# LittleDang/2DLIW-SLAM

Hardware: AMD Instinct MI355X
Metric: sliding-window solves/sec (30 KF, 2k scan pts) (higher is better)
Workload: dtype f64; 1 GPU; C2 synthetic: 49152 windows/GPU x (n=30 frames, L=2000 laser_factor blocks, 29 IMU + 29 wheel, 1800 ground); step = init-topology LM solve (cap 50 iters) + marginalization per window; windows_per_gpu=49152, frames=30, laser_blocks=2000, parallelism=windows replicated over 1 GPU(s), no data-path collective, distinct_windows_per_gpu=64

## Files before the change

2dliw-slam_amd/__init__.py:

```python
import ctypes as C
import os

import numpy as np

_HERE = os.path.dirname(os.path.abspath(__file__))
LIB_PATH = os.path.join(_HERE, "libliw_window.so")

LIW_MODE_INIT, LIW_MODE_TRACK, LIW_MODE_MARG = 0, 1, 2
LIW_ENODEV = -19
LASER_PARTIAL = 128
LASER_PARTIAL_COMPACT = 48

dp = C.POINTER(C.c_double)
ip = C.POINTER(C.c_int)
up = C.POINTER(C.c_ubyte)


class LiwError(RuntimeError):
    def __init__(self, code, msg):
        super().__init__("liw error %d: %s" % (code, msg))
        self.code = code


class ParamsC(C.Structure):
    _fields_ = [("T_imu_to_wheel", C.c_double * 16), ("T_imu_to_laser", C.c_double * 16), ("g", C.c_double),
                ("line_to_line_sigma", C.c_double), ("manifold_p_sigma", C.c_double), ("manifold_q_sigma", C.c_double),
                ("imu_noise_acc_sigma", C.c_double * 3), ("imu_bias_acc_sigma", C.c_double * 3),
                ("imu_noise_gyro_sigma", C.c_double * 3), ("imu_bias_gyro_sigma", C.c_double * 3),
                ("wheel_sigma", C.c_double * 3), ("fast_mode", C.c_int), ("normalize_extrinsics", C.c_int),
                ("device", C.c_int)]


class WindowC(C.Structure):
    _fields_ = [("n", C.c_int), ("L", C.c_int), ("states", dp), ("laser_frame", ip), ("laser_pts", dp),
                ("match_pose", dp), ("has_match", up), ("imu_X", dp), ("imu_J", dp), ("imu_sqrtP", dp), ("imu_Dt", dp),
                ("wheel_T", dp), ("wheel_sqrtP", dp), ("wheel_Dt", dp)]


class SummaryC(C.Structure):
    _fields_ = [("iterations", C.c_int), ("successful_steps", C.c_int), ("termination", C.c_int),
                ("initial_cost", C.c_double), ("final_cost", C.c_double)]


class BatchC(C.Structure):
    _fields_ = [("B", C.c_int), ("n", C.c_int), ("Ltot", C.c_int), ("x", C.c_void_p), ("laser_off", C.c_void_p),
                ("laser_frame", C.c_void_p), ("laser_pts", C.c_void_p), ("match_pose", C.c_void_p),
                ("has_match", C.c_void_p), ("imu_X", C.c_void_p), ("imu_J", C.c_void_p), ("imu_sqrtP", C.c_void_p),
                ("imu_Dt", C.c_void_p), ("wheel_T", C.c_void_p), ("wheel_sqrtP", C.c_void_p), ("prior_X", C.c_void_p),
                ("prior_J", C.c_void_p), ("prior_R", C.c_void_p), ("has_prior", C.c_void_p), ("eval_small", C.c_int),
                ("history_records", C.c_int)]


class WsLayoutC(C.Structure):
    _fields_ = [("bytes", C.c_size_t), ("laser_partial_off", C.c_size_t * 2), ("laser_partial_bytes", C.c_size_t),
                ("info_off", C.c_size_t), ("history_off", C.c_size_t), ("laser_partial_stride", C.c_int)]


EXPORTS = [
    "liw_create", "liw_destroy", "liw_last_error", "liw_get_extrinsics", "liw_set_window", "liw_clear_window", "liw_solve", "liw_get_history",
    "liw_linearize", "liw_eval_factors", "liw_marginalize", "liw_get_prior", "liw_set_prior", "liw_batch_ws_layout",
    "liw_batch_set_max_iters", "liw_batch_launch_paths", "liw_batch_packed_rows", "liw_batch_linearize", "liw_batch_time_kernels", "liw_batch_lm_begin", "liw_batch_lm_linearize", "liw_batch_laser_records", "liw_batch_lm_step",
    "liw_batch_lm_finish", "liw_batch_lm_linearize_async", "liw_batch_lm_join", "liw_batch_exchange_doubles", "liw_batch_exchange_pack",
    "liw_batch_exchange_unpack", "liw_batch_solve_sharded", "liw_batch_exchange_timing", "liw_batch_p2p_area_doubles", "liw_batch_p2p_setup", "liw_batch_p2p_status", "liw_batch_solve", "liw_batch_marg_linearize", "liw_batch_marg_schur", "liw_batch_export_dense",
    "liw_set_timing", "liw_get_timing", "liw_batch_imu_preint", "liw_batch_wheel_preint", "liw_imu_preint_create", "liw_imu_preint_destroy", "liw_imu_preint_reset",
    "liw_imu_preint_add", "liw_imu_preint_update_only_t", "liw_imu_preint_Dt", "liw_imu_preint_result",
    "liw_wheel_preint_create", "liw_wheel_preint_destroy", "liw_wheel_preint_reset", "liw_wheel_preint_add",
    "liw_wheel_preint_update_only_t", "liw_wheel_preint_result",
]

_LIB = None


def lib():
    global _LIB
    if _LIB is None:
        if not os.path.exists(LIB_PATH):
            raise LiwError(-2, "libliw_window.so is not built (run python 2dliw-slam_amd/build.py); there is no CPU fallback")
        try:
            import torch
        except ImportError:
            pass
        L = C.CDLL(LIB_PATH)
        L.liw_create.restype = C.c_void_p
        L.liw_create.argtypes = [C.POINTER(ParamsC)]
        L.liw_last_error.restype = C.c_char_p
        L.liw_last_error.argtypes = [C.c_void_p]
        L.liw_destroy.argtypes = [C.c_void_p]
        L.liw_imu_preint_create.restype = C.c_void_p
        L.liw_imu_preint_create.argtypes = [C.POINTER(ParamsC)]
        L.liw_wheel_preint_create.restype = C.c_void_p
        L.liw_wheel_preint_create.argtypes = [C.POINTER(ParamsC)]
        L.liw_imu_preint_Dt.restype = C.c_double
        for name in ("liw_imu_preint_destroy", "liw_wheel_preint_destroy"):
            getattr(L, name).argtypes = [C.c_void_p]
        _LIB = L
    return _LIB


def params_struct(prm, device=0):
    s = ParamsC()
    s.T_imu_to_wheel[:] = [float(v) for v in np.asarray(prm["T_imu_to_wheel"], dtype=np.float64).reshape(16)]
    s.T_imu_to_laser[:] = [float(v) for v in np.asarray(prm["T_imu_to_laser"], dtype=np.float64).reshape(16)]
    for k in ("g", "line_to_line_sigma", "manifold_p_sigma", "manifold_q_sigma"):
        setattr(s, k, float(prm[k]))
    for k in ("imu_noise_acc_sigma", "imu_bias_acc_sigma", "imu_noise_gyro_sigma", "imu_bias_gyro_sigma", "wheel_sigma"):
        getattr(s, k)[:] = [float(v) for v in prm[k]]
    s.fast_mode = int(bool(prm.get("fast_mode", False)))
    s.normalize_extrinsics = int(bool(prm.get("normalize_extrinsics", True)))
    s.device = int(device)
    return s


def _p(a):
    return a.ctypes.data_as(dp)
# ... 216 lines not shown
```

2dliw-slam_amd/batch.py:

```python
import ctypes as C

import numpy as np


XFN = C.CFUNCTYPE(C.c_int, C.c_void_p, C.c_void_p, C.c_void_p, C.c_size_t, C.c_void_p)


def shard_laser(win, rank, world):
    L = int(np.asarray(win["laser_frame"]).shape[0])
    lo, hi = (L * rank) // world, (L * (rank + 1)) // world
    out = dict(win)
    out["laser_frame"] = np.asarray(win["laser_frame"])[lo:hi].copy()
    out["laser_pts"] = np.asarray(win["laser_pts"])[lo:hi].copy()
    return out


def allreduce_sum_(t, group=None):
    import torch.distributed as dist
    if dist.is_available() and dist.is_initialized() and dist.get_world_size(group) > 1:
        dist.all_reduce(t, op=dist.ReduceOp.SUM, group=group)
    return t


def allgather_(out, t, group=None):
# ... 164 lines not shown
        self.comm = comm if comm is not None else TorchComm(group)
        self.exchange_ms, self.exchange_calls, self._xev, self._xbuf = 0.0, 0, [], {}
        self.time_exchange = False
        if world > 1:
            windows = [shard_laser(w, rank, world) for w in windows]
        self.n = int(windows[0]["n"])
        n = self.n
        for w in windows:
            assert int(w["n"]) == n, "uniform n per batch"
        if tile is None:
            self.B = len(windows)
            host = host_arrays(windows)
            self.Ltot = int(host.pop("_Ltot"))
            self.t = {}
            for k, a in host.items():
                if a.size == 0:
                    a = np.zeros(1, dtype=a.dtype)
                self.t[k] = torch.from_numpy(a).to(self.dev)
        else:
            self.t, self.B, self.Ltot = tiled_tensors(windows, tile, self.dev)
        B = self.B
        self.history_records = int(history_records)
        lay = WsLayoutC()
        r = self.L.liw_batch_ws_layout(C.c_int(B), C.c_int(n), C.c_int(self.history_records), C.byref(lay))
        if r < 0:
            raise LiwError(r, "liw_batch_ws_layout")
        self.lay = lay
        self.ws = torch.zeros(int(lay.bytes), dtype=torch.uint8, device=self.dev)
        b = BatchC()
        b.B, b.n, b.Ltot = B, n, self.Ltot
        for k in ("x", "laser_off", "laser_frame", "laser_pts", "match_pose", "has_match", "imu_X", "imu_J", "imu_sqrtP", "imu_Dt",
                  "wheel_T", "wheel_sqrtP", "prior_X", "prior_J", "prior_R", "has_prior"):
            setattr(b, k, self.t[k].data_ptr())
        b.eval_small = 1
        b.history_records = self.history_records
        self.b = b
        nd = int(lay.laser_partial_bytes) // 8
        self.PL_raw = [self.ws[int(lay.laser_partial_off[k]):int(lay.laser_partial_off[k]) + nd * 8].view(torch.float64) for k in range(2)]
        self._pl_mode = 0

    @property
    def PL(self):
        from . import LASER_PARTIAL
        if int(self.lay.laser_partial_stride) == LASER_PARTIAL:
            return self.PL_raw
        out = []
        for k in range(2):
            o = self.torch.empty(self.B * self.n * LASER_PARTIAL, dtype=self.torch.float64, device=self.dev)
            self._chk(self.L.liw_batch_laser_records(self.h, C.byref(self.b), C.c_int(self._pl_mode), C.c_int(k), self._wsp(),
                                                     C.c_void_p(o.data_ptr()), self._stream()))
            out.append(o)
        return out

    INPUT_KEYS = ("x", "laser_off", "laser_frame", "laser_pts", "match_pose", "has_match", "imu_X", "imu_J", "imu_sqrtP", "imu_Dt", "wheel_T", "wheel_sqrtP")

    def rebind(self, t, Ltot):
        for k in self.INPUT_KEYS:
            self.t[k] = t[k]
            setattr(self.b, k, t[k].data_ptr())
        self.Ltot = int(Ltot)
        self.b.Ltot = int(Ltot)

    def close(self):
        if self.h:
            self.L.liw_destroy(self.h)
            self.h = None

    def __del__(self):
        try:
            self.close()
        except Exception:
            pass

    def _chk(self, r):
        if r < 0:
            raise self.LiwError(r, self.L.liw_last_error(self.h).decode())
        return r

    def _stream(self):
        return C.c_void_p(self.torch.cuda.current_stream(self.dev).cuda_stream)

    def _wsp(self):
        return C.c_void_p(self.ws.data_ptr())

    def launch_paths(self):
        flags, rows, blocks = C.c_int(0), C.c_longlong(0), C.c_longlong(0)
        self._chk(self.L.liw_batch_launch_paths(self.h, C.byref(self.b), self._wsp(), C.byref(flags)))
        self._chk(self.L.liw_batch_packed_rows(self.h, C.byref(self.b), self._wsp(), C.byref(rows), C.byref(blocks)))
        return dict(flags=flags.value, large_batch_format=bool(flags.value & 1), lane_per_group_laser=bool(flags.value & 2), packed_rows=rows.value,
                    blocks=blocks.value, padding_ratio=(64.0 * rows.value / blocks.value) if (rows.value and blocks.value) else None)

    def solve(self, mode, max_iters=0, use_graph=False):
        self._pl_mode = int(mode)
        if not self.sharded:
            if use_graph:
                torch = self.torch
                if getattr(self, "_side", None) is None:
                    self._side = torch.cuda.Stream(device=self.dev)
                cur = torch.cuda.current_stream(self.dev)
                self._side.wait_stream(cur)
                with torch.cuda.stream(self._side):
                    self._chk(self.L.liw_batch_solve(self.h, C.byref(self.b), C.c_int(mode), C.c_int(max_iters), self._wsp(), self._stream(), C.c_int(1)))
                cur.wait_stream(self._side)
                return
            self._chk(self.L.liw_batch_solve(self.h, C.byref(self.b), C.c_int(mode), C.c_int(max_iters), self._wsp(), self._stream(), C.c_int(0)))
            return
# ... 323 lines not shown
```

2dliw-slam_amd/csrc/k_linearize.hip:

```cpp
#include <type_traits>
#include <cstring>
#include "liw_kernels.hpp"

#ifndef LIW_IMU_PROBE_NOSTORE
#define LIW_IMU_PROBE_NOSTORE 0
#endif
#ifndef LIW_IMU_PROBE_PHASE
#define LIW_IMU_PROBE_PHASE 0
#endif
namespace liw {

__device__ __forceinline__ void frame_tf_record(const DevParams& P, const double* pose6, int dir, double* o) {
    V3<LJ> p = cast_v3<LJ>(pose6);
    V3<LJ> th(LJ(pose6[3], dir == 0 ? 1.0 : 0.0), LJ(pose6[4], dir == 1 ? 1.0 : 0.0), LJ(pose6[5], dir == 2 ? 1.0 : 0.0));
    Iso<LJ> Twl = mul(make_tf(p, th), cast_iso<LJ>(P.Ril, P.til));
    const LJ tt[2] = {Twl.t.x, Twl.t.y};
    if (dir == 3) {
        for (int r = 0; r < 2; ++r) { for (int c = 0; c < 3; ++c) o[r * 3 + c] = Twl.R(r, c).v; o[6 + r] = tt[r].v; }
    } else {
        for (int r = 0; r < 2; ++r) { for (int c = 0; c < 3; ++c) o[8 + 6 * dir + r * 3 + c] = Twl.R(r, c).d; o[26 + 2 * dir + r] = tt[r].d; }
    }
}
template <int V, int BIT>
__device__ __forceinline__ void bfly_step(double* v, int lane) {
// ... 410 lines not shown
#pragma unroll
                    for (int r = 0; r < 4; ++r) img[so_d[r]] = (ml == 15 && !with_gi) ? 0.0 : gd[r];
                    lds_sync();
                    if (lane < 60 && !LIW_IMU_PROBE_NOSTORE) nt_store<4>(reinterpret_cast<dbl2*>(rec + PIF_D + 2 * lane), *reinterpret_cast<const dbl2*>(img + 2 * lane));
                    if (lane < 15) rec[PIF_GI + lane] = img[120 + lane];
                    lds_sync();
                };
                diag_out(g00, rf, true);
                if (lastb) diag_out(g11, rf + PIFS, false);
                if (mk == 3 && ml == 15) { rf[PIFS + PIF_C] = g00[3]; if (A.CS[0]) (sel ? A.CS[1] : A.CS[0])[cs_index(n, bq, CS_IMU, kq)] = g00[3]; }
                continue;
            }
            double* out = (sel ? A.PI[1] : A.PI[0]) + fg * PIS;
#pragma unroll
            for (int r = 0; r < 4; ++r) {
                const int row = mk + 4 * r;
                if (row < 15 && ml < 15) {
                    out[PI_IJ + row * 15 + ml] = g01[r];
                    if (ml >= row) {
                        const int tq = row * 15 - (row * (row - 1)) / 2 + (ml - row);
                        out[PI_II + tq] = g00[r];
                        out[PI_JJ + tq] = g11[r];
                    }
                }
                if (row < 15 && ml == 15) out[PI_G + row] = g00[r];
                if (r == 3) {
                    if (row == 15 && ml < 15) out[PI_G + 15 + ml] = g01[r];
                    if (row == 15 && ml == 15) out[PI_C] = g00[r];
                }
                if (A.dbg_imu_res && ml == 15 && row < 15) A.dbg_imu_res[fg * 15 + row] = y0[r];
                if (A.dbg_imu_jac && row < 15 && ml < 15) {
                    A.dbg_imu_jac[(fg * 15 + row) * 30 + ml] = y0[r];
                    A.dbg_imu_jac[(fg * 15 + row) * 30 + 15 + ml] = y1[r];
                }
            }
        }
        if constexpr (COAL) {
#pragma unroll
            for (int q = 0; q < GRP; ++q) sraw[q] = srawn[q];
        } else {
#pragma unroll
            for (int q = 0; q < GRP; ++q)
#pragma unroll
                for (int c = 0; c < 4; ++c) sop[q][c] = sopn[q][c];
        }
    }
    LSTAMP(311);
}

constexpr int WHEEL_PER_WAVE = 21;
struct WheelRcTab { int e[PWS]; };
constexpr WheelRcTab make_wheel_rc() {
    WheelRcTab t{};
    for (int e = 0; e < PWS; ++e) {
        int r = 12, c = 12;
        if (e < PW_IJ(0, 0) || (e >= PW_JJ(0, 0) && e < PW_G(0))) {
            const int jj = e >= PW_JJ(0, 0);
            int q = e - (jj ? PW_JJ(0, 0) : 0);
            r = 0;
            while (q >= 6 - r) { q -= 6 - r; ++r; }
            c = r + q + (jj ? 6 : 0); r += jj ? 6 : 0;
        } else if (e < PW_JJ(0, 0)) { r = (e - PW_IJ(0, 0)) / 6; c = 6 + (e - PW_IJ(0, 0)) % 6; }
        else if (e < PW_C) { r = e - PW_G(0); c = 12; }
        t.e[e] = e <= PW_C ? (r << 8) | c : -1;
    }
    return t;
}
__constant__ WheelRcTab c_wheel_rc = make_wheel_rc();
template <int ND, bool COSTCOPY>
__device__ __forceinline__ void wheel_blocks(const LinArgs& A, const DevParams& P, int wave, double* lds, const int* const act) {
    constexpr int LPB = 9 / ND;
    constexpr int MAXB = 63 / LPB;
    typedef LJN<ND> JN;
    const int lane = threadIdx.x & 63, blk = lane / LPB, g = lane % LPB;
    const int f = g / (LPB / 3), e0 = ND == 3 ? 0 : g % 3;
    const int n = A.n, nb = n - 1;
    const long total = (long)(act ? act[0] : A.B) * nb, gb = (long)wave * A.small_per_wave + blk;
    bool on = blk < A.small_per_wave && gb < total;
    const int wi = on ? (int)(gb / nb) : 0, k = on ? (int)(gb % nb) : 0;
    const int b = act ? act[1 + wi] : wi;
    if (on && !act) on = window_live(A, b);
    double* Y = lds + (blk < MAXB ? blk : 0) * 64;
    const size_t fk = on ? (size_t)b * nb + k : 0;
    if (on) {
        const double* si_ = A.x + ((size_t)b * n + k) * 15;
        const double* sj_ = si_ + 15;
        const double* T12 = A.wheel_T + fk * 12;
        const double* sq9 = A.wheel_sqrtP + fk * 9;
        const V3<double> thi = cast_v3<double>(si_ + 3), thj = cast_v3<double>(sj_ + 3);
        V3<JN> arg;
        {
            JN* ac[3] = {&arg.x, &arg.y, &arg.z};
            const double av[3] = {f == 1 ? thj.x : thi.x, f == 1 ? thj.y : thi.y, f == 1 ? thj.z : thi.z};
#pragma unroll
            for (int c = 0; c < 3; ++c) {
                *ac[c] = JN(av[c]);
#pragma unroll
                for (int e = 0; e < ND; ++e) if (f < 2 && c == e0 + e) ac[c]->d[e] = 1.0;
            }
        }
        const M3<JN> Md = exp_so3(arg);
        M3<double> Ri, Rj;
        {
            const int l0 = lane - g;
#pragma unroll
            for (int q = 0; q < 9; ++q) {
                const double mv = Md.m[q].v;
                Ri.m[q] = __shfl(mv, l0, 64);
                Rj.m[q] = __shfl(mv, l0 + LPB / 3, 64);
            }
        }
        const M3<double> Riw = cast_m3<double>(P.Riw);
        const V3<double> tiw(P.tiw[0], P.tiw[1], P.tiw[2]);
        const M3<double> Rwi = mul(Ri, Riw);
        const M3<double> Am = transpose(Rwi);
        const M3<double> RjRiw = mul(Rj, Riw);
        const V3<double> Rjt = mul(Rj, tiw);
        const V3<double> w(Rjt.x + sj_[0] - si_[0], Rjt.y + sj_[1] - si_[1], Rjt.z + sj_[2] - si_[2]);
// ... 83 lines not shown
    if (on && A.dbg_wheel_jac)
        for (int e = g; e < 36; e += LPB) A.dbg_wheel_jac[fk * 36 + e] = Y[(e / 12) * 13 + e % 12];
    int* meta = reinterpret_cast<int*>(lds + WHEEL_PER_WAVE * 64);
    if (g == 0 && blk < MAXB) {
        meta[blk] = on ? (A.lm ? (A.candidate ? 1 - A.lm[b].cur : A.lm[b].cur) : 0) : -1;
        meta[32 + blk] = (int)fk;
        meta[64 + blk] = (int)cs_index(n, b, CS_WHEEL, k);
    }
    lds_sync();
    {
        const long gb0 = (long)wave * A.small_per_wave;
        const int nblk = (int)min((long)A.small_per_wave, total - gb0);
        const int ml = lane < MAXB ? lane : 0;
        const int selv = meta[ml], fkv = meta[32 + ml], csv = meta[64 + ml];
        const bool all_on = __builtin_amdgcn_ballot_w64(lane < nblk && selv < 0) == 0;
        if (lane < PWS / 2) {
            const int rc0 = c_wheel_rc.e[2 * lane], rc1 = c_wheel_rc.e[2 * lane + 1];
            const int r0 = rc0 >> 8, c0 = rc0 & 255;
            const int r1 = rc1 >= 0 ? rc1 >> 8 : 0, c1 = rc1 >= 0 ? rc1 & 255 : 0;
            auto block = [&](int q) {
                const double* Yq = lds + q * 64;
                double2 v;
                v.x = __builtin_fma(Yq[26 + r0], Yq[26 + c0], __builtin_fma(Yq[r0], Yq[c0], Yq[13 + r0] * Yq[13 + c0]));
                const double w1 = __builtin_fma(Yq[26 + r1], Yq[26 + c1], __builtin_fma(Yq[r1], Yq[c1], Yq[13 + r1] * Yq[13 + c1]));
                v.y = rc1 >= 0 ? w1 : 0.0;
                return v;
            };
            auto put = [&](int q, const double2& v) {
                const int sel = __builtin_amdgcn_readlane(selv, q);
                nt_store<8>(reinterpret_cast<double2*>(&(sel ? A.PW[1] : A.PW[0])[(size_t)__builtin_amdgcn_readlane(fkv, q) * PWS + 2 * lane]), v);
            };
            int q = 0;
            if (all_on)
                for (; q + 3 <= nblk; q += 3) {
                    const double2 va = block(q), vb = block(q + 1), vc = block(q + 2);
                    put(q, va); put(q + 1, vb); put(q + 2, vc);
                }
            for (; q < nblk; ++q) {
                const double2 v = block(q);
                if (__builtin_amdgcn_readlane(selv, q) >= 0) put(q, v);
            }
        }
        if (COSTCOPY && A.CS[0] && lane < nblk && selv >= 0) {
            const double* Yq = lds + lane * 64;
            (selv ? A.CS[1] : A.CS[0])[csv] = __builtin_fma(Yq[38], Yq[38], __builtin_fma(Yq[12], Yq[12], Yq[25] * Yq[25]));
        }
    }
}

constexpr int GROUND_PER_WAVE = 32;
struct GroundRcTab { int e[PGS]; };
constexpr GroundRcTab make_ground_rc() {
    GroundRcTab t{};
    for (int e = 0; e < PGS; ++e) {
        int r = 0, c = e;
        while (c >= 7 - r) { c -= 7 - r; ++r; }
        t.e[e] = (r << 8) | (c + r);
    }
    return t;
}
__constant__ GroundRcTab c_ground_rc = make_ground_rc();
template <bool COSTCOPY>
__device__ __forceinline__ void ground_frames(const LinArgs& A, const DevParams& P, int wave, double* lds, const int* const act) {
    const int lane = threadIdx.x & 63, sub = lane >> 1, g = lane & 1;
    const int n = A.n;
    const long total = (long)(act ? act[0] : A.B) * n, gf = (long)wave * GROUND_PER_WAVE + sub;
    bool on = gf < total;
    const int wi = on ? (int)(gf / n) : 0;
    const int b = act ? act[1 + wi] : wi;
    if (on && !act) on = window_live(A, b);
    double* Y = lds + sub * 16;
    const size_t fi = on ? (size_t)b * n + (size_t)(gf % n) : 0;
    if (on) {
        const double* s_ = A.x + fi * 15;
        J3 res[2];
        {
            V3<J3> q;
            q.x = seed<3>(s_[3], 0, g == 1); q.y = seed<3>(s_[4], 1, g == 1); q.z = seed<3>(s_[5], 2, g == 1);
            const M3<J3> R = exp_so3(q);
            const J3 pz = seed<3>(s_[2], 2, g == 0);
            res[0] = (R(2, 0) * P.tiw[0] + R(2, 1) * P.tiw[1] + R(2, 2) * P.tiw[2] + pz) * P.ground_p_info;
            const J3 zx = R(0, 0) * P.Riw[2] + R(0, 1) * P.Riw[5] + R(0, 2) * P.Riw[8];
            const J3 zy = R(1, 0) * P.Riw[2] + R(1, 1) * P.Riw[5] + R(1, 2) * P.Riw[8];
            res[1] = dasin(dsqrt(zy * zy + zx * zx)) * P.ground_q_info;
        }
#pragma unroll
        for (int e = 0; e < 3; ++e) { Y[3 * g + e] = res[0].d[e]; Y[7 + 3 * g + e] = res[1].d[e]; }
        if (g == 0) { Y[6] = res[0].v; Y[13] = res[1].v; }
        if (g == 0 && A.dbg_ground_res) { A.dbg_ground_res[fi * 2] = res[0].v; A.dbg_ground_res[fi * 2 + 1] = res[1].v; }
        if (A.dbg_ground_jac)
            for (int e = 0; e < 3; ++e) { A.dbg_ground_jac[(fi * 2) * 6 + 3 * g + e] = res[0].d[e]; A.dbg_ground_jac[(fi * 2 + 1) * 6 + 3 * g + e] = res[1].d[e]; }
    }
    int* meta = reinterpret_cast<int*>(lds + GROUND_PER_WAVE * 16);
    if (g == 0) { meta[sub] = on ? (A.lm ? (A.candidate ? 1 - A.lm[b].cur : A.lm[b].cur) : 0) : -1; meta[32 + sub] = (int)fi; meta[64 + sub] = (int)cs_index(n, b, CS_GROUND, (int)(gf % n)); }
    lds_sync();
    {
        const long gf0 = (long)wave * GROUND_PER_WAVE;
        const int nfr = (int)min((long)GROUND_PER_WAVE, total - gf0);
        const double mult = (double)n;
        constexpr int LPF = PGS / 2;
        const int j = lane / LPF, pr = lane - j * LPF;
        const bool all_on = __builtin_amdgcn_ballot_w64(lane < nfr && meta[lane & 31] < 0) == 0;
        if (j < 4) {
            const int rc0 = c_ground_rc.e[2 * pr], rc1 = c_ground_rc.e[2 * pr + 1];
            const int r0 = rc0 >> 8, c0 = rc0 & 255, r1 = rc1 >> 8, c1 = rc1 & 255;
            auto frame = [&](int q) {
                const double* Yq = lds + q * 16;
                double2 v;
                v.x = mult * __builtin_fma(Yq[7 + r0], Yq[7 + c0], Yq[r0] * Yq[c0]);
                v.y = mult * __builtin_fma(Yq[7 + r1], Yq[7 + c1], Yq[r1] * Yq[c1]);
                return v;
            };
            auto put = [&](int sel, int fq, const double2& v) { nt_store<8>(reinterpret_cast<double2*>(&(sel ? A.PG[1] : A.PG[0])[(size_t)fq * PGS + 2 * pr]), v); };
            int q = j;
            if (all_on)
                for (; q + 4 < nfr; q += 8) {
                    const int sa = meta[q], fa = meta[32 + q], sb = meta[q + 4], fb = meta[36 + q];
                    const double2 va = frame(q), vb = frame(q + 4);
                    put(sa, fa, va); put(sb, fb, vb);
                }
            for (; q < nfr; q += 4) {
                const int sel = meta[q], fq = meta[32 + q];
                const double2 v = frame(q);
                if (sel >= 0) put(sel, fq, v);
            }
        }
        if (COSTCOPY && A.CS[0] && lane < nfr && meta[lane & 31] >= 0) {
            const double* Yq = lds + lane * 16;
            (meta[lane] ? A.CS[1] : A.CS[0])[meta[64 + lane]] = mult * __builtin_fma(Yq[13], Yq[13], Yq[6] * Yq[6]);
        }
    }
}

constexpr int WG_PER_WAVE = 31, WG_REC = 68;
constexpr int WG_LDS = WG_PER_WAVE * WG_REC + 96;
__device__ __forceinline__ LJN<4> ext4(const J3& a) { LJN<4> r; r.v = a.v; r.d[0] = a.d[0]; r.d[1] = a.d[1]; r.d[2] = a.d[2]; r.d[3] = 0.0; return r; }
template <bool COSTCOPY>
__device__ __forceinline__ void wheel_ground2_blocks(const LinArgs& A, const DevParams& P, int wave, double* lds, const int* const act) {
    typedef LJN<4> J4;
    typedef LJN<6> J6;
    const int lane = threadIdx.x & 63, blk = lane >> 1, f = lane & 1;
    const int n = A.n, nb = n - 1;
    const long total = (long)(act ? act[0] : A.B) * nb, gb = (long)wave * A.small_per_wave + blk;
    bool on = blk < A.small_per_wave && blk < WG_PER_WAVE && gb < total;
    const int wi = on ? (int)(gb / nb) : 0, k = on ? (int)(gb % nb) : 0;
    const int b = act ? act[1 + wi] : wi;
    if (on && !act) on = window_live(A, b);
    double* Y = lds + (blk < WG_PER_WAVE ? blk : 0) * WG_REC;
    const size_t fk = on ? (size_t)b * nb + k : 0, fi0 = on ? (size_t)b * n + k : 0;
    if (on) {
#if defined(LIW_SMALL_PROBE_INCACHE)
        const double* si_ = A.x;
        const double* sj_ = si_ + 15;
        const double* T12 = A.wheel_T;
        const double* sq9 = A.wheel_sqrtP;
#else
// ... 81 lines not shown
            const J6 dx = p.x / len, dy = p.y / len;
            const J6 cz = dy * odx - dx * ody;
            angle = dasin(dsqrt(cz * cz));
        } else {
            angle = len;
        }
        if (len.v < 0.0001 || o_len < 0.0001) res0 = len * sq9[0];
        else res0 = (J6(o_len) - len) * sq9[0];
        res1 = angle * sq9[4];
        const J4 nq = norm(q);
        const double noq = sqrt(oq.x * oq.x + oq.y * oq.y + oq.z * oq.z);
        J4 res2;
        if (nq.v < 0.001 || noq < 0.001) res2 = nq * sq9[8];
        else res2 = (J4(noq) - nq) * sq9[8];
#pragma unroll
        for (int e = 0; e < 3; ++e) {
            const int col = f ? 9 + e : 3 + e;
            Y[col] = res0.d[e]; Y[13 + col] = res1.d[e]; Y[26 + col] = res2.d[e];
        }
        if (f == 0) {
            const double Dp[3][3] = {{res0.d[3], res0.d[4], res0.d[5]}, {res1.d[3], res1.d[4], res1.d[5]}, {res2.d[3], res2.d[3], res2.d[3]}};
#pragma unroll
            for (int r = 0; r < 3; ++r) {
#pragma unroll
                for (int c = 0; c < 3; ++c) {
                    const double v = Dp[r][0] * Rwi.m[c * 3] + Dp[r][1] * Rwi.m[c * 3 + 1] + Dp[r][2] * Rwi.m[c * 3 + 2];
                    Y[r * 13 + 6 + c] = v;
                    Y[r * 13 + c] = -v;
                }
            }
            Y[12] = res0.v; Y[25] = res1.v; Y[38] = res2.v;
        }
    }
    lds_sync();
    if (on && f == 0 && A.dbg_wheel_res)
        for (int r = 0; r < 3; ++r) A.dbg_wheel_res[fk * 3 + r] = Y[r * 13 + 12];
    if (on && A.dbg_wheel_jac)
        for (int e = f; e < 36; e += 2) A.dbg_wheel_jac[fk * 36 + e] = Y[(e / 12) * 13 + e % 12];
    int* meta = reinterpret_cast<int*>(lds + WG_PER_WAVE * WG_REC);
    if (f == 0 && blk < WG_PER_WAVE) {
        meta[blk] = on ? (A.lm ? (A.candidate ? 1 - A.lm[b].cur : A.lm[b].cur) : 0) : -1;
        meta[32 + blk] = (int)fk;
        meta[64 + blk] = (int)cs_index(n, b, CS_WHEEL, k);
        meta[96 + blk] = (int)fi0;
        meta[128 + blk] = (int)cs_index(n, b, CS_GROUND, k);
        meta[160 + blk] = k;
    }
    lds_sync();
    const long gb0 = (long)wave * A.small_per_wave;
    const int nblk = (int)min((long)min(A.small_per_wave, WG_PER_WAVE), total - gb0);
    const int ml = lane < WG_PER_WAVE ? lane : 0;
    const int selv = meta[ml], fkv = meta[32 + ml], csv = meta[64 + ml], fiv = meta[96 + ml], cgv = meta[128 + ml], kv = meta[160 + ml];
    const bool all_on = __builtin_amdgcn_ballot_w64(lane < nblk && selv < 0) == 0;
    if (lane < PWS / 2) {
        const int rc0 = c_wheel_rc.e[2 * lane], rc1 = c_wheel_rc.e[2 * lane + 1];
        const int r0 = rc0 >> 8, c0 = rc0 & 255;
        const int r1 = rc1 >= 0 ? rc1 >> 8 : 0, c1 = rc1 >= 0 ? rc1 & 255 : 0;
        auto block = [&](int q) {
            const double* Yq = lds + q * WG_REC;
            double2 v;
            v.x = __builtin_fma(Yq[26 + r0], Yq[26 + c0], __builtin_fma(Yq[r0], Yq[c0], Yq[13 + r0] * Yq[13 + c0]));
            const double w1 = __builtin_fma(Yq[26 + r1], Yq[26 + c1], __builtin_fma(Yq[r1], Yq[c1], Yq[13 + r1] * Yq[13 + c1]));
            v.y = rc1 >= 0 ? w1 : 0.0;
            return v;
        };
        auto put = [&](int q, const double2& v) {
            const int sel = __builtin_amdgcn_readlane(selv, q);
            nt_store<8>(reinterpret_cast<double2*>(&(sel ? A.PW[1] : A.PW[0])[(size_t)__builtin_amdgcn_readlane(fkv, q) * PWS + 2 * lane]), v);
        };
        int q = 0;
        if (all_on)
            for (; q + 3 <= nblk; q += 3) {
                const double2 va = block(q), vb = block(q + 1), vc = block(q + 2);
                put(q, va); put(q + 1, vb); put(q + 2, vc);
            }
        for (; q < nblk; ++q) {
            const double2 v = block(q);
            if (__builtin_amdgcn_readlane(selv, q) >= 0) put(q, v);
        }
    }
    {
        const double mult = (double)n;
        constexpr int LPF = PGS / 2;
        const int j = lane / LPF, pr = lane - j * LPF;
        const bool any_k0 = __builtin_amdgcn_ballot_w64(lane < nblk && kv == 0) != 0;
        if (j < 4) {
            const int rc0 = c_ground_rc.e[2 * pr], rc1 = c_ground_rc.e[2 * pr + 1];
            const int r0 = rc0 >> 8, c0 = rc0 & 255, r1 = rc1 >> 8, c1 = rc1 & 255;
            for (int pass = 0; pass < (any_k0 ? 2 : 1); ++pass) {
                const int yo = pass ? 53 : 39;
                for (int q = j; q < nblk; q += 4) {
                    const int sel = meta[q], fq = meta[96 + q] + (pass ? 0 : 1), kq = meta[160 + q];
                    const double* Yq = lds + q * WG_REC + yo;
                    double2 v;
                    v.x = mult * __builtin_fma(Yq[7 + r0], Yq[7 + c0], Yq[r0] * Yq[c0]);
                    v.y = mult * __builtin_fma(Yq[7 + r1], Yq[7 + c1], Yq[r1] * Yq[c1]);
                    if (sel >= 0 && (pass == 0 || kq == 0))
                        nt_store<8>(reinterpret_cast<double2*>(&(sel ? A.PG[1] : A.PG[0])[(size_t)fq * PGS + 2 * pr]), v);
                }
            }
        }
        if (COSTCOPY && A.CS[0] && lane < nblk && selv >= 0) {
            const double* Yq = lds + lane * WG_REC;
            double* CSb = selv ? A.CS[1] : A.CS[0];
            CSb[csv] = __builtin_fma(Yq[38], Yq[38], __builtin_fma(Yq[12], Yq[12], Yq[25] * Yq[25]));
            CSb[cgv + 1] = mult * __builtin_fma(Yq[39 + 13], Yq[39 + 13], Yq[39 + 6] * Yq[39 + 6]);
            if (kv == 0) CSb[cgv] = mult * __builtin_fma(Yq[53 + 13], Yq[53 + 13], Yq[53 + 6] * Yq[53 + 6]);
        }
        (void)fiv;
    }
}

__host__ __device__ inline int imu_wave_count(int B, int n, int per_wave) { return n > 1 ? (int)(((long)B * (n - 1) + per_wave - 1) / per_wave) : 0; }
__host__ __device__ inline int wheel_wave_count(int B, int n, int per_wave) { return imu_wave_count(B, n, per_wave); }
__host__ __device__ inline int ground_wave_count(int B, int n) { return (int)(((long)B * n + GROUND_PER_WAVE - 1) / GROUND_PER_WAVE); }
template <int ND, bool COSTCOPY>
__device__ __forceinline__ void small_role(const LinArgs& A, const DevParams& P, int vblock, double* lds, const int* const act) {
    const int nw = wheel_wave_count(A.B, A.n, A.small_per_wave);
    if (vblock < nw) wheel_blocks<ND, COSTCOPY>(A, P, vblock, lds, act);
    else ground_frames<COSTCOPY>(A, P, vblock - nw, lds, act);
}
constexpr int SMALL_LDS = WHEEL_PER_WAVE * 64 + 32 + 16 + 64;
__global__ __launch_bounds__(64, 2) void k_lin_imu(LinArgs A, DevParams P) {
    __shared__ double lds[IMU_PER_WAVE * IMU_REC];
    const int* const act = usable_active_list(A.active, A.B);
    if (A.imu_pk && *A.imu_pk_bad == 0) imu_blocks<3, true>(A, P, (int)blockIdx.x, lds, act);
    else imu_blocks<3>(A, P, (int)blockIdx.x, lds, act);
}
__global__ __launch_bounds__(64, 2) void k_lin_imu_chain(LinArgs A, DevParams P) {
    __shared__ __attribute__((aligned(16))) double lds[IMU_PER_WAVE * IMU_REC + IMU_STAGE + IMU_SBUF];
    const int* const act = usable_active_list(A.active, A.B);
    if (A.imu_pk && *A.imu_pk_bad == 0) imu_blocks<3, true, true>(A, P, (int)blockIdx.x, lds, act);
    else imu_blocks<3, false, true>(A, P, (int)blockIdx.x, lds, act);
}
__global__ __launch_bounds__(64, 2) void k_lin_imu_chain_multi(LinArgs A, DevParams P) {
    __shared__ __attribute__((aligned(16))) double lds[IMU_PER_WAVE * IMU_REC + IMU_STAGE + IMU_SBUF];
    const int* const act = usable_active_list(A.active, A.B);
    if (A.imu_pk && *A.imu_pk_bad == 0) imu_blocks<3, true, true, true>(A, P, (int)blockIdx.x, lds, act);
    else imu_blocks<3, false, true, true>(A, P, (int)blockIdx.x, lds, act);
// ... 207 lines not shown
            hipStreamWaitEvent(s, fk->ev_join[1], 0);
        }
    }
}
void launch_linearize_join(hipStream_t s, const LinFork* fk) {
    if (!fk || !fk->side[0]) return;
    hipStreamWaitEvent(s, fk->ev_join[0], 0);
    hipStreamWaitEvent(s, fk->ev_join[1], 0);
}

__global__ void k_exchange_pack(int groups, int n, int np, int compact, LaserPackTable tb, const double* PL0, const double* PL1, int candidate, const LmState* lm, double* buf) {
    const int t = blockIdx.x * blockDim.x + threadIdx.x;
    if (t >= groups * np) return;
    const int grp = t / np, p = t % np;
    const bool dead = lm && lm[grp / n].done;
    const int sel = lm ? (candidate ? 1 - lm[grp / n].cur : lm[grp / n].cur) : 0;
    const double* PL = sel ? PL1 : PL0;
    double v;
    if (compact) v = PL[(size_t)grp * LPC + p];
    else { v = PL[(size_t)grp * LP + tb.slot[p]]; v = tb.neg[p] ? -v : v; }
    buf[t] = dead ? 0.0 : v;
}
template <bool BOTH>
__global__ void k_exchange_unpack(int groups, int n, int np, int compact, int world, size_t stride, const double* buf, double* PL0, double* PL1, double* CS0, double* CS1, int candidate, const LmState* lm, int sysload) {
    const int t = blockIdx.x * blockDim.x + threadIdx.x;
    const int lps = laser_stride(compact);
    if (t >= groups * lps) return;
    const int grp = t / lps, s = t % lps;
    const int sel = lm ? (candidate ? 1 - lm[grp / n].cur : lm[grp / n].cur) : 0;
    double* PL = sel ? PL1 : PL0;
    const int code = compact ? (s < np ? s : -1) : laser_slot_code<BOTH>(s);
    double v = 0.0;
    if (code >= 0) {
        const double* src = buf + (size_t)grp * np + (code & 63);
        for (int r = 0; r < world; ++r)
            v += sysload ? __hip_atomic_load(src + (size_t)r * stride, __ATOMIC_RELAXED, __HIP_MEMORY_SCOPE_SYSTEM) : src[(size_t)r * stride];
        if (code & 64) v = -v;
    }
    PL[t] = v;
    if (s == (compact ? np - 1 : 120) && CS0) (sel ? CS1 : CS0)[cs_index(n, grp / n, CS_LASER, grp % n)] = v;
}
template <bool BOTH>
__global__ void k_laser_expand(int groups, int compact, const double* PL, double* out) {
    const size_t t = (size_t)blockIdx.x * blockDim.x + threadIdx.x;
    if (t >= (size_t)groups * LP) return;
    out[t] = laser_slot<BOTH>(PL + (t / LP) * laser_stride(compact), (int)(t % LP), compact);
}
void launch_laser_expand(int B, int n, bool both, int compact, const double* PL, double* out, hipStream_t s) {
    const int groups = B * n;
    const unsigned blocks = (unsigned)(((size_t)groups * LP + 255) / 256);
    if (both) hipLaunchKernelGGL(k_laser_expand<true>, dim3(blocks), dim3(256), 0, s, groups, compact, PL, out);
    else hipLaunchKernelGGL(k_laser_expand<false>, dim3(blocks), dim3(256), 0, s, groups, compact, PL, out);
}
__global__ void k_count_active(int B, const LmState* lm, double* out) {
    __shared__ int cnt;
    if (threadIdx.x == 0) cnt = 0;
    __syncthreads();
    int c = 0;
    for (int b = threadIdx.x; b < B; b += blockDim.x) c += lm[b].done ? 0 : 1;
    atomicAdd(&cnt, c);
    __syncthreads();
    if (threadIdx.x == 0) out[0] = (double)cnt;
}
void launch_exchange_pack(int B, int n, bool both, int compact, const double* PL0, const double* PL1, int candidate, const LmState* lm, double* buf, hipStream_t s) {
    const int np = both ? 45 : 21, groups = B * n;
    LaserPackTable tb{};
    for (int p = 0; p < np; ++p) tb.slot[p] = -1;
    for (int sl = 0; sl < LP; ++sl) {
        const int code = both ? laser_slot_code<true>(sl) : laser_slot_code<false>(sl);
        if (code >= 0 && tb.slot[code & 63] < 0) { tb.slot[code & 63] = sl; tb.neg[code & 63] = (code & 64) ? 1 : 0; }
    }
    hipLaunchKernelGGL(k_exchange_pack, dim3((groups * np + 255) / 256), dim3(256), 0, s, groups, n, np, compact, tb, PL0, PL1, candidate, lm, buf);
    if (lm) hipLaunchKernelGGL(k_count_active, dim3(1), dim3(256), 0, s, B, lm, buf + (size_t)groups * np);
}
void launch_exchange_unpack(int B, int n, bool both, int compact, int world, size_t stride, const double* buf, double* PL0, double* PL1, double* CS0, double* CS1, int candidate, const LmState* lm, hipStream_t s, bool sysload) {
    const int np = both ? 45 : 21, groups = B * n, lps = laser_stride(compact);
    if (both) hipLaunchKernelGGL(k_exchange_unpack<true>, dim3((groups * lps + 255) / 256), dim3(256), 0, s, groups, n, np, compact, world, stride, buf, PL0, PL1, CS0, CS1, candidate, lm, sysload ? 1 : 0);
    else hipLaunchKernelGGL(k_exchange_unpack<false>, dim3((groups * lps + 255) / 256), dim3(256), 0, s, groups, n, np, compact, world, stride, buf, PL0, PL1, CS0, CS1, candidate, lm, sysload ? 1 : 0);
}

__global__ void k_p2p_push(size_t nd, const double* buf, P2pPeers peers, int rank, int world, int parity) {
    const size_t t = (size_t)blockIdx.x * blockDim.x + threadIdx.x;
    if (t >= nd) return;
    const double v = buf[t];
    for (int p = 0; p < world; ++p)
        __hip_atomic_store(peers.area[p] + ((size_t)(parity * world + rank)) * nd + t, v, __ATOMIC_RELAXED, __HIP_MEMORY_SCOPE_SYSTEM);
}
__global__ void k_p2p_signal(P2pPeers peers, int rank, int world, unsigned long long epoch) {
    const int p = threadIdx.x;
    if (p >= world) return;
    __atomic_thread_fence(__ATOMIC_RELEASE);
    __hip_atomic_store(peers.flags[p] + rank, epoch, __ATOMIC_RELEASE, __HIP_MEMORY_SCOPE_SYSTEM);
}
__global__ void k_p2p_wait(const unsigned long long* flags, int world, unsigned long long epoch, long long max_polls, int* err) {
    const int r = threadIdx.x;
    if (r < world && *(volatile int*)err == 0) {
        long long polls = 0;
        while (__hip_atomic_load(flags + r, __ATOMIC_RELAXED, __HIP_MEMORY_SCOPE_SYSTEM) < epoch) {
            __builtin_amdgcn_s_sleep(32);
            if (++polls > max_polls) { atomicExch(err, 1 + r); break; }
        }
    }
    __syncthreads();
    __atomic_thread_fence(__ATOMIC_ACQUIRE);
}
void launch_p2p_exchange(size_t nd, const double* buf, const P2pPeers& peers, int rank, int world, unsigned long long epoch, int* err, hipStream_t s) {
// ... 15 lines not shown
```

2dliw-slam_amd/csrc/k_lm.hip:

```cpp
#include "liw_kernels.hpp"
#include "k_lm_common.hpp"

namespace liw {

typedef double d4 __attribute__((ext_vector_type(4)));
#ifdef LIW_CLK
__device__ long long g_clk[8192];
__device__ long long g_span[3 * 16384];
#ifndef LIW_CLK_IT
#define LIW_CLK_IT 3
#endif
#define STAMP(id) do { if (b == 0 && lane == 0 && iteration_dbg == LIW_CLK_IT) g_clk[(id)] = clock64(); } while (0)
#define STAMPE(id) do { if (b == 0 && lane == 0 && iteration == LIW_CLK_IT) g_clk[(id)] = clock64(); } while (0)
#define STAMPM(id) do { if (b == 0 && lane == 0) g_clk[(id)] = clock64(); } while (0)
#define JSTAMP(id) do { if (t == 0 && blockIdx.x == 0 && sweep == 1 && rnd == 3) g_clk[(id)] = clock64(); } while (0)
#define JSTAMPV(id, v) do { double w_ = (v); asm volatile("" : "+v"(w_)); if (t == 0 && blockIdx.x == 0 && sweep == 1 && rnd == 3) g_clk[(id)] = clock64(); } while (0)
#define SPAN(k) do { if (lane == 0 && iteration_dbg == LIW_CLK_IT && b < 16384) { g_span[3 * b + (k)] = clock64(); \
                     if ((k) == 0) g_span[3 * b + 2] = __builtin_amdgcn_s_getreg((4 << 0) | (0 << 6) | (31 << 11)); } } while (0)
#else
#define STAMP(id) do { } while (0)
#define STAMPE(id) do { } while (0)
#define STAMPM(id) do { } while (0)
#define JSTAMP(id) do { } while (0)
#define JSTAMPV(id, v) do { } while (0)
#define SPAN(k) do { } while (0)
#endif


struct AsmCtx {
    int n, mode, fast, b, buf;
    int pif;
    int plc;
    const double* PL; const double* PI; const double* PW; const double* PG;
    const double* x;
    const double* pJ; const double* pX; bool prior_on;
};

__device__ __forceinline__ double prior_r(const AsmCtx& c, int k) {
    const double* xs = c.x + (size_t)(c.n - 2) * 15;
    double s = 0.0;
    for (int j = 0; j < 15; ++j) s += c.pJ[k * 15 + j] * (xs[j] - c.pX[j]);
    return s;
}

__device__ __forceinline__ double pl_slot(const AsmCtx& c, const double* rec, int s) { return laser_slot(rec, s, c.plc, c.mode == LIW_MODE_INIT); }

struct FrameExtra { double sc_i, sc_m, dg_i, x_i; };

constexpr int MS = 41;
template <int LAYOUT> struct Tiles {
    double* D; double* O; double* R; double* g;
    __device__ __forceinline__ double& d(int r, int c) const { return LAYOUT ? D[r * MS + c] : D[r * 16 + c]; }
    __device__ __forceinline__ double& o(int r, int c) const { return LAYOUT ? D[c * MS + 16 + r] : O[r * 16 + c]; }
    __device__ __forceinline__ double& rr(int r, int c) const { return LAYOUT ? D[c * MS + 32 + r] : R[r * 16 + c]; }
    __device__ __forceinline__ double& gg(int r) const { return LAYOUT ? D[r * MS + 40] : g[r]; }
};

struct AsmRegs {
    double v5[4], v6[4], v7[4];
    double t1, t2, t3, t4, t8, t9, t10;
    double g1, g2, g3, g4, g5, g6;
    double xq, sc_i, sc_m, dg_i;
    double e1[2], e2;
};
struct PriorRegs { double pj[4], pdx; };
__device__ __forceinline__ PriorRegs prior_issue(const AsmCtx& c, int lane) {
    PriorRegs P;
#pragma unroll
    for (int q = 0; q < 4; ++q) {
        const int e = lane + 64 * q, r = e >> 4, cc = e & 15;
        P.pj[q] = (r < 15 && cc < 15) ? c.pJ[r * 15 + cc] : 0.0;
    }
    const int v = lane < 15 ? lane : 0;
    P.pdx = c.x[(size_t)(c.n - 2) * 15 + v] - c.pX[v];
    return P;
}
constexpr int ASM_TMP = 16;

__device__ __forceinline__ AsmRegs asm_issue(const AsmCtx& c, int i, const double* scl, const double* dgl, int lane = threadIdx.x & 63, int dir = -1) {
    const int n = c.n;
    const bool up = dir > 0;
    const int LPS = laser_stride(c.plc);
    const double* PLb = c.PL + (size_t)c.b * n * LPS;
    const bool pif = c.pif != 0;
    const bool hasm = i >= 1, hasp = i <= n - 2;
    const double* PIb = c.PI + (size_t)c.b * (pif ? (size_t)n * PIFS : (size_t)(n - 1) * PIS);
    const double* PWb = c.PW + (size_t)c.b * (n - 1) * PWS;
    const double* PGb = c.PG + (size_t)c.b * n * PGS;
    const double* PIm = pif ? PIb + (size_t)i * PIFS : PIb + (size_t)(hasm ? i - 1 : 0) * PIS;
    const double* PIp = pif ? PIb + (size_t)(hasp ? i + 1 : i) * PIFS : PIb + (size_t)(hasp ? i : 0) * PIS;
    const int oJJ = pif ? PIF_D : PI_JJ, oIJ = pif ? PIF_IJ : PI_IJ;
    const double* PWm = PWb + (size_t)(hasm ? i - 1 : 0) * PWS;
    const double* PWp = PWb + (size_t)(hasp ? i : 0) * PWS;
    const double* PLi = PLb + (size_t)i * LPS;
    const double* PL1 = PLb + (size_t)(n > 1 ? 1 : 0) * LPS;
    const double* PGi = PGb + (size_t)i * PGS;
    AsmRegs R;
#pragma unroll
    for (int q = 0; q < 4; ++q) {
        const int e = lane + 64 * q, r = e >> 4, cc = e & 15;
        const bool valid = r < 15 && cc < 15;
        const int rs = valid ? r : 0, cs = valid ? cc : 0;
        const int tq = pi_tri(rs, cs);
        R.v5[q] = PIm[(unsigned)(oJJ + tq)];
        R.v6[q] = pif ? 0.0 : PIp[(unsigned)(PI_II + tq)];
        R.v7[q] = up ? PIp[(unsigned)(oIJ + cs * 15 + rs)] : PIm[(unsigned)(oIJ + rs * 15 + cs)];
    }
    {
        const bool pl = lane < 36;
        const int r = pl ? lane / 6 : 0, cc = pl ? lane % 6 : 0;
        R.t1 = pl_slot(c, PLi, 36 + r * 6 + cc);
        R.t2 = PWm[(unsigned)PW_JJ(r, cc)];
        R.t3 = PWp[(unsigned)PW_II(r, cc)];
        R.t4 = PGi[(unsigned)PG_H(r, cc)];
        R.t8 = up ? PWp[(unsigned)PW_IJ(cc, r)] : PWm[(unsigned)PW_IJ(r, cc)];
        R.e2 = up ? PWm[(unsigned)PW_IJ(r, cc)] : 0.0;
        R.t9 = pl_slot(c, PL1, 72 + r * 6 + cc);
        R.t10 = pl_slot(c, PLi, 72 + r * 6 + cc);
    }
    {
        const int r = lane < 15 ? lane : 0, r6 = r < 6 ? r : 0;
        R.g1 = pl_slot(c, PLi, 114 + r6);
        R.g2 = PWm[(unsigned)PW_G(6 + r6)];
        R.g3 = PWp[(unsigned)PW_G(r6)];
        R.g4 = PGi[(unsigned)PG_G(r6)];
        R.g5 = PIm[(unsigned)((pif ? PIF_GJ : PI_G + 15) + r)];
        R.g6 = pif ? PIm[(unsigned)(PIF_GI + r)] : PIp[(unsigned)(PI_G + r)];
    }
    const int nbf = up ? (hasp ? i + 1 : i) : (hasm ? i - 1 : i);
    {
        int idx = i * 15 + (lane < 15 ? lane : 0);
        if (lane >= 16 && lane < 19) idx = nbf * 15 + 3 + (lane - 16);
        if (lane >= 20 && lane < 23) idx = 3 + (lane - 20);
        R.xq = c.x[(unsigned)idx];
        const int v = lane < 15 ? lane : 0;
        R.sc_i = scl ? scl[(unsigned)(i * 15 + v)] : 1.0;
        R.sc_m = scl ? scl[(unsigned)(nbf * 15 + v)] : 1.0;
        R.dg_i = dgl ? dgl[(unsigned)(i * 15 + v)] : 0.0;
    }
#pragma unroll
    for (int q = 0; q < 2; ++q) {
        const int e = lane + 64 * q;
        R.e1[q] = up ? PIm[(unsigned)(oIJ + (e < 90 ? e : 0))] : 0.0;
    }
    return R;
}

__device__ __forceinline__ d4 xty16(const double* X, const double* Y);
template <int LAYOUT>
__device__ void asm_commit(const AsmCtx& c, int i, const AsmRegs& R, const Tiles<LAYOUT>& T_, double* tmp, FrameExtra* ex = nullptr,
                           int lane = threadIdx.x & 63, int dir = -1, const PriorRegs* pr = nullptr) {
    const int n = c.n;
    const int LPS = laser_stride(c.plc);
    const double* PLb = c.PL + (size_t)c.b * n * LPS;
    const bool hasm = i >= 1, hasp = i <= n - 2;
    const bool up = dir > 0, hasnb = up ? hasp : hasm;
    const int nbf = up ? (hasp ? i + 1 : i) : (hasm ? i - 1 : i);
    const bool arrow1 = up && i == 1;
    const bool prior_here = c.prior_on && i == n - 2;
    d4 jtj = {0.0, 0.0, 0.0, 0.0};
    double gprior = 0.0;
    if (prior_here) {
        double* Jt = T_.D;
        double* dxp = LAYOUT ? T_.D + 256 : T_.O;
        const PriorRegs P_ = pr ? *pr : prior_issue(c, lane);
#pragma unroll
        for (int q = 0; q < 4; ++q) Jt[lane + 64 * q] = P_.pj[q];
        if (lane < 16) dxp[lane] = lane < 15 ? P_.pdx : 0.0;
        lds_sync();
        if (lane < 15) {
            double sp = 0.0;
#pragma unroll
            for (int j = 0; j < 15; ++j) sp += Jt[lane * 16 + j] * dxp[j];
            tmp[lane] = sp;
        }
        jtj = xty16(Jt, Jt);
        lds_sync();
        if (lane < 15) {
// ... 98 lines not shown
                    double t[3];
                    for (int k = 0; k < 3; ++k) t[k] = at(kind, r, 3) * P[k] + at(kind, r, 4) * P[3 + k] + at(kind, r, 5) * P[6 + k];
                    for (int k = 0; k < 3; ++k) at(kind, r, 3 + k) = t[k];
                }
            };
            auto left = [&](int kind, const double* P) {
                for (int cc = 0; cc < 15; ++cc) {
                    double t[3];
                    for (int k = 0; k < 3; ++k) t[k] = P[k] * at(kind, 3, cc) + P[3 + k] * at(kind, 4, cc) + P[6 + k] * at(kind, 5, cc);
                    for (int k = 0; k < 3; ++k) at(kind, 3 + k, cc) = t[k];
                }
            };
            if (li) {
                right(0, 15, Pi); left(0, Pi); right(1, 15, Pi); right(2, 6, Pi);
                double t[3];
                for (int k = 0; k < 3; ++k) t[k] = Pi[k] * T_.gg(3) + Pi[3 + k] * T_.gg(4) + Pi[6 + k] * T_.gg(5);
                for (int k = 0; k < 3; ++k) T_.gg(3 + k) = t[k];
            }
            if (lm) left(1, Pm);
            if (l0) left(2, P0);
        }
        lds_sync();
    }
    if (c.mode == LIW_MODE_TRACK) {
        for (int e = lane; e < 256; e += 64) {
            const int r = e >> 4, cc = e & 15;
            if (r < 15 && cc < 15) {
                const bool cr = var_is_const(c.mode, c.fast, n, i, r), ccn = var_is_const(c.mode, c.fast, n, i, cc);
                if (cr || ccn) T_.d(r, cc) = 0.0;
                if ((hasnb && var_is_const(c.mode, c.fast, n, nbf, r)) || ccn) T_.o(r, cc) = 0.0;
                if (arrow1 && r < 6 && (var_is_const(c.mode, c.fast, n, 0, r) || ccn)) T_.rr(r, cc) = 0.0;
            }
        }
        if (lane < 15 && var_is_const(c.mode, c.fast, n, i, lane)) T_.gg(lane) = 0.0;
        lds_sync();
    }
}

template <int LAYOUT>
__device__ void assemble_frame(const AsmCtx& c, int i, const Tiles<LAYOUT>& T_, double* tmp,
                               const double* scl = nullptr, const double* dgl = nullptr, FrameExtra* ex = nullptr) {
    const AsmRegs R = asm_issue(c, i, scl, dgl);
    __builtin_amdgcn_sched_barrier(0);
    asm_commit<LAYOUT>(c, i, R, T_, tmp, ex);
}

__device__ double window_cost(const AsmCtx& c, double* gchk = nullptr) {
    const int lane = threadIdx.x & 63;
    const int n = c.n;
    const int LPS = laser_stride(c.plc);
    const double* PLb = c.PL + (size_t)c.b * n * LPS;
    const bool pif = c.pif != 0;
    const double* PIb = c.PI + (size_t)c.b * (pif ? (size_t)n * PIFS : (size_t)(n - 1) * PIS);
    const double* PWb = c.PW + (size_t)c.b * (n - 1) * PWS;
    const double* PGb = c.PG + (size_t)c.b * n * PGS;
    const bool track = c.mode == LIW_MODE_TRACK;
    double s = 0.0, gs = 0.0;
    for (int i = lane; i < n; i += 64) {
        const bool gon = !(track && i < n - 1);
        if (gon) s += pl_slot(c, PLb + (size_t)i * LPS, 120);
        if (gon) s += PGb[(size_t)i * PGS + PG_C];
        if (gchk) {
            if (gon) {
#pragma unroll
                for (int k = 0; k < 12; ++k) gs += pl_slot(c, PLb + (size_t)i * LPS, 108 + k);
            }
            if (gon) {
#pragma unroll
                for (int k = 0; k < 6; ++k) gs += PGb[(size_t)i * PGS + PG_G(k)];
            }
        }
    }
    for (int k = lane; k < n - 1; k += 64) {
        s += pif ? PIb[(size_t)(k + 1) * PIFS + PIF_C] : PIb[(size_t)k * PIS + PI_C];
        const bool won = !(track && k < n - 2);
        if (won) s += PWb[(size_t)k * PWS + PW_C];
        if (gchk) {
#pragma unroll
            for (int e = 0; e < 30; ++e)
                gs += pif ? (e < 15 ? PIb[(size_t)k * PIFS + PIF_GI + e] : PIb[(size_t)(k + 1) * PIFS + PIF_GJ + e - 15]) : PIb[(size_t)k * PIS + PI_G + e];
            if (won) {
#pragma unroll
                for (int e = 0; e < 12; ++e) gs += PWb[(size_t)k * PWS + PW_G(e)];
            }
        }
    }
    if (c.prior_on && lane < 15) { const double r = prior_r(c, lane); s += r * r; }
    if (gchk) *gchk = wave_sum(gs);
    return 0.5 * wave_sum(s);
}

__device__ __forceinline__ d4 xty16(const double* X, const double* Y) {
    const int lane = threadIdx.x & 63;
    d4 acc = {0.0, 0.0, 0.0, 0.0};
#pragma unroll
    for (int c = 0; c < 4; ++c) {
        const int k = (lane >> 4) + 4 * c;
        acc = __builtin_amdgcn_mfma_f64_16x16x4f64(X[k * 16 + (lane & 15)], Y[k * 16 + (lane & 15)], acc, 0, 0, 0);
    }
    return acc;
}

template <int XS, int YS>
__device__ __forceinline__ d4 xty15(const double* X, const double* Y, const double* Z) {
    const int lane = threadIdx.x & 63, m = lane & 15;
    d4 acc = {0.0, 0.0, 0.0, 0.0};
#pragma unroll
    for (int c = 0; c < 4; ++c) {
        const int k = (lane >> 4) + 4 * c;
        const double* xr = X + k * XS;
        const double* yr = Y + k * YS;
        if (c == 3) { const bool z = (lane >> 4) == 3; xr = z ? Z : xr; yr = z ? Z : yr; }
        acc = __builtin_amdgcn_mfma_f64_16x16x4f64(xr[m], yr[m], acc, 0, 0, 0);
    }
    return acc;
}

struct LdsTiles {
    double D[256], O[256], R[256], W[256], Wa[256], CD[256], CR[256];
    double g[16], Cg[16], y0[16], yprev[16], tmp[ASM_TMP], D0acc[36], g0acc[8], sci[16], scm[16], sc0[16], dgi[16];
};
struct LdsStep {
    double M[720], C[15 * MS], Z[16];
    double tmp[ASM_TMP], D0acc[36], g0acc[8];
};
constexpr int LW = 0, LLI = 240, LWA = 480;
struct LdsDense2 {
    LdsStep S;
    double D1[256], O1[256], R1[256], D0[256], O0[256], R0[256], g1[16], g0[16];
};
__device__ __forceinline__ LdsStep& step_lds(LdsStep& T) { return T; }
__device__ __forceinline__ LdsStep& step_lds(LdsDense2& T) { return T.S; }

template <int NP = 15>
__device__ __forceinline__ bool fused_chol_solve(double (&a)[15]) {
    bool ok = true;
#pragma unroll
    for (int k = 0; k < NP; ++k) {
        const double piv = rdlane(a[k], k);
        if (k == NP - 1 && (!(piv > 0.0) || !isfinite(piv))) ok = false;
        const double inv = fast_rsqrt(piv);
        const double wk = a[k] * inv;
        a[k] = wk;
#pragma unroll
        for (int r = k + 1; r < 15; ++r) a[r] -= rdlane(wk, r) * wk;
    }
    return ok;
}

__device__ __forceinline__ bool fused_chol_solve30(double (&a)[30], unsigned inert) {
    bool ok = true;
#pragma unroll
    for (int k = 0; k < 30; ++k) {
        if (k < 15 && ((inert >> k) & 1u)) continue;
        const double piv = rdlane(a[k], k);
        if (k == 29 && (!(piv > 0.0) || !isfinite(piv))) ok = false;
        const double inv = fast_rsqrt(piv);
        const double wk = a[k] * inv;
        a[k] = wk;
#pragma unroll
        for (int r = k + 1; r < 30; ++r) a[r] -= rdlane(wk, r) * wk;
    }
    return ok;
}

template <bool WAVE_ONLY = false>
__device__ double frame_diag(const AsmCtx& c, int i, LdsStep& T) {
    const int lane = threadIdx.x & 63, n = c.n;
    double Pq[9];
    if (so3_plus_jac(c.x + (size_t)i * 15 + 3, Pq)) {
        assemble_frame<1>(c, i, Tiles<1>{T.M, nullptr, nullptr, nullptr}, T.tmp);
        const double d = lane < 15 ? T.M[lane * MS + lane] : 0.0;
        lds_sync();
        return d;
    }
    if (lane >= 15) return 0.0;
    const int r = lane;
    const int LPS = laser_stride(c.plc);
    const double* PLb = c.PL + (size_t)c.b * n * LPS;
    const double* PIb = c.PI + (size_t)c.b * (c.pif ? (size_t)n * PIFS : (size_t)(n - 1) * PIS);
    const double* PWb = c.PW + (size_t)c.b * (n - 1) * PWS;
    const double* PGb = c.PG + (size_t)c.b * n * PGS;
    double d = 0.0;
    if (r < 6) {
        d += pl_slot(c, PLb + (size_t)i * LPS, 36 + r * 7);
        if (i == 0) for (int j = 0; j < n; ++j) d += pl_slot(c, PLb + (size_t)j * LPS, r * 7);
        if (i >= 1) d += PWb[(size_t)(i - 1) * PWS + PW_JJ(r, r)];
        if (i <= n - 2) d += PWb[(size_t)i * PWS + PW_II(r, r)];
        d += PGb[(size_t)i * PGS + PG_H(r, r)];
    }
    if (c.pif) { if (n > 1) d += PIb[(size_t)i * PIFS + PIF_D + pi_tri(r, r)]; }
    else {
        if (i >= 1) d += PIb[(size_t)(i - 1) * PIS + PI_JJ + pi_tri(r, r)];
        if (i <= n - 2) d += PIb[(size_t)i * PIS + PI_II + pi_tri(r, r)];
    }
    if (c.prior_on && i == n - 2) { double s = 0.0; for (int k = 0; k < 15; ++k) s += c.pJ[k * 15 + r] * c.pJ[k * 15 + r]; d += s; }
    return d;
}

template <bool THROUGHPUT, bool DENSE2 = false, class LDS = LdsStep>
__device__ __forceinline__ void lm_step_body(const StepArgs& a, const int b, LDS& TL) {
    constexpr bool LIW_PF1 = !THROUGHPUT, LIW_PF2 = true;
    LdsStep& T = step_lds(TL);
    const int lane = threadIdx.x & 63;
    LmState& st = a.w.lm[b];
    if constexpr (DENSE2) {
        double pf_sink = 0.0;
        int done0 = st.done;
        const int n2 = a.n;
        const bool pr = a.mode == LIW_MODE_TRACK && !a.fast_mode;
        double v[14];
#pragma unroll
        for (int k = 0; k < 2; ++k) {
            v[4 * k + 0] = touch_lines(a.w.PL[k] + (size_t)b * n2 * laser_stride(a.w.pl_compact), sizeof(double) * n2 * laser_stride(a.w.pl_compact));
            v[4 * k + 1] = touch_lines(a.w.PI[k] + (size_t)b * (n2 - 1) * PIS, sizeof(double) * (n2 - 1) * PIS);
            v[4 * k + 2] = touch_lines(a.w.PW[k] + (size_t)b * (n2 - 1) * PWS, sizeof(double) * (n2 - 1) * PWS);
            v[4 * k + 3] = touch_lines(a.w.PG[k] + (size_t)b * n2 * PGS, sizeof(double) * n2 * PGS);
        }
        v[8] = touch_lines(a.x + (size_t)b * n2 * 15, sizeof(double) * n2 * 15);
        v[9] = touch_lines(a.w.x_cand + (size_t)b * n2 * 15, sizeof(double) * n2 * 15);
        v[10] = touch_lines(st.scale, sizeof(double) * n2 * 15);
        v[11] = touch_lines(st.diagonal, sizeof(double) * n2 * 15);
        {
            const double* const xb = a.x + (size_t)b * n2 * 15;
            const double* const PJ = a.prior_J; const double* const PX = a.prior_X;
            const bool pj = pr && PJ != nullptr, px = pr && PX != nullptr;
            const size_t qj = (size_t)(PJ + (size_t)b * 225), qx = (size_t)(PX + (size_t)b * 15), q0 = (size_t)xb;
            v[12] = touch_lines(reinterpret_cast<const void*>(pj ? qj : q0), pj ? sizeof(double) * 225 : sizeof(double) * 8);
            v[13] = touch_lines(reinterpret_cast<const void*>(px ? qx : q0), px ? sizeof(double) * 15 : sizeof(double) * 8);
        }
#pragma unroll
        for (int k = 0; k < 14; ++k) pf_sink += v[k];
        asm volatile("" : "+v"(pf_sink), "+v"(done0));
        if (done0) return;
    }
    if (st.done) return;
    if (a.only_slow) {
        const int taken = st.pad_;
        wave_mem_sync();
        if (taken) { if (lane == 0) st.pad_ = 0; return; }
    }
    const int n = a.n;
    double* xw = a.x + (size_t)b * n * 15;
    double* xc = a.w.x_cand + (size_t)b * n * 15;

    AsmCtx c;
    c.pif = a.w.pi_frame;
    c.plc = a.w.pl_compact;
    c.n = n; c.mode = a.mode; c.fast = a.fast_mode; c.b = b;
    c.pJ = a.prior_J + (size_t)b * 225; c.pX = a.prior_X + (size_t)b * 15;
    c.prior_on = a.mode == LIW_MODE_TRACK && a.has_prior[b] && !a.fast_mode;

    double radius = st.radius, dec = st.decrease_factor, x_cost = st.x_cost, x_norm = st.x_norm;
    int reuse = __builtin_amdgcn_readfirstlane(st.reuse_diagonal), iteration = __builtin_amdgcn_readfirstlane(st.iteration),
        cur = __builtin_amdgcn_readfirstlane(st.cur);
    bool last_successful = true;
    bool fresh = false;
    STAMPE(4000);

    if (iteration == 0 && !st.have_candidate) {
        c.buf = cur; c.PL = a.w.PL[cur]; c.PI = a.w.PI[cur]; c.PW = a.w.PW[cur]; c.PG = a.w.PG[cur]; c.x = xw;
        x_cost = window_cost(c);
        if (lane == 0) { st.initial_cost = x_cost; st.minimum_cost = x_cost; }
        if (!isfinite(x_cost)) {
            if (lane == 0) { st.done = 1; st.termination = 6; st.x_cost = x_cost; }
            return;
        }
        double s = 0.0;
        for (int e = lane; e < n * 15; e += 64) {
            const double xv = xw[e];
            st.x0[e] = xv;
            if (!var_is_const(a.mode, a.fast_mode, n, e / 15, e % 15)) s += xv * xv;
        }
        x_norm = sqrt(wave_sum(s));
        fresh = true;
        if (a.w.history && a.w.history_records > 0)
            for (int e = lane; e < n * 15; e += 64) a.w.history[((size_t)b) * n * 15 + e] = xw[e];
    } else if (st.have_candidate) {
        const int cb = 1 - cur;
        c.buf = cb; c.PL = a.w.PL[cb]; c.PI = a.w.PI[cb]; c.PW = a.w.PW[cb]; c.PG = a.w.PG[cb]; c.x = xc;
        double cand_cost = window_cost(c);
        STAMPE(4001);
        if (!isfinite(cand_cost)) cand_cost = 1.7976931348623157e308;
        int term = 0;
        if (st.cand_step_norm <= kParamTol * (x_norm + kParamTol)) term = 3;
        else if (fabs(x_cost - cand_cost) <= kFuncTol * x_cost) term = 2;
        if (term) {
            if (a.w.history && iteration < a.w.history_records)
                for (int e = lane; e < n * 15; e += 64) a.w.history[((size_t)iteration * a.B + b) * n * 15 + e] = xw[e];
            if (lane == 0) { st.done = 1; st.termination = term; }
            return;
        }
        const double rho = (x_cost - cand_cost) / st.model_cost_change;
        if (rho > kMinRelDec) {
            for (int e = lane; e < n * 15; e += 64) xw[e] = xc[e];
            cur = cb;
            x_cost = cand_cost;
            double s = 0.0;
            for (int e = lane; e < n * 15; e += 64) if (!var_is_const(a.mode, a.fast_mode, n, e / 15, e % 15)) s += xc[e] * xc[e];
            x_norm = sqrt(wave_sum(s));
            { const double t3 = 2.0 * rho - 1.0; radius = radius / fmax(1.0 / 3.0, 1.0 - t3 * t3 * t3); }
// ... 397 lines not shown
    if (b < a.B) {
        LmState& st = a.w.lm[b];
        if (!st.done) { if (st.pad_) st.pad_ = 0; else mine = true; }
    }
    unsigned long long m = __ballot(mine);
    if (!m) return;
    wave_mem_sync();
    while (m) {
        const int l = __builtin_amdgcn_readfirstlane(__builtin_ctzll(m));
        m &= m - 1;
        lm_step_body<true>(a, (int)blockIdx.x * 64 + l, T);
        lds_sync();
    }
}

__global__ __launch_bounds__(64, 1) void k_lm_step_dense2(StepArgs a) {
    __shared__ LdsDense2 T;
    if ((int)blockIdx.x >= a.B) return;
    lm_step_body<false, true, LdsDense2>(a, (int)blockIdx.x, T);
}

struct LdsTwSide {
    double PM[720], Ptmp[ASM_TMP];
    double PT[2][15 * MS];
    LdsStep T;
};
struct LdsTw {
    LdsTwSide side[2];
    double Haa[36], ga[8];
    double sc0[16], dg0[16];
    double ya[8];
    double red[4][4];
    double ctld[4];
    int ctl[8];
};

__global__ __launch_bounds__(256, 1) void k_lm_step_tw(StepArgs a) {
    __shared__ LdsTw S;
    const int b = blockIdx.x, lane = threadIdx.x & 63, w = threadIdx.x >> 6;
    if (b >= a.B) return;
    LmState& st = a.w.lm[b];
    if (st.done) return;
    const int n = a.n;
    double* xw = a.x + (size_t)b * n * 15;
    double* xc = a.w.x_cand + (size_t)b * n * 15;
    const int sd = w & 1;
    const bool producer = w >= 2;
    LdsTwSide& SS = S.side[sd];
    LdsStep& T = SS.T;

    AsmCtx c;
    c.pif = a.w.pi_frame;
    c.plc = a.w.pl_compact;
    c.n = n; c.mode = a.mode; c.fast = a.fast_mode; c.b = b;
    c.pJ = a.prior_J + (size_t)b * 225; c.pX = a.prior_X + (size_t)b * 15;
    c.prior_on = a.mode == LIW_MODE_TRACK && a.has_prior[b] && !a.fast_mode;

    double radius = 0.0, dec = 0.0, x_cost = 0.0, x_norm = 0.0;
    int reuse = 0, iteration = 0, cur = 0;
    bool last_successful = true, fresh = false;

    if (w == 0) {
        radius = st.radius; dec = st.decrease_factor; x_cost = st.x_cost; x_norm = st.x_norm;
        reuse = st.reuse_diagonal; iteration = st.iteration; cur = st.cur;
        int proceed = 1;
        if (iteration == 0 && !st.have_candidate) {
            c.buf = cur; c.PL = a.w.PL[cur]; c.PI = a.w.PI[cur]; c.PW = a.w.PW[cur]; c.PG = a.w.PG[cur]; c.x = xw;
            double gchk;
            x_cost = window_cost(c, &gchk);
            if (lane == 0) { st.initial_cost = x_cost; st.minimum_cost = x_cost; }
            double sq = 0.0;
            for (int e = lane; e < n * 15; e += 64) {
                const double xv = xw[e];
                st.x0[e] = xv;
                if (!var_is_const(a.mode, a.fast_mode, n, e / 15, e % 15)) sq += xv * xv;
            }
            x_norm = sqrt(wave_sum(sq));
            fresh = true;
            if (a.w.history && a.w.history_records > 0)
                for (int e = lane; e < n * 15; e += 64) a.w.history[((size_t)b) * n * 15 + e] = xw[e];
            if (!isfinite(x_cost) || !isfinite(gchk)) {
                if (lane == 0) { st.done = 1; st.termination = 6; st.x_cost = x_cost; }
                proceed = 0;
            }
        } else if (st.have_candidate) {
            const int cb = 1 - cur;
            c.buf = cb; c.PL = a.w.PL[cb]; c.PI = a.w.PI[cb]; c.PW = a.w.PW[cb]; c.PG = a.w.PG[cb]; c.x = xc;
            double cand_gchk;
            double cand_cost = window_cost(c, &cand_gchk);
            if (!isfinite(cand_cost)) cand_cost = 1.7976931348623157e308;
            int term = 0;
            if (st.cand_step_norm <= kParamTol * (x_norm + kParamTol)) term = 3;
            else if (fabs(x_cost - cand_cost) <= kFuncTol * x_cost) term = 2;
            const double rho = term ? 0.0 : (x_cost - cand_cost) / st.model_cost_change;
            if (term) {
                if (a.w.history && iteration < a.w.history_records)
                    for (int e = lane; e < n * 15; e += 64) a.w.history[((size_t)iteration * a.B + b) * n * 15 + e] = xw[e];
                if (lane == 0) { st.done = 1; st.termination = term; }
                proceed = 0;
            } else if (rho > kMinRelDec && !isfinite(cand_gchk)) {
                if (st.successful > 0)
                    for (int e = lane; e < n * 15; e += 64) xw[e] = st.x0[e];
                wave_mem_sync();
                if (lane == 0) { st.done = 1; st.termination = 6; st.iteration = iteration - 1; st.x_cost = st.initial_cost; st.have_candidate = 0; }
                proceed = 0;
            } else {
// ... 368 lines not shown
        } else if (a.mode == LIW_MODE_TRACK) {
            if (i == n - 1 && a.has_match[i]) a.match_pose[i * 12 + 6 + k] = a.x[(size_t)i * 15 + k];
        }
    }
    __syncthreads();
    int* hdr = reinterpret_cast<int*>(a.out);
    if (t == 0) { hdr[0] = a.lm[0].done; hdr[1] = a.marg_status ? a.marg_status[0] : 3; hdr[2] = 0; }
    if (t == 1) {
        const LmState& st = a.lm[0];
        liw_summary o;
        o.iterations = st.iteration; o.successful_steps = st.successful; o.termination = st.termination;
        o.initial_cost = st.initial_cost; o.final_cost = st.x_cost;
        *reinterpret_cast<liw_summary*>(a.out + 2) = o;
        a.info[0] = o;
    }
    double* o = a.out + LIW_RESULT_HDR;
    for (int e = t; e < n * 15; e += blockDim.x) o[e] = a.x[e];
    o += n * 15;
    for (int e = t; e < n * 12; e += blockDim.x) o[e] = a.match_pose[e];
    o += n * 12;
    if (a.marg) for (int e = t; e < 276; e += blockDim.x) o[e] = a.marg[e];
    __threadfence_system();
    __syncthreads();
    if (t == 0) { __threadfence_system(); __hip_atomic_store(hdr + 3, a.seq, __ATOMIC_RELEASE, __HIP_MEMORY_SCOPE_SYSTEM); }
}
__global__ void k_pack_result(PackArgs a) { pack_result_body(a); }

__global__ void k_lm_finish(StepArgs a) {
    const int t = blockIdx.x * blockDim.x + threadIdx.x;
    const int n = a.n;
    if (t >= a.B * n * 6) return;
    const int k = t % 6, i = (t / 6) % n, b = t / (6 * n);
    const double* xw = a.x + (size_t)b * n * 15;
    double* mp = a.match_pose + (size_t)b * n * 12;
    if (a.mode == LIW_MODE_INIT) {
        if (a.has_match[b * n + i]) { mp[i * 12 + k] = xw[k]; mp[i * 12 + 6 + k] = xw[(size_t)i * 15 + k]; }
    } else if (a.mode == LIW_MODE_TRACK) {
        if (i == n - 1 && a.has_match[b * n + i]) mp[i * 12 + 6 + k] = xw[(size_t)i * 15 + k];
    }
    if (i == 0 && k == 0) {
        const LmState& st = a.w.lm[b];
        liw_summary& o = a.w.info[b];
        o.iterations = st.iteration; o.successful_steps = st.successful; o.termination = st.termination;
        o.initial_cost = st.initial_cost; o.final_cost = st.x_cost;
    }
}

__global__ __launch_bounds__(64) void k_export_dense(ExportArgs a) {
    __shared__ LdsTiles T;
    const int b = blockIdx.x, lane = threadIdx.x & 63, n = a.n, N = 15 * n;
    AsmCtx c;
    c.pif = a.w.pi_frame;
    c.plc = a.w.pl_compact;
    c.n = n; c.mode = a.mode; c.fast = a.fast_mode; c.b = b; c.buf = a.buf;
    c.PL = a.w.PL[0]; c.PI = a.w.PI[0]; c.PW = a.w.PW[0]; c.PG = a.w.PG[0];
    c.x = a.x + (size_t)b * n * 15;
    c.pJ = a.prior_J + (size_t)b * 225; c.pX = a.prior_X + (size_t)b * 15;
    c.prior_on = a.has_prior[b] && ((a.mode == LIW_MODE_TRACK && !a.fast_mode) || a.mode == LIW_MODE_MARG);
    double* H = a.H + (size_t)b * N * N;
    double* g = a.g + (size_t)b * N;
    for (size_t e = lane; e < (size_t)N * N; e += 64) H[e] = 0.0;
    __syncthreads();
    const double sgn = a.mode == LIW_MODE_MARG ? -1.0 : 1.0;
    for (int i = 0; i < n; ++i) {
        assemble_frame<0>(c, i, Tiles<0>{T.D, T.O, T.R, T.g}, T.tmp);
        for (int e = lane; e < 256; e += 64) {
            const int r = e >> 4, cc = e & 15;
            if (r < 15 && cc < 15) {
                H[(size_t)(i * 15 + r) * N + i * 15 + cc] = T.D[e];
                if (i >= 1) { H[(size_t)((i - 1) * 15 + r) * N + i * 15 + cc] = T.O[e]; H[(size_t)(i * 15 + cc) * N + (i - 1) * 15 + r] = T.O[e]; }
                if (i >= 2 && r < 6) { H[(size_t)r * N + i * 15 + cc] = T.R[e]; H[(size_t)(i * 15 + cc) * N + r] = T.R[e]; }
            }
        }
        if (lane < 15) g[i * 15 + lane] = sgn * T.g[lane];
        __syncthreads();
    }
    const double cst = window_cost(c);
    if (lane == 0) a.cost[b] = cst;
}

template <class TILES>
__device__ __forceinline__ bool marg_chain(const MargArgs& a, const int b, TILES& T) {
    const int lane = threadIdx.x & 63, n = a.n;
    AsmCtx c;
    c.pif = a.w.pi_frame;
    c.plc = a.w.pl_compact;
    const int sel = a.use_cur ? __builtin_amdgcn_readfirstlane(a.w.lm[b].cur) : 0;
    c.n = n; c.mode = LIW_MODE_MARG; c.fast = 0; c.b = b; c.buf = sel;
    c.PL = sel ? a.w.PL[1] : a.w.PL[0]; c.PI = sel ? a.w.PI[1] : a.w.PI[0]; c.PW = sel ? a.w.PW[1] : a.w.PW[0]; c.PG = sel ? a.w.PG[1] : a.w.PG[0];
    c.x = a.x + (size_t)b * n * 15;
    c.pJ = a.prior_J + (size_t)b * 225; c.pX = a.prior_X + (size_t)b * 15;
    c.prior_on = a.has_prior[b] != 0;
    STAMPM(5000);
    for (int e = lane; e < 256; e += 64) { T.CD[e] = 0.0; T.W[e] = 0.0; }
    if (lane < 16) T.Cg[lane] = 0.0;
    lds_sync();
    bool ok = true;
    double* Dc = T.D; double* gc = T.g;
    double* Dn = T.Wa; double* gn = T.y0;
    assemble_frame<0>(c, 0, Tiles<0>{Dc, T.O, T.R, gc}, T.tmp);
    AsmRegs areg = asm_issue(c, n > 1 ? 1 : 0, nullptr, nullptr);
    for (int i = 0; i + 1 < n; ++i) {
        asm_commit<0>(c, i + 1, areg, Tiles<0>{Dn, T.O, T.R, gn}, T.tmp);
        __builtin_amdgcn_sched_barrier(0);
        if (i + 2 < n) areg = asm_issue(c, i + 2, nullptr, nullptr);
        __builtin_amdgcn_sched_barrier(0);
        double col[15];
        {
            const bool ml_ = lane < 15, ol_ = lane >= 16 && lane < 31, gl_ = lane == 40;
            const double* pA = ml_ ? Dc + lane : (ol_ ? T.O + (lane - 16) : (gl_ ? gc : T.R));
            const double* pB = ml_ ? T.CD + lane : (gl_ ? T.Cg : (ol_ ? T.Cg + 15 : T.R));
            const int st = gl_ ? 1 : 16, stB = ol_ ? 0 : st;
#pragma unroll
            for (int r = 0; r < 15; ++r) col[r] = pA[r * st] + pB[r * stB];
        }
        if (!fused_chol_solve(col)) { ok = false; break; }
        if ((lane >= 16 && lane < 31) || lane == 40) {
            double* const wc = T.W + (lane == 40 ? 15 : lane - 16);
#pragma unroll
            for (int r = 0; r < 15; ++r) wc[r * 16] = col[r];
        }
        lds_sync();
        const d4 p1 = xty16(T.W, T.W);
        lds_sync();
#pragma unroll
        for (int r = 0; r < 4; ++r) {
            const int row = (lane >> 4) + 4 * r, colx = lane & 15;
            if (row < 15 && colx < 15) T.CD[row * 16 + colx] = -p1[r];
            if (row < 15 && colx == 15) T.Cg[row] = -p1[r];
        }
        lds_sync();
        double* t1 = Dc; Dc = Dn; Dn = t1;
        double* t2 = gc; gc = gn; gn = t2;
    }
    {
        double dv[4], gv = 0.0;
#pragma unroll
        for (int q = 0; q < 4; ++q) {
            const int e = lane + 64 * q, r = e >> 4, cc = e & 15;
// ... 452 lines not shown
```

2dliw-slam_amd/csrc/k_lm_quad.hip:

```cpp
#include <cstddef>
#include <cstdlib>
#include <type_traits>

#include "liw_kernels.hpp"
#include "k_lm_common.hpp"

namespace liw {

template <int B_, int E_, class F> __device__ __forceinline__ void sfor(F&& f) {
    if constexpr (B_ < E_) { f(std::integral_constant<int, B_>{}); sfor<B_ + 1, E_>(f); }
}
#define KI(K) (std::remove_reference_t<decltype(K)>::value)
template <int V> using KC = std::integral_constant<int, V>;
__device__ __forceinline__ double bits_and(double x, unsigned long long m) { return __longlong_as_double((long long)((unsigned long long)__double_as_longlong(x) & m)); }

template <int L> __device__ __forceinline__ double bc(double v) {
    double r;
    asm volatile("v_mov_b64_dpp %0, %1 row_newbcast:%2 row_mask:0xf bank_mask:0xf" : "=v"(r) : "v"(v), "n"(L));
    return r;
}
template <int L> __device__ __forceinline__ void fnma_bc(double& acc, double src, double mul) {
    asm volatile("v_fmac_f64_dpp %0, -%1, %2 row_newbcast:%3 row_mask:0xf bank_mask:0xf" : "+v"(acc) : "v"(src), "v"(mul), "n"(L));
}
template <int L> __device__ __forceinline__ double mul_bc(double src, double mul) {
    double r;
    asm volatile("v_mul_f64_dpp %0, %1, %2 row_newbcast:%3 row_mask:0xf bank_mask:0xf" : "=v"(r) : "v"(src), "v"(mul), "n"(L));
    return r;
}
__device__ __forceinline__ double mul_nop(double x, double y) {
    double r;
    asm volatile("v_mul_f64 %0, %1, %2\n s_nop 1" : "=v"(r) : "v"(x), "v"(y));
    return r;
}
__device__ __forceinline__ void dpp_fence() { asm volatile("s_nop 1"); }

__device__ __forceinline__ double row_max(double v) {
    v = fmax(v, dpp64<0xB1>(v, v)); v = fmax(v, dpp64<0x4E>(v, v)); v = fmax(v, dpp64<0x141>(v, v)); v = fmax(v, dpp64<0x140>(v, v));
    return v;
}

__device__ long long g_qclk[64];
__device__ int g_qclk_on[4];
__device__ int g_qprobe;
#define QSTAMP(id) do { if (clk_on && i == clk_frame) { if (lane == 0) g_qclk[(id)] = clock64(); } } while (0)

#ifdef LIW_QUAD_TILE_ALIAS
constexpr int QTR = 0;
#else
constexpr int QNT1 = (LIW_NT_MASK & 16) ? 2 : 0, QNT2 = (LIW_NT_MASK & 64) ? 2 : 0;
constexpr int QTR = 4 * 15 * 6;
#endif
constexpr int K_A = 0, K_B = 6, K_C = 12, K_HA = 18, K_D = 24, K_CW = 39, K_GSH = 45, K_RL = 46, NRD = 52;
constexpr int QTAB = NRD * 16;
constexpr int QZB = 86;
constexpr int QPAD = 96;
constexpr int QTOT_1 = 4 * (PIFS + LPC + PWS + PGS) + QPAD + QTR + QZB + QTAB;
constexpr int quad_laser_slot(int kind, int r, int j) {
    return kind == 0 ? (j == 15 ? 114 + r : 36 + r * 6 + j) : kind == 1 ? (j == 15 ? 108 + r : r * 6 + j) : 72 + j * 6 + r;
}
template <bool BOTH> constexpr bool quad_sign_rows_ok() {
    for (int jj = 0; jj < 7; ++jj) {
        const int j = jj < 6 ? jj : 15;
        auto sg = [&](int kind, int r) { const int c = laser_slot_code<BOTH>(quad_laser_slot(kind, r, j)); return c >= 0 && (c & 64) != 0; };
        for (int r = 0; r < 6; ++r) {
            if (sg(1, r)) return false;
            if (sg(0, r) != (r < 2 ? sg(0, 0) : (r > 2 && sg(0, 3)))) return false;
            if (j < 6 && sg(2, r) != (r < 2 && sg(2, 0))) return false;
        }
        if (sg(0, 0) != sg(0, 1) || (j < 6 && sg(2, 0) != sg(2, 1))) return false;
    }
    return true;
}
static_assert(quad_sign_rows_ok<true>() && quad_sign_rows_ok<false>(), "sign rows of the laser reads");
template <bool BOTH> constexpr unsigned long long quad_code_pack(int kind, int r) {
    unsigned long long v = 0;
    for (int jj = 0; jj < 7; ++jj) {
        const int c = (kind == 2 && jj == 6) ? -1 : laser_slot_code<BOTH>(quad_laser_slot(kind, r, jj < 6 ? jj : 15));
        v |= (unsigned long long)(c < 0 ? 0xff : c) << (8 * jj);
    }
    return v;
}
template <int KIND, int R> __device__ __forceinline__ int quad_code(bool track, int role) {
    constexpr unsigned long long both = quad_code_pack<true>(KIND, R), one = quad_code_pack<false>(KIND, R);
    const int c = (int)(((track ? one : both) >> (8 * role)) & 0xffull);
    return c == 0xff ? -1 : c;
}
__device__ __forceinline__ double flip_sign(double x, unsigned m) { return __hiloint2double(__double2hiint(x) ^ (int)m, __double2loint(x)); }
#ifndef LIW_QUAD_BSD
#define LIW_QUAD_BSD 3
#endif
constexpr int BSD2 = LIW_QUAD_BSD;
constexpr int QTOT_2 = BSD2 * (((4 * REC_GS + 127) / 128) * 128 + 6 * 32);
constexpr int QTOT = QTOT_1 > QTOT_2 ? QTOT_1 : QTOT_2;

template <int R> __device__ __forceinline__ int tri_rc(int j, int cj) {
    constexpr int cR = 14 * R - (R * (R - 1)) / 2;
    return R <= j ? cR + j : cj + R;
}

#ifndef LIW_QUAD_OCC
#define LIW_QUAD_OCC 1
#endif
__global__ __launch_bounds__(64, LIW_QUAD_OCC) void k_lm_step_quad(StepArgs a) {
    __shared__ double S[QTOT];
    const int lane = threadIdx.x & 63, j = lane & 15, w = lane >> 4;
    const int n = a.n;
    const bool track = a.mode == LIW_MODE_TRACK;
    const int fast = a.fast_mode;
    auto is_const = [&](int i, int v) { return track && i < n - 1 && (v < 6 || (fast && v >= 9)); };
// ... 89 lines not shown
        {
            double s2 = 0.0;
            const bool restore = act && fail_eval && !fresh && successful0 > 0;
            const bool hist = act && a.w.history && iteration < a.w.history_records && !fail_eval;
            for (int e0 = j; e0 < n * 15; e0 += 16 * 8) {
                double xv[8];
#pragma unroll
                for (int q = 0; q < 8; ++q) {
                    const int e = e0 + 16 * q;
                    const unsigned ee = (unsigned)(e < n * 15 ? e : j);
                    xv[q] = restore ? LMD[oLM + LM_X0 + ee] : (accept ? XC[oX + ee] : X[oX + ee]);
                }
#pragma unroll
                for (int q = 0; q < 8; ++q) {
                    const int e = e0 + 16 * q;
                    if (e < n * 15) {
                        if (act && (accept || restore)) X[oX + (unsigned)e] = xv[q];
                        if (act && fresh) LMD[oLM + LM_X0 + (unsigned)e] = xv[q];
                        if (!is_const(e / 15, e % 15)) s2 += xv[q] * xv[q];
                        if (hist) a.w.history[((size_t)iteration * a.B + b) * (size_t)(n * 15) + e] = xv[q];
                    }
                }
            }
            s2 = row_sum(s2);
            if (fresh || accept) x_norm = sqrt(s2);
        }
        if (act && (fail_eval || term)) {
            if (j == 0) {
                st.done = 1; st.termination = fail_eval ? 6 : term;
                if (fail_eval) { st.x_cost = fresh ? cost : initial_cost0; st.have_candidate = 0; if (!fresh) st.iteration = iteration - 1; }
                if (fresh) { st.initial_cost = initial_cost; st.minimum_cost = minimum_cost; }
            }
            proceed = false;
        }
        const bool cap = proceed && iteration >= max_iters && !fresh;
        if (proceed && j == 0) {
            st.radius = radius; st.decrease_factor = dec; st.x_cost = x_cost; st.x_norm = x_norm; st.cur = cur;
            st.successful = successful; st.minimum_cost = minimum_cost;
            if (fresh) st.initial_cost = initial_cost;
            if (cap) { st.done = 1; st.termination = 4; st.reuse_diagonal = reuse; st.have_candidate = 0; }
        }
        if (cap) proceed = false;
        inv_radius = 1.0 / radius;
    }
    if (!__any(proceed)) return;

    const double* const PL0 = a.w.PL[0];
    const double* const PI0 = a.w.PI[0];
    const double* const PW0 = a.w.PW[0];
    const double* const PG0 = a.w.PG[0];
    const unsigned bp = (g_qprobe & 1) ? 0u : (unsigned)b;
    const unsigned oPL = bp * (unsigned)(n * LPC) + (cur ? (unsigned)(a.w.PL[1] - a.w.PL[0]) : 0u);
    const unsigned oPI = bp * (unsigned)(n * PIFS) + (cur ? (unsigned)(a.w.PI[1] - a.w.PI[0]) : 0u);
    const unsigned oPW = bp * (unsigned)((n - 1) * PWS) + (cur ? (unsigned)(a.w.PW[1] - a.w.PW[0]) : 0u);
    const unsigned oPG = bp * (unsigned)(n * PGS) + (cur ? (unsigned)(a.w.PG[1] - a.w.PG[0]) : 0u);
    const int qprobe = g_qprobe;
    const unsigned oWS = (qprobe & 2) ? 0u : (unsigned)b * (unsigned)(n * SOLVE_WS);
    double* const WS = a.w.solve_ws;
    const unsigned oSC = oLM + LM_SCALE, oDG = oLM + LM_DIAG;
    const int jc = j < 15 ? j : 0;
    const bool l6 = j < 6, lm = j < 15;

    const bool prior_row = track && !fast && a.has_prior[b] != 0;
    if (__any(proceed && fresh)) {
        double sp = 0.0;
        if (prior_row) for (int k = 0; k < 15; ++k) { const double v = a.prior_J[(size_t)b * 225 + k * 15 + jc]; sp += v * v; }
        const int cbb = track ? laser_slot_code<false>(36 + (l6 ? jc : 0) * 7) : laser_slot_code<true>(36 + (l6 ? jc : 0) * 7);
        const int caa = track ? laser_slot_code<false>((l6 ? jc : 0) * 7) : laser_slot_code<true>((l6 ? jc : 0) * 7);
        for (int i0 = 0; i0 < n; i0 += 4) {
            double vbb[4], vjj[4], vii[4], vg[4], vi[4];
#pragma unroll
            for (int u = 0; u < 4; ++u) {
                const int i = min(i0 + u, n - 1);
                const int j6 = l6 ? jc : 0;
                vbb[u] = PL0[oPL + (unsigned)(i * LPC + (cbb >= 0 ? cbb & 63 : 0))];
                vbb[u] = cbb >= 0 ? vbb[u] : 0.0;
                vjj[u] = n > 1 ? PW0[oPW + (unsigned)(max(i - 1, 0) * PWS + PW_JJ(j6, j6))] : 0.0;
                vii[u] = n > 1 ? PW0[oPW + (unsigned)(min(i, n - 2) * PWS + PW_II(j6, j6))] : 0.0;
                vg[u] = PG0[oPG + (unsigned)(i * PGS + PG_H(j6, j6))];
                vi[u] = PI0[oPI + (unsigned)(i * PIFS + PIF_D + pi_tri(jc, jc))];
            }
#pragma unroll
            for (int u = 0; u < 4; ++u) {
                const int i = i0 + u;
                if (i >= n) break;
                double dd = 0.0;
                if (l6) {
                    dd += vbb[u];
                    if (i == 0) for (int f = 0; f < n; ++f) { const double va = PL0[oPL + (unsigned)(f * LPC + (caa >= 0 ? caa & 63 : 0))]; dd += caa >= 0 ? va : 0.0; }
                    if (i >= 1) dd += vjj[u];
                    if (i <= n - 2) dd += vii[u];
                    dd += vg[u];
                }
                if (n > 1) dd += vi[u];
                if (prior_row && i == n - 2) dd += sp;
                if (proceed && fresh && lm) LMD[oSC + (unsigned)(i * 15 + j)] = is_const(i, j) ? 1.0 : 1.0 / (1.0 + sqrt(dd));
            }
        }
    }
    const double sc0 = l6 ? LMD[oSC + (unsigned)jc] : 0.0;

    constexpr int S_IMU = 0, S_PL = 4 * PIFS, S_PW = S_PL + 4 * LPC, S_PG = S_PW + 4 * PWS, S_TR = S_PG + 4 * PGS + QPAD;
    constexpr int S_ZERO = S_TR + QTR, S_TAB = S_ZERO + QZB;
    static_assert(S_TAB + QTAB <= QTOT && 8 * QTOT < 65536, "LDS layout");
    const unsigned rPI[4] = {(unsigned)__builtin_amdgcn_readlane(oPI, 0), (unsigned)__builtin_amdgcn_readlane(oPI, 16), (unsigned)__builtin_amdgcn_readlane(oPI, 32), (unsigned)__builtin_amdgcn_readlane(oPI, 48)};
    const unsigned rPW[4] = {(unsigned)__builtin_amdgcn_readlane(oPW, 0), (unsigned)__builtin_amdgcn_readlane(oPW, 16), (unsigned)__builtin_amdgcn_readlane(oPW, 32), (unsigned)__builtin_amdgcn_readlane(oPW, 48)};
    const unsigned oPGw = oPG + (unsigned)(PG0 - PW0);
    const unsigned oPLw = oPL + (unsigned)(PL0 - PW0);
    const unsigned rPLw[4] = {(unsigned)__builtin_amdgcn_readlane(oPLw, 0), (unsigned)__builtin_amdgcn_readlane(oPLw, 16), (unsigned)__builtin_amdgcn_readlane(oPLw, 32), (unsigned)__builtin_amdgcn_readlane(oPLw, 48)};
    const unsigned rPGw[4] = {(unsigned)__builtin_amdgcn_readlane(oPGw, 0), (unsigned)__builtin_amdgcn_readlane(oPGw, 16), (unsigned)__builtin_amdgcn_readlane(oPGw, 32), (unsigned)__builtin_amdgcn_readlane(oPGw, 48)};
    typedef __attribute__((address_space(3))) void* lds_t;
    const int j_ = j;
    double scm_n = 1.0, dg_n = 0.0, xq_n = 0.0;
    auto prefetch_regs = [&](int f) {
        const int jq = j_ < 15 ? j_ : 0;
        scm_n = (j_ < 15 && f >= 1) ? LMD[oSC + (unsigned)((f - 1) * 15 + jq)] : 1.0;
        dg_n = LMD[oDG + (unsigned)(f * 15 + jq)];
        xq_n = X[oX + (unsigned)(f * 15 + jq)];
    };
    auto prefetch = [&](int f) {
        asm volatile("s_waitcnt lgkmcnt(0)" ::: "memory");
        const int k = f - 1;
        int lane2 = lane * 2;
        asm volatile("" : "+v"(lane2));
        if (n > 1) {
            sfor<0, 4>([&](auto W) {
                constexpr int ws = KI(W);
                const double* g = PI0 + rPI[ws] + (unsigned)(f * PIFS) + lane2;
                sfor<0, 3>([&](auto Q) { __builtin_amdgcn_global_load_lds(g, (lds_t)(S + S_IMU + ws * PIFS), 16, KI(Q) * 1024, QNT1); });
            });
        }
        {
            const unsigned fl = (unsigned)(f * LPC), fw = (unsigned)((k >= 0 ? k : 0) * PWS), fg = (unsigned)(f * PGS);
            constexpr int NPC = (4 * (LPC + PWS + PGS) + 127) / 128;
            static_assert(NPC * 128 - 4 * (LPC + PWS + PGS) <= QPAD && LPC % 2 == 0 && PWS % 2 == 0 && PGS % 2 == 0, "stream pieces: pad, 16-byte slots");
            sfor<0, NPC>([&](auto P) {
                constexpr int q0 = KI(P) * 128;
                unsigned off = 0;
                sfor<0, 12>([&](auto G) {
                    constexpr int g = KI(G);
                    constexpr int st = g < 4 ? g * LPC : g < 8 ? 4 * LPC + (g - 4) * PWS : 4 * (LPC + PWS) + (g - 8) * PGS;
                    constexpr int en = g == 11 ? (1 << 20) : st + (g < 4 ? LPC : g < 8 ? PWS : PGS);
                    if constexpr (st < q0 + 128 && en > q0) {
                        const unsigned v = (g < 4 ? rPLw[g & 3] + fl : g < 8 ? rPW[g & 3] + fw : rPGw[g & 3] + fg) + (unsigned)(lane2 - (st - q0));
                        if constexpr (st <= q0) off = v; else off = lane2 >= st - q0 ? v : off;
                    }
                });
                __builtin_amdgcn_global_load_lds(PW0 + off, (lds_t)(S + S_PL + q0), 16, 0, QNT1);
            });
        }
        asm volatile("" ::: "memory");
        prefetch_regs(f);
    };
    const double* SI = S + S_IMU + w * PIFS;
    unsigned short* const TAB = reinterpret_cast<unsigned short*>(S + S_TAB);
    {
        const int jt = j < 15 ? j : 0, cjt = 14 * jt - (jt * (jt - 1)) / 2, j6t = j < 6 ? j : 0;
        const bool t6 = j < 6, t15 = j == 15, tm = j < 15;
        const int oL = S_PL + w * LPC, oW_ = S_PW + w * PWS, oG = S_PG + w * PGS, oI = S_IMU + w * PIFS;
        auto put = [&](int k, bool on, int idx) { TAB[k * 64 + lane] = (unsigned short)(8 * (on ? idx : S_ZERO)); };
        const int role = t15 ? 6 : j6t;
        auto put_laser = [&](int k, bool on, int code) { put(k, on && code >= 0, oL + (code & 63)); };
        for (int e = lane; e < QZB; e += 64) S[S_ZERO + e] = 0.0;
        sfor<0, 6>([&](auto R) {
            constexpr int r = KI(R);
            put_laser(K_A + r, t6 || t15, quad_code<0, r>(track, role));
            put(K_B + r, t6 || t15, oW_ + (t15 ? PW_G(6 + r) : PW_JJ(r, j6t)));
            put(K_C + r, t6 || t15, oG + (t15 ? PG_G(r) : PG_H(r, j6t)));
            put_laser(K_HA + r, t6 || t15, quad_code<1, r>(track, role));
            put(K_CW + r, t6 || t15, oW_ + (t15 ? PW_G(r) : PW_II(r, j6t)));
            put_laser(K_RL + r, t6, quad_code<2, r>(track, role));
        });
        put(K_GSH, t6, oW_ + PW_G(j6t));
        sfor<0, 15>([&](auto R) {
            constexpr int r = KI(R);
            put(K_D + r, tm, oI + PIF_D + tri_rc<r>(jt, cjt));
        });
    }
    unsigned sgA0, sgA3, sgR0;
    {
        const bool t6 = j < 6, t15 = j == 15;
        const int role = t15 ? 6 : (t6 ? j : 0);
        const int cA0 = quad_code<0, 0>(track, role), cA3 = quad_code<0, 3>(track, role), cR0 = quad_code<2, 0>(track, role);
        sgA0 = ((t6 || t15) && cA0 >= 0 && (cA0 & 64)) ? 0x80000000u : 0u;
        sgA3 = ((t6 || t15) && cA3 >= 0 && (cA3 & 64)) ? 0x80000000u : 0u;
        sgR0 = (t6 && cR0 >= 0 && (cR0 & 64)) ? 0x80000000u : 0u;
    }
    const int lane_tab = lane * 2;
    auto RD = [&](auto K) -> double {
        constexpr int k = KI(K);
        const unsigned off = *reinterpret_cast<const unsigned short*>(reinterpret_cast<const char*>(TAB) + k * 128 + lane_tab);
        return *reinterpret_cast<const double*>(reinterpret_cast<const char*>(S) + off);
    };
#ifdef LIW_QUAD_TILE_ALIAS
    double* ST = S + S_IMU + w * PIFS + PIF_IJ + 100;
#else
    double* ST = S + S_TR + w * 90;
#endif

    double d[15], o[15], rr[15], cd[15], crt[6], D0[6], hA[6];
    double g0 = 0.0, gm = 0.0, ytg = 0.0, pdiag = 0.0, gsum = 0.0, gsh = 0.0;
    bool solved = true;
    sfor<0, 15>([&](auto R) { constexpr int r = KI(R); cd[r] = 0.0; });
    sfor<0, 6>([&](auto R) { D0[KI(R)] = 0.0; crt[KI(R)] = 0.0; hA[KI(R)] = 0.0; });
    const bool clk_on = g_qclk_on[0] && (int)blockIdx.x == g_qclk_on[1] && iteration == g_qclk_on[3];
    const int clk_frame = g_qclk_on[2];
    if (clk_k) g_qclk[13] = clock64();
    prefetch(n - 1);
    double sci_carry = (j_ < 15) ? LMD[oSC + (unsigned)((n - 1) * 15 + (j_ < 15 ? j_ : 0))] : 1.0;
    for (int i = n - 1; i >= 0; --i) {
        QSTAMP(0);
        int j = j_;
        asm volatile("" : "+v"(j));
        const int jc = j < 15 ? j : 0, j6 = j < 6 ? j : 0;
        const bool l6 = j < 6, l15 = j == 15, lm = j < 15;
        const bool hasm = i >= 1;
        asm volatile("s_waitcnt vmcnt(0)" ::: "memory");
        QSTAMP(1);
        const double sci = sci_carry, scm = scm_n, dg_old = dg_n, xq = xq_n;
        sci_carry = scm;
        const unsigned long long m15 = l15 ? ~0ull : 0ull, mh = hasm ? ~0ull : 0ull;
        double tS[6], oW[6], rL[6];
        {
            constexpr int NT = K_D - K_A;
            unsigned of[NT + 15], ofR[6];
            auto tab_at = [&](int k) { return (unsigned)*reinterpret_cast<const unsigned short*>(reinterpret_cast<const char*>(TAB) + k * 128 + lane_tab); };
            sfor<0, NT>([&](auto Q) { constexpr int q = KI(Q); of[q] = tab_at(K_A + q); });
            sfor<0, 6>([&](auto Q) { constexpr int q = KI(Q); ofR[q] = tab_at(K_RL + q); });
            if (n > 1) sfor<0, 15>([&](auto Q) { constexpr int q = KI(Q); of[NT + q] = tab_at(K_D + q); });
            const char* const Sb = reinterpret_cast<const char*>(S);
            const int w8 = (lane >> 4) * 8;
            const char* const bOV = Sb + (l15 ? 8 * (S_IMU + PIF_GJ) : 8 * (S_IMU + PIF_IJ) + jc * 120) + w8 * PIFS;
            const char* const bGI = Sb + (l15 ? 8 * (S_IMU + PIF_GI) + w8 * PIFS : 8 * S_ZERO);
            const char* const bOW = Sb + (l6 ? 8 * (S_PW + PW_IJ(0, 0)) + w8 * PWS + j6 * 48 : 8 * S_ZERO);
            double gi[15];
            if (n > 1) {
                sfor<0, 15>([&](auto R) { constexpr int r = KI(R); o[r] = *reinterpret_cast<const double*>(bOV + 8 * r); gi[r] = *reinterpret_cast<const double*>(bGI + 8 * r); });
            } else {
                sfor<0, 15>([&](auto R) { constexpr int r = KI(R); d[r] = 0.0; o[r] = 0.0; gi[r] = 0.0; });
            }
            sfor<0, 6>([&](auto R) { constexpr int r = KI(R); oW[r] = *reinterpret_cast<const double*>(bOW + 8 * r); });
            asm volatile("" ::: "memory");
            double pb[NT];
            sfor<0, NT>([&](auto Q) { constexpr int q = KI(Q); pb[q] = *reinterpret_cast<const double*>(Sb + of[q]); });
            sfor<0, 6>([&](auto R) { constexpr int r = KI(R); rL[r] = *reinterpret_cast<const double*>(Sb + ofR[r]); });
            if (n > 1) sfor<0, 15>([&](auto Q) { constexpr int q = KI(Q); d[q] = *reinterpret_cast<const double*>(Sb + of[NT + q]); });
            asm volatile("" ::: "memory");
            pb[K_A + 0] = flip_sign(pb[K_A + 0], sgA0); pb[K_A + 1] = flip_sign(pb[K_A + 1], sgA0);
            pb[K_A + 3] = flip_sign(pb[K_A + 3], sgA3); pb[K_A + 4] = flip_sign(pb[K_A + 4], sgA3); pb[K_A + 5] = flip_sign(pb[K_A + 5], sgA3);
            rL[0] = flip_sign(rL[0], sgR0); rL[1] = flip_sign(rL[1], sgR0);
            sfor<0, 6>([&](auto R) { constexpr int r = KI(R); tS[r] = pb[K_A + r] + bits_and(pb[K_B + r], mh) + pb[K_C + r]; });
            if (!track) {
                sfor<0, 6>([&](auto R) { constexpr int r = KI(R); hA[r] += pb[K_HA + r]; });
                if (i == 0) sfor<0, 6>([&](auto R) { tS[KI(R)] += hA[KI(R)]; });
            }
            sfor<0, 15>([&](auto R) { constexpr int r = KI(R); o[r] = bits_and(o[r], mh) + gi[r]; });
        }
        sfor<0, 15>([&](auto R) { rr[KI(R)] = 0.0; });
        sfor<0, 6>([&](auto R) {
            constexpr int r = KI(R);
            d[r] += bits_and(tS[r], ~m15);
            o[r] += bits_and(tS[r], m15) + bits_and(oW[r], mh);
            rr[r] = bits_and(rL[r], mh);
        });
        if (track && i == n - 2 && __any(prior_row)) {
            double Jc[15];
            const double dxl = (lm && prior_row) ? X[oX + (unsigned)((n - 2) * 15 + jc)] - a.prior_X[(size_t)b * 15 + jc] : 0.0;
            sfor<0, 15>([&](auto K) { constexpr int k = KI(K); Jc[k] = (lm && prior_row) ? a.prior_J[(size_t)b * 225 + k * 15 + jc] : 0.0; });
            double gp = 0.0;
            sfor<0, 15>([&](auto K) { constexpr int k = KI(K); const double rp = row_sum(Jc[k] * dxl); gp = __builtin_fma(Jc[k], rp, gp); });
            dpp_fence();
            sfor<0, 15>([&](auto R) {
                constexpr int r = KI(R);
                sfor<0, 15>([&](auto K) { constexpr int k = KI(K); fnma_bc<r>(d[r], Jc[k], -Jc[k]); });
                const double gr = bc<r>(gp);
                o[r] += l15 ? gr : 0.0;
            });
        }
        QSTAMP(2);
        QSTAMP(3);
        {
            double* GT = const_cast<double*>(SI) + PIF_IJ;
            if (l15) sfor<0, 15>([&](auto R) { constexpr int r = KI(R); GT[r] = o[r]; });
            const double gt = gsh + (lm ? GT[jc] : 0.0);
            double m = fabs(gt);
            {
                const double av = xq - gt;
                const double a2 = mul_nop(av, av);
                const double s2 = bc<3>(a2) + bc<4>(a2) + bc<5>(a2);
                if (__any(proceed && !(s2 < 9.8))) {
                    dpp_fence();
                    const V3<double> nq = normalize_so3(V3<double>(bc<3>(av), bc<4>(av), bc<5>(av)));
                    if (j == 3) m = fabs(xq - nq.x);
                    if (j == 4) m = fabs(xq - nq.y);
                    if (j == 5) m = fabs(xq - nq.z);
                }
            }
            if (!lm || is_const(i, j)) m = 0.0;
            gm = fmax(gm, m);
            gsum += lm ? gt : 0.0;
        }
        double dmp;
        {
            double mjj = d[0];
            sfor<1, 15>([&](auto R) { constexpr int r = KI(R); mjj = (j == r) ? d[r] : mjj; });
            double dgv = dg_old;
            if (!reuse) {
                dgv = fmin(fmax(__builtin_fma(mjj, sci * sci, pdiag), kMinDiag), kMaxDiag);
                if (proceed && lm) LMD[oDG + (unsigned)(i * 15 + j)] = dgv;
            }
            dmp = dgv * inv_radius;
        }
        QSTAMP(4);
        dpp_fence();
        const double* const stp = (l6 && i < n - 1) ? ST + j6 : S + S_ZERO;
        sfor<0, 15>([&](auto R) {
            constexpr int r = KI(R);
            const double rs = bc<r>(sci);
            d[r] = __builtin_fma(d[r], rs * sci, cd[r]) + ((j == r) ? dmp : 0.0);
            o[r] = __builtin_fma(o[r], rs * scm, bits_and(cd[r], m15));
            rr[r] = __builtin_fma(rr[r], rs * sc0, stp[r * 6]);
        });
        if (i == 1) {
            sfor<0, 15>([&](auto R) { constexpr int r = KI(R); o[r] += rr[r]; rr[r] = 0.0; });
        }
        if (i == 0) {
            dpp_fence();
            sfor<0, 6>([&](auto R) {
                constexpr int r = KI(R);
                const double gr = bc<r>(g0);
                d[r] += D0[r];
                o[r] += l15 ? gr : 0.0;
            });
        }
        if (track) {
            const bool colc = lm && is_const(i, j);
            const bool nbc = lm && hasm && is_const(i - 1, j);
            sfor<0, 15>([&](auto R) {
                constexpr int r = KI(R);
                const bool rowc = is_const(i, r);
                if (rowc || colc) d[r] = (j == r) ? 1.0 : 0.0;
                if (rowc || nbc) o[r] = 0.0;
                if (rowc) rr[r] = 0.0;
            });
        }
        QSTAMP(5);
        if (hasm) {
            dpp_fence();
            double cw[6];
            sfor<0, 6>([&](auto R) { constexpr int r = KI(R); cw[r] = RD(KC<K_CW + r>{}); });
            gsh = RD(KC<K_GSH>{});
            __builtin_amdgcn_sched_barrier(0);
            sfor<0, 15>([&](auto R) {
                constexpr int r = KI(R);
                double fi = 0.0;
                if constexpr (r < 6) {
                    const double rs = bc<r>(scm);
                    fi = cw[r] * (rs * scm);
                }
                cd[r] = fi;
                pdiag = (j == r) ? cd[r] : pdiag;
            });
        } else {
            gsh = 0.0;
        }
        sfor<0, 6>([&](auto Q) { crt[KI(Q)] = 0.0; });
        if (i >= 1) prefetch(i - 1);
        QSTAMP(6);
        sfor<0, 15>([&](auto K) {
            constexpr int k = KI(K);
            const double piv = bc<k>(d[k]);
            if (k == 14) solved = solved && (piv > 0.0) && isfinite(piv);
            const double inv = fast_rsqrt(piv);
            const double wkd = mul_nop(d[k], inv);
            const double wko = o[k] * inv, wkr = rr[k] * inv;
            d[k] = l15 ? inv : wkd;
            o[k] = wko; rr[k] = wkr;
            sfor<k + 1, 15>([&](auto R) {
                constexpr int r = KI(R);
                fnma_bc<r>(d[r], wkd, wkd);
                fnma_bc<r>(o[r], wkd, wko);
                fnma_bc<r>(rr[r], wkd, wkr);
            });
        });
        QSTAMP(7);
        sfor<0, 15>([&](auto K) { constexpr int k = KI(K); ytg = __builtin_fma(o[k], o[k], ytg); });
        if (hasm) {
            dpp_fence();
            sfor<0, 15>([&](auto K) {
                constexpr int k = KI(K);
                sfor<0, 15>([&](auto C) { constexpr int c = KI(C); fnma_bc<c>(cd[c], o[k], o[k]); });
            });
            if (i >= 2) {
                sfor<0, 15>([&](auto K) {
                    constexpr int k = KI(K);
                    sfor<0, 6>([&](auto Q) { constexpr int q = KI(Q); fnma_bc<q>(crt[q], rr[k], o[k]); });
                    sfor<0, 6>([&](auto C) { constexpr int c = KI(C); fnma_bc<c>(D0[c], rr[k], rr[k]); });
                    fnma_bc<15>(g0, o[k], rr[k]);
                });
            }
            if (lm) sfor<0, 6>([&](auto Q) { constexpr int q = KI(Q); ST[jc * 6 + q] = crt[q]; });
        }
        QSTAMP(8);
        dpp_fence();
// ... 135 lines not shown
        }
    };
    sfor<0, BSD2>([&](auto Q) { constexpr int q = KI(Q); if (q < n) stage2(q, q); });
    for (int i0 = 0; i0 < n; i0 += BSD2) {
        sfor<0, BSD2>([&](auto Q) {
            constexpr int q = KI(Q);
            __builtin_amdgcn_sched_barrier(0);
            const int i = i0 + q;
            if (i < n) {
                const int later = min(n - 1 - i, BSD2 - 1);
                if (later >= 2) asm volatile("s_waitcnt vmcnt(%0)" ::"n"(2 * NLD) : "memory");
                else if (later == 1) asm volatile("s_waitcnt vmcnt(%0)" ::"n"(NLD) : "memory");
                else asm volatile("s_waitcnt vmcnt(0)" ::: "memory");
                solve_frame(q, i);
                if (i + BSD2 < n) stage2(i + BSD2, q);
            }
        });
    }
    if (clk_k) g_qclk[15] = clock64();
    const double step_norm = sqrt(row_sum(sn2));
    const double model_cost_change = 0.5 * (ytg + row_sum(dsum));
    const bool valid = solved && model_cost_change > 0.0 && isfinite(model_cost_change);
    const int invalid0 = st.invalid_steps, successful = st.successful;
    const bool fail5 = !valid && invalid0 + 1 >= 5;
    if (proceed && fail5 && successful > 0) {
        for (int e = j; e < n * 15; e += 16) X[oX + (unsigned)e] = LMD[oLM + LM_X0 + (unsigned)e];
    }
    if (proceed && j == 0) {
        const double radius = st.radius, dec = st.decrease_factor;
        st.iteration = iteration + 1;
        if (fail5 && successful > 0) st.x_cost = st.initial_cost;
        if (valid) {
            st.reuse_diagonal = 1;
            st.model_cost_change = model_cost_change; st.cand_step_norm = step_norm; st.have_candidate = 1; st.invalid_steps = 0;
        } else {
            st.invalid_steps = invalid0 + 1;
            st.have_candidate = 0;
            if (fail5) { st.done = 1; st.termination = 6; st.iteration = iteration; }
            st.radius = radius / dec; st.decrease_factor = dec * 2.0; st.reuse_diagonal = 1;
        }
    }
}

bool lm_step_quad_fits(const StepArgs& a) {
    const unsigned long long lim = 0xFFFFFFFFull - 4096;
    auto span = [&](const double* p0, const double* p1, unsigned long long per) {
        const unsigned long long d = p1 >= p0 ? (unsigned long long)(p1 - p0) : ~0ull;
        return d <= lim && d + (unsigned long long)a.B * per <= lim;
    };
    const int nm = a.n > 1 ? a.n - 1 : 1;
    return a.n >= 1 && (a.mode == LIW_MODE_INIT || (a.mode == LIW_MODE_TRACK && a.n >= 2)) && span(a.w.PL[0], a.w.PL[1], (unsigned long long)a.n * LPC) && a.w.pi_frame && a.w.pl_compact &&
           a.w.PL[0] >= a.w.PW[0] && span(a.w.PW[0], a.w.PL[1], (unsigned long long)a.n * LPC) &&
           a.w.CS[0] && a.w.CS[1] && span(a.w.PI[0], a.w.PI[1], (unsigned long long)a.n * PIFS) &&
           span(a.w.PW[0], a.w.PW[1], (unsigned long long)nm * PWS) && span(a.w.PG[0], a.w.PG[1], (unsigned long long)a.n * PGS) &&
           a.w.PG[0] >= a.w.PW[0] && span(a.w.PW[0], a.w.PG[1], (unsigned long long)a.n * PGS) &&
           (unsigned long long)a.B * (sizeof(LmState) / 8) <= lim && (unsigned long long)a.B * a.n * SOLVE_WS <= lim;
}
extern "C" void liw_debug_quad_clk(int on, int block, int frame, int iteration, long long* out) {
    const int v[4] = {on, block, frame, iteration};
    (void)hipMemcpyToSymbol(HIP_SYMBOL(g_qclk_on), v, sizeof(v));
    if (out) (void)hipMemcpyFromSymbol(out, HIP_SYMBOL(g_qclk), sizeof(long long) * 64);
}
void launch_lm_step_quad(const StepArgs& a, hipStream_t s) {
    static const int probe = [] { const char* e = getenv("LIW_QUAD_PROBE"); const int v = e ? atoi(e) : 0; if (v) (void)hipMemcpyToSymbol(HIP_SYMBOL(g_qprobe), &v, sizeof(v)); return v; }();
    (void)probe;
    hipLaunchKernelGGL(k_lm_step_quad, dim3((a.B + 3) / 4), dim3(64), 0, s, a);
}

}
```

2dliw-slam_amd/csrc/liw_capi.hip:

```cpp
#include <hip/hip_runtime.h>

#include <algorithm>
#include <cmath>
#include <cstdio>
#include <cstdlib>
#include <atomic>
#include <chrono>
#include <cstring>
#include <string>
#include <vector>

#include "liw_kernels.hpp"

using namespace liw;

struct DevBuf {
    void* p = nullptr;
    size_t cap = 0;
    int ensure(size_t bytes) {
        if (bytes <= cap && p) return 0;
        if (p) (void)hipFree(p);
        p = nullptr; cap = 0;
        if (hipMalloc(&p, bytes ? bytes : 8) != hipSuccess) return -1;
        cap = bytes ? bytes : 8;
// ... 145 lines not shown
            }
        }
    }
    if (!c->have_device && c->err.empty()) c->err = "no HIP device";
    return c;
}

void liw_destroy(liw_ctx* c) {
    if (!c) return;
    if (c->have_device) {
        (void)hipSetDevice(c->prm.device);
        DevBuf* bufs[] = {&c->lpk, &c->lpk_off, &c->lpk_mx, &c->lpk_perm, &c->p2p_err, &c->arena, &c->prior_X, &c->prior_J, &c->prior_R, &c->has_prior, &c->ws, &c->scratch,
                          &c->priorn_X, &c->priorn_J, &c->priorn_R, &c->has_priorn, &c->result, &c->marg_status};
        if (c->pinned) (void)hipHostFree(c->pinned);
        if (c->rb_pin) (void)hipHostFree(c->rb_pin);
        if (c->ev_upload) (void)hipEventDestroy(c->ev_upload);
        for (DevBuf* b : bufs) b->release();
        for (auto e : c->ev_lin) (void)hipEventDestroy(e);
        for (auto e : c->ev_step) (void)hipEventDestroy(e);
        for (auto e : c->ev_x) (void)hipEventDestroy(e);
        if (c->gexec) (void)hipGraphExecDestroy(c->gexec);
        if (c->have_fork) {
            (void)hipStreamDestroy(c->fork.side[0]); (void)hipStreamDestroy(c->fork.side[1]);
            (void)hipEventDestroy(c->fork.ev_fork); (void)hipEventDestroy(c->fork.ev_join[0]); (void)hipEventDestroy(c->fork.ev_join[1]); (void)hipEventDestroy(c->fork.ev_compact);
        }
        if (c->stream) (void)hipStreamDestroy(c->stream);
    }
    delete c;
}

const char* liw_last_error(const liw_ctx* c) { return c ? c->err.c_str() : "null ctx"; }

int liw_get_extrinsics(const liw_ctx* c, double* A, double* Bm) {
    if (!c) return LIW_EINVAL;
    auto put = [](const double* R, const double* t, double* m) {
        for (int i = 0; i < 3; ++i) { for (int j = 0; j < 3; ++j) m[i * 4 + j] = R[i * 3 + j]; m[i * 4 + 3] = t[i]; }
        m[12] = m[13] = m[14] = 0.0; m[15] = 1.0;
    };
    if (A) put(c->dp.Riw, c->dp.tiw, A);
    if (Bm) put(c->dp.Ril, c->dp.til, Bm);
    return LIW_OK;
}

static size_t al256(size_t v) { return (v + 255) & ~(size_t)255; }
struct FullLayout {
    size_t PL[2], PI[2], PW[2], PG[2], CS[2], x_cand, group_off, lm, solve_ws, info, history, active, imu_pk, imu_pk_bad, bytes;
};
static FullLayout full_layout(int B, int n, int hist) {
    FullLayout f{};
    size_t o = 0;
    const int nm = n > 1 ? n - 1 : 1;
    const int lps = laser_stride(pi_frame_format(B) ? 1 : 0);
    for (int k = 0; k < 2; ++k) { f.PI[k] = o; o = al256(o + sizeof(double) * (size_t)B * pi_doubles_per_window(n)); }
    for (int k = 0; k < 2; ++k) { f.PW[k] = o; o = al256(o + sizeof(double) * (size_t)B * nm * PWS); }
    for (int k = 0; k < 2; ++k) { f.PL[k] = o; o = al256(o + sizeof(double) * (size_t)B * n * lps); }
    for (int k = 0; k < 2; ++k) { f.PG[k] = o; o = al256(o + sizeof(double) * (size_t)B * n * PGS); }
    f.x_cand = o; o = al256(o + sizeof(double) * (size_t)B * n * 15);
    f.group_off = o; o = al256(o + sizeof(int) * (size_t)B * (n + 1));
    f.active = o; o = al256(o + compact_list_bytes_host(B));
    f.lm = o; o = al256(o + sizeof(LmState) * (size_t)B);
    f.solve_ws = o; o = al256(o + sizeof(double) * (size_t)B * n * SOLVE_WS);
    f.info = o; o = al256(o + sizeof(liw_summary) * (size_t)B);
    f.history = hist > 0 ? o : 0;
    if (hist > 0) o = al256(o + sizeof(double) * (size_t)hist * B * n * 15);
    f.imu_pk_bad = o; o = al256(o + 2 * sizeof(int));
    f.imu_pk = o; o = al256(o + sizeof(double) * (size_t)B * nm * IMU_PK);
    for (int k = 0; k < 2; ++k) { f.CS[k] = o; o = al256(o + sizeof(double) * (size_t)B * 4 * n); }
    f.bytes = o;
    return f;
}
static WsView make_view(void* ws, int B, int n, int hist) {
    FullLayout f = full_layout(B, n, hist);
    char* base = (char*)ws;
    WsView v{};
    for (int k = 0; k < 2; ++k) {
        v.PL[k] = (double*)(base + f.PL[k]); v.PI[k] = (double*)(base + f.PI[k]);
        v.PW[k] = (double*)(base + f.PW[k]); v.PG[k] = (double*)(base + f.PG[k]);
    }
    v.x_cand = (double*)(base + f.x_cand);
    v.group_off = (int*)(base + f.group_off);
    v.lm = (LmState*)(base + f.lm);
    v.solve_ws = (double*)(base + f.solve_ws);
    v.info = (liw_summary*)(base + f.info);
    v.history = hist > 0 ? (double*)(base + f.history) : nullptr;
    v.history_records = hist;
    v.active = (int*)(base + f.active);
    v.pi_frame = pi_frame_format(B) ? 1 : 0;
    v.pl_compact = v.pi_frame;
    for (int k = 0; k < 2; ++k) v.CS[k] = (double*)(base + f.CS[k]);
    v.imu_pk = (double*)(base + f.imu_pk);
    v.imu_pk_bad = (int*)(base + f.imu_pk_bad);
    return v;
}

int liw_batch_ws_layout(int B, int n, int history_records, liw_ws_layout* out) {
    if (!out || B <= 0 || n <= 0 || n > 64) return LIW_EINVAL;
    FullLayout f = full_layout(B, n, history_records);
    out->bytes = f.bytes;
    out->laser_partial_off[0] = f.PL[0];
    out->laser_partial_off[1] = f.PL[1];
    out->laser_partial_stride = laser_stride(pi_frame_format(B) ? 1 : 0);
    out->laser_partial_bytes = sizeof(double) * (size_t)B * n * out->laser_partial_stride;
    out->info_off = f.info;
    out->history_off = f.history;
    return LIW_OK;
}

static int check_batch(liw_ctx* c, const liw_batch* b, int min_n = 1) {
    if (!b || b->B <= 0 || b->n <= 0 || b->n > 64) return fail(c, LIW_EINVAL, "bad batch (need 1 <= n <= 64, B >= 1)");
    if (b->n < min_n) return fail(c, LIW_EINVAL, "TRACK / MARG topology needs n >= 2 (the prior block is tied to frame n-2)");
    return LIW_OK;
}
static int min_frames(int mode) { return mode == LIW_MODE_INIT ? 1 : 2; }
static bool lpk_matches(const liw_ctx* c, const liw_batch* b, const void* ws) {
    return c && c->lpk_on && c->lpk_key.ws == ws && c->lpk_key.pts == b->laser_pts && c->lpk_key.frame == b->laser_frame && c->lpk_key.B == b->B &&
           c->lpk_key.n == b->n && c->lpk_key.Ltot == (long)b->Ltot;
}
static int laser_slab_begin(liw_ctx* c, const liw_batch* b, int mode, const WsView& v, void* ws, hipStream_t s, bool may_sync) {
    c->lpk_on = false;
    if (!may_sync || std::getenv("LIW_NO_LASER_SLAB")) return LIW_OK;
    const int S = laser_slab_count(b->B), N = S * b->n;
    if ((mode == LIW_MODE_INIT ? N < 2048 : S < 256) || b->Ltot <= 0) return LIW_OK;
    if (c->lpk_mx.ensure(sizeof(int) * (size_t)N) || c->lpk_off.ensure(sizeof(long long) * ((size_t)N + 2)) || c->lpk_perm.ensure(sizeof(int) * (size_t)N * 64))
        return fail(c, LIW_ENOMEM, "hipMalloc");
    launch_laser_slab_prepare(b->B, b->n, v.group_off, c->lpk_perm.as<int>(), c->lpk_mx.as<int>(), c->lpk_off.as<long long>(), v.imu_pk_bad + 1, s);
    if (!c->rb_pin) HIPCHK(c, hipHostMalloc((void**)&c->rb_pin, 64, hipHostMallocDefault));
    long long* const tail = reinterpret_cast<long long*>(c->rb_pin) + 2;
    tail[0] = 0; tail[1] = 1;
    HIPCHK(c, hipMemcpyAsync(tail, c->lpk_off.as<long long>() + N, 2 * sizeof(long long), hipMemcpyDeviceToHost, s));
    HIPCHK(c, hipStreamSynchronize(s));
    const long long rows = tail[0];
    if (tail[1] != 0 || rows <= 0) return LIW_OK;
    if (rows * 64 > 4 * (long long)b->Ltot + 64ll * N) return LIW_OK;
    if (c->lpk.ensure(sizeof(double) * LASER_SLAB_ROWD * (size_t)rows)) { c->lpk.release(); return LIW_OK; }
    launch_laser_slab_pack(b->B, b->n, (long)b->Ltot, v.group_off, c->lpk_perm.as<int>(), b->laser_pts, c->lpk_off.as<long long>(), c->lpk_mx.as<int>(), c->lpk.as<double>(), s);
    c->lpk_key = {ws, b->laser_pts, b->laser_frame, b->B, b->n, (long)b->Ltot};
    c->lpk_on = true;
    c->lpk_rows = rows;
    return LIW_OK;
}
static LinArgs lin_args(const liw_batch* b, int mode, const double* x, const WsView& v, int candidate, bool use_lm, bool packed = false, const liw_ctx* c = nullptr, const void* ws = nullptr) {
    LinArgs A{};
    A.B = b->B; A.n = b->n; A.mode = mode; A.eval_small = b->eval_small;
    A.x = x; A.group_off = v.group_off; A.laser_off = b->laser_off; A.laser_pts = b->laser_pts; A.Ltot = b->Ltot;
    A.match_pose = b->match_pose; A.has_match = b->has_match;
    A.imu_X = b->imu_X; A.imu_J = b->imu_J; A.imu_sqrtP = b->imu_sqrtP; A.imu_Dt = b->imu_Dt;
    A.wheel_T = b->wheel_T; A.wheel_sqrtP = b->wheel_sqrtP;
    for (int k = 0; k < 2; ++k) { A.PL[k] = v.PL[k]; A.PI[k] = v.PI[k]; A.PW[k] = v.PW[k]; A.PG[k] = v.PG[k]; }
    A.lm = use_lm ? v.lm : nullptr;
    A.active = use_lm ? v.active : nullptr;
    A.candidate = candidate;
    A.pi_frame = v.pi_frame;
    A.pl_compact = v.pl_compact;
    for (int k = 0; k < 2; ++k) A.CS[k] = v.pi_frame ? v.CS[k] : nullptr;
    if (packed && b->n > 1 && b->eval_small) { A.imu_pk = v.imu_pk; A.imu_pk_bad = v.imu_pk_bad; }
    if (packed) A.laser_hz = v.imu_pk_bad + 1;
    if (packed && lpk_matches(c, b, ws)) { A.laser_pk = c->lpk.as<double>(); A.laser_slab_off = c->lpk_off.as<long long>(); A.laser_perm = c->lpk_perm.as<int>(); }
    return A;
}
static StepArgs step_args(liw_ctx* c, const liw_batch* b, int mode, int max_iters, const WsView& v) {
    StepArgs a{};
    a.B = b->B; a.n = b->n; a.mode = mode; a.max_iters = max_iters; a.fast_mode = c->prm.fast_mode;
    a.x = b->x; a.match_pose = b->match_pose; a.has_match = b->has_match;
    a.prior_X = b->prior_X; a.prior_J = b->prior_J; a.has_prior = b->has_prior;
    a.w = v;
    a.use_active = lin_builds_active_list(b->B, b->eval_small) ? 1 : 0;
    return a;
}
static int resolve_iters(liw_ctx* c, int mode, int max_iters) {
    if (max_iters > 0) return max_iters;
    return (mode == LIW_MODE_TRACK && c->prm.fast_mode) ? 10 : 50;
}


int liw_batch_lm_begin(liw_ctx* c, const liw_batch* b, int mode, int max_iters, void* ws, void* stream) {
    NEEDDEV(c);
    if (int r = check_batch(c, b, min_frames(mode))) return r;
    c->last_iters = resolve_iters(c, mode, max_iters);
    WsView v = make_view(ws, b->B, b->n, b->history_records);
    hipStream_t s = (hipStream_t)stream;
    launch_group_offsets(b->B, b->n, b->laser_off, b->laser_frame, v.group_off, s);
    launch_lm_begin(b->B, b->n, v.lm, c->last_iters, s);
    (void)hipMemsetAsync(v.active + b->B + 1, 0, compact_list_bytes_host(b->B) - sizeof(int) * ((size_t)b->B + 1), s);
    if (b->n > 1 && b->eval_small) {
        if ((long)b->B * (b->n - 1) >= 4096 && !std::getenv("LIW_NO_IMU_PACK"))
            launch_imu_pack(b->B, b->n, b->imu_X, b->imu_J, b->imu_sqrtP, b->imu_Dt, v.imu_pk, v.imu_pk_bad, s);
        else (void)hipMemsetAsync(v.imu_pk_bad, 0xff, sizeof(int), s);
    }
    if ((long)b->B * (b->n - 1) >= 4096) {
        launch_laser_z_scan(b->Ltot, b->laser_pts, v.imu_pk_bad + 1, s);
        hipStreamCaptureStatus cap = hipStreamCaptureStatusNone;
        (void)hipStreamIsCapturing(s, &cap);
        if (int r = laser_slab_begin(c, b, mode, v, ws, s, cap == hipStreamCaptureStatusNone)) return r;
    } else {
        (void)hipMemsetAsync(v.imu_pk_bad + 1, 0xff, sizeof(int), s);
        c->lpk_on = false;
    }
    HIPCHK(c, hipGetLastError());
    return LIW_OK;
}
int liw_batch_launch_paths(liw_ctx* c, const liw_batch* b, const void* ws, int* flags) {
    if (!c) return LIW_EINVAL;
    if (int r = check_batch(c, b)) return r;
    if (!flags) return fail(c, LIW_EINVAL, "liw_batch_launch_paths: null flags");
    *flags = (pi_frame_format(b->B) ? 1 : 0) | (lpk_matches(c, b, ws) ? 2 : 0);
    return LIW_OK;
}
int liw_batch_packed_rows(liw_ctx* c, const liw_batch* b, const void* ws, long long* rows, long long* blocks) {
    if (!c) return LIW_EINVAL;
    if (int r = check_batch(c, b)) return r;
    if (rows) *rows = lpk_matches(c, b, ws) ? c->lpk_rows : 0;
    if (blocks) *blocks = (long long)b->Ltot;
    return LIW_OK;
}
int liw_batch_lm_linearize(liw_ctx* c, const liw_batch* b, int mode, int candidate, void* ws, void* stream) {
    NEEDDEV(c);
    if (int r = check_batch(c, b, min_frames(mode))) return r;
    WsView v = make_view(ws, b->B, b->n, b->history_records);
    LinArgs A = lin_args(b, mode, candidate ? v.x_cand : b->x, v, candidate != 0, true, true, c, ws);
    launch_linearize(A, c->dp, (hipStream_t)stream, c->have_fork ? &c->fork : nullptr);
    HIPCHK(c, hipGetLastError());
    return LIW_OK;
}
int liw_batch_lm_linearize_async(liw_ctx* c, const liw_batch* b, int mode, int candidate, void* ws, void* stream) {
    NEEDDEV(c);
    if (int r = check_batch(c, b, min_frames(mode))) return r;
    WsView v = make_view(ws, b->B, b->n, b->history_records);
    LinArgs A = lin_args(b, mode, candidate ? v.x_cand : b->x, v, candidate != 0, true, true, c, ws);
    launch_linearize(A, c->dp, (hipStream_t)stream, c->have_fork ? &c->fork : nullptr, true);
    HIPCHK(c, hipGetLastError());
    return LIW_OK;
}
int liw_batch_lm_join(liw_ctx* c, void* stream) {
    NEEDDEV(c);
    launch_linearize_join((hipStream_t)stream, c->have_fork ? &c->fork : nullptr);
    HIPCHK(c, hipGetLastError());
    return LIW_OK;
}
int liw_batch_exchange_doubles(int B, int n, int mode) {
    if (B <= 0 || n <= 0 || n > 64) return LIW_EINVAL;
    return B * n * (mode == LIW_MODE_INIT ? 45 : 21) + 1;
}
int liw_batch_exchange_pack(liw_ctx* c, const liw_batch* b, int mode, int candidate, void* ws, double* buf, void* stream) {
    NEEDDEV(c);
    if (int r = check_batch(c, b, min_frames(mode))) return r;
    if (!buf) return fail(c, LIW_EINVAL, "liw_batch_exchange_pack: null buffer");
    WsView v = make_view(ws, b->B, b->n, b->history_records);
    launch_exchange_pack(b->B, b->n, mode == LIW_MODE_INIT, v.pl_compact, v.PL[0], v.PL[1], candidate, mode == LIW_MODE_MARG ? nullptr : v.lm, buf, (hipStream_t)stream);
    HIPCHK(c, hipGetLastError());
    return LIW_OK;
}
int liw_batch_exchange_unpack(liw_ctx* c, const liw_batch* b, int mode, int candidate, void* ws, const double* buf, int copies, void* stream) {
    NEEDDEV(c);
    if (int r = check_batch(c, b, min_frames(mode))) return r;
    if (!buf || copies < 1) return fail(c, LIW_EINVAL, "liw_batch_exchange_unpack: null buffer / copies < 1");
    WsView v = make_view(ws, b->B, b->n, b->history_records);
    const size_t stride = (size_t)liw_batch_exchange_doubles(b->B, b->n, mode);
    launch_exchange_unpack(b->B, b->n, mode == LIW_MODE_INIT, v.pl_compact, copies, stride, buf, v.PL[0], v.PL[1], v.pi_frame ? v.CS[0] : nullptr, v.pi_frame ? v.CS[1] : nullptr, candidate, mode == LIW_MODE_MARG ? nullptr : v.lm, (hipStream_t)stream);
    HIPCHK(c, hipGetLastError());
    return LIW_OK;
}
int liw_batch_laser_records(liw_ctx* c, const liw_batch* b, int mode, int buffer, void* ws, double* out, void* stream) {
    NEEDDEV(c);
    if (int r = check_batch(c, b, min_frames(mode))) return r;
    if (!out || buffer < 0 || buffer > 1) return fail(c, LIW_EINVAL, "liw_batch_laser_records: null output / buffer not 0 or 1");
    WsView v = make_view(ws, b->B, b->n, b->history_records);
    launch_laser_expand(b->B, b->n, mode == LIW_MODE_INIT, v.pl_compact, v.PL[buffer], out, (hipStream_t)stream);
    HIPCHK(c, hipGetLastError());
    return LIW_OK;
}
static hipEvent_t next_event(std::vector<hipEvent_t>& pool, size_t& used);
int liw_batch_solve_sharded(liw_ctx* c, const liw_batch* b, int mode, int max_iters, void* ws, void* stream,
                            double* xbuf, double* xall, int world, liw_exchange_fn exchange, void* user) {
    NEEDDEV(c);
    if (int r = check_batch(c, b, min_frames(mode))) return r;
    if (mode != LIW_MODE_INIT && mode != LIW_MODE_TRACK) return fail(c, LIW_EINVAL, "liw_batch_solve_sharded: mode must be INIT or TRACK");
    const bool p2p = exchange == nullptr && c->p2p_world > 0;
    if (!xbuf || (!exchange && !p2p) || world < 1) return fail(c, LIW_EINVAL, "liw_batch_solve_sharded: exchange buffer / callback (or liw_batch_p2p_setup) / world");
    if (p2p && world != c->p2p_world) return fail(c, LIW_EINVAL, "liw_batch_solve_sharded: world differs from liw_batch_p2p_setup");
    const int K = resolve_iters(c, mode, max_iters);
    const size_t nd = (size_t)liw_batch_exchange_doubles(b->B, b->n, mode);
    hipStream_t s = (hipStream_t)stream;
    c->xev_used = 0;
    auto lin_exchange = [&](int cand) -> int {
        if (int r = liw_batch_lm_linearize_async(c, b, mode, cand, ws, stream)) return r;
        if (c->time_exchange) (void)hipEventRecord(next_event(c->ev_x, c->xev_used), s);
        if (int r = liw_batch_exchange_pack(c, b, mode, cand, ws, xbuf, stream)) return r;
        if (p2p) {
            const unsigned long long e = ++c->p2p_epoch;
            launch_p2p_exchange(nd, xbuf, c->p2p, c->p2p_rank, world, e, c->p2p_err.as<int>(), s);
            c->last_x = c->p2p.area[c->p2p_rank] + (size_t)(e & 1ull) * world * nd;
            c->last_x_copies = world;
            WsView v = make_view(ws, b->B, b->n, b->history_records);
            launch_exchange_unpack(b->B, b->n, mode == LIW_MODE_INIT, v.pl_compact, world, nd, c->last_x, v.PL[0], v.PL[1], v.pi_frame ? v.CS[0] : nullptr, v.pi_frame ? v.CS[1] : nullptr, cand, v.lm, s, true);
            HIPCHK(c, hipGetLastError());
            if (c->time_exchange) (void)hipEventRecord(next_event(c->ev_x, c->xev_used), s);
            return liw_batch_lm_join(c, stream);
        }
        const int copies = exchange(user, xbuf, xall, nd, stream);
        if (copies != 1 && !(copies == world && xall)) return fail(c, LIW_EINVAL, "liw_batch_solve_sharded: the exchange callback must return 1 (sum in buf) or world (images in all)");
        c->last_x = copies == 1 ? xbuf : xall;
        c->last_x_copies = copies;
        if (int r = liw_batch_exchange_unpack(c, b, mode, cand, ws, c->last_x, copies, stream)) return r;
        if (c->time_exchange) (void)hipEventRecord(next_event(c->ev_x, c->xev_used), s);
        return liw_batch_lm_join(c, stream);
    };
    auto p2p_failed = [&]() -> int {
        int e = 0;
        HIPCHK(c, hipMemcpyAsync(&e, c->p2p_err.p, sizeof(int), hipMemcpyDeviceToHost, s));
        HIPCHK(c, hipStreamSynchronize(s));
        if (e) return fail(c, LIW_EHIP, "peer-write exchange: a peer's flag never arrived (rank in p2p status)");
// ... 702 lines not shown
```

2dliw-slam_amd/csrc/liw_kernels.hpp:

```cpp
#pragma once
#include <cstdlib>
#include <hip/hip_runtime.h>
#include <stdint.h>

#include "../../include/liw_window.h"
#include "liw_dual.hpp"

namespace liw {

struct DevParams {
    double Riw[9], tiw[3];
    double Ril[9], til[3];
    double g;
    double laser_sqrt_info;
    double ground_p_info;
    double ground_q_info;
    int fast_mode;
};

constexpr int LP = LIW_LASER_PARTIAL;
constexpr int PIS = 496;
constexpr int PI_II = 0, PI_IJ = 120, PI_JJ = 345, PI_G = 465, PI_C = 495;
__host__ __device__ inline int pi_tri(int r, int c) {
    const int lo = r < c ? r : c, hi = r < c ? c : r;
    return lo * 15 - (lo * (lo - 1)) / 2 + (hi - lo);
}
constexpr int PIF_D = 0, PIF_IJ = 120, PIF_GJ = 345, PIF_GI = 360, PIF_C = 375, PIFS = 376;
constexpr int QUAD_MIN_BATCH = 1024;
inline bool pi_frame_format(int B) {
    const char* env = getenv("LIW_STEP_VARIANT");
    return env ? env[0] == '3' : B >= QUAD_MIN_BATCH;
}
__host__ __device__ inline size_t pi_doubles_per_window(int n) {
    const size_t a = (size_t)(n > 1 ? n - 1 : 1) * PIS, b = (size_t)n * PIFS;
    return a > b ? a : b;
}
template <int N> __host__ __device__ constexpr int tri_sym(int r, int c) {
    return r <= c ? r * N - (r * (r - 1)) / 2 + (c - r) : c * N - (c * (c - 1)) / 2 + (r - c);
}
constexpr int CS_LASER = 0, CS_GROUND = 1, CS_IMU = 2, CS_WHEEL = 3;
__host__ __device__ inline size_t cs_index(int n, int b, int role, int rec) { return ((size_t)b * 4 + role) * n + rec; }
constexpr int PWS = 92;
__host__ __device__ constexpr int PW_II(int r, int c) { return tri_sym<6>(r, c); }
__host__ __device__ constexpr int PW_IJ(int r, int c) { return 21 + r * 6 + c; }
__host__ __device__ constexpr int PW_JJ(int r, int c) { return 57 + tri_sym<6>(r, c); }
__host__ __device__ constexpr int PW_G(int e) { return 78 + e; }
constexpr int PW_C = 90;
constexpr int PGS = 28;
__host__ __device__ constexpr int PG_H(int r, int c) { return tri_sym<7>(r, c); }
__host__ __device__ constexpr int PG_G(int r) { return tri_sym<7>(r, 6); }
constexpr int PG_C = 27;
constexpr int FTF = 32;

struct LmState {
    double radius, decrease_factor, x_cost, x_norm, minimum_cost;
    double cand_step_norm, model_cost_change;
    int reuse_diagonal, iteration, done, termination, successful, cur, invalid_steps, have_candidate;
    int max_iters, pad_;
    double initial_cost;
    double scale[15 * 64];
    double diagonal[15 * 64];
    double x0[15 * 64];
};

__device__ __forceinline__ void lm_reset(LmState& s, int max_iters) {
    s.radius = 1e4; s.decrease_factor = 2.0; s.x_cost = 0.0; s.x_norm = 0.0; s.minimum_cost = 0.0;
    s.cand_step_norm = 0.0; s.model_cost_change = 0.0; s.reuse_diagonal = 0; s.iteration = 0; s.done = 0; s.termination = 0;
    s.successful = 0; s.cur = 0; s.invalid_steps = 0; s.have_candidate = 0; s.initial_cost = 0.0; s.max_iters = max_iters; s.pad_ = 0;
}

struct WsView {
    double* PL[2]; double* PI[2]; double* PW[2]; double* PG[2];
    double* x_cand;
    int* group_off;
    LmState* lm;
    double* solve_ws;
    liw_summary* info;
    double* history;
    int history_records;
    int* active;
    int pi_frame;
    int pl_compact;
    double* CS[2];
    double* imu_pk;
    int* imu_pk_bad;
};
constexpr int IMU_PK = 192, IPK_DT = 15, IPK_J = 16, IPK_S = 70;
constexpr int REC_LD = 22;
constexpr int REC_GS = 15 * REC_LD;
constexpr int SOLVE_WS = REC_GS + 16;

struct LinArgs {
    int B, n, mode, eval_small;
    const double* x;
    const int* group_off;
    const int* laser_off;
    const double* laser_pts; int Ltot;
    const double* match_pose;
    const unsigned char* has_match;
    const double* imu_X; const double* imu_J; const double* imu_sqrtP; const double* imu_Dt;
    const double* wheel_T; const double* wheel_sqrtP;
    double* PL[2]; double* PI[2]; double* PW[2]; double* PG[2];
    const LmState* lm;
    const LmState* gate;
    LmState* reset_lm;
    int reset_iters;
    int marg_older;
    int candidate;
    int small_per_wave;
    int imu_per_wave;
    int small_nd;
    int* active;
    int pi_frame;
    int pl_compact;
    double* CS[2];
    const double* imu_pk;
    const int* imu_pk_bad;
    const int* laser_hz;
    const double* laser_pk;
    const long long* laser_slab_off;
    const int* laser_perm;
    int role_mask;
    double* dbg_laser_res; double* dbg_laser_jac; double* dbg_imu_res; double* dbg_imu_jac;
    double* dbg_wheel_res; double* dbg_wheel_jac; double* dbg_ground_res; double* dbg_ground_jac;
};

template <bool BOTH> constexpr int laser_pairidx(int c1, int c2) {
    constexpr int NC = BOTH ? 9 : 6;
    return c1 > c2 ? laser_pairidx<BOTH>(c2, c1) : c1 * NC - c1 * (c1 - 1) / 2 + (c2 - c1);
}
constexpr int laser_col_a(int idx) { return idx < 2 ? idx : (idx == 2 ? -1 : idx - 1); }
template <bool BOTH> constexpr int laser_col_b(int idx) { return BOTH ? (idx < 2 ? idx : (idx == 2 ? -1 : idx + 2)) : (idx == 2 ? -1 : (idx < 2 ? idx : idx - 1)); }
template <bool BOTH> constexpr bool laser_neg_b(int idx) { return BOTH && idx < 2; }
template <bool BOTH>
__host__ __device__ constexpr int laser_slot_code(int s) {
    constexpr int RC = (BOTH ? 9 : 6) - 1;
    int src = -1;
    bool neg = false;
    if (s < 0) {
    } else if (s < 36) {
        const int ca = laser_col_a(s / 6), cb = laser_col_a(s % 6);
        if (BOTH && ca >= 0 && cb >= 0) src = laser_pairidx<BOTH>(ca, cb);
    } else if (s < 72) {
        const int ia = (s - 36) / 6, ib = (s - 36) % 6, ca = laser_col_b<BOTH>(ia), cb = laser_col_b<BOTH>(ib);
        if (ca >= 0 && cb >= 0) { src = laser_pairidx<BOTH>(ca, cb); neg = laser_neg_b<BOTH>(ia) != laser_neg_b<BOTH>(ib); }
    } else if (s < 108) {
        const int ia = (s - 72) / 6, ib = (s - 72) % 6, ca = laser_col_a(ia), cb = laser_col_b<BOTH>(ib);
        if (BOTH && ca >= 0 && cb >= 0) { src = laser_pairidx<BOTH>(ca, cb); neg = laser_neg_b<BOTH>(ib); }
    } else if (s < 114) {
        const int ca = laser_col_a(s - 108);
        if (BOTH && ca >= 0) src = laser_pairidx<BOTH>(ca, RC);
    } else if (s < 120) {
        const int cb = laser_col_b<BOTH>(s - 114);
        if (cb >= 0) { src = laser_pairidx<BOTH>(cb, RC); neg = laser_neg_b<BOTH>(s - 114); }
    } else if (s == 120) {
        src = laser_pairidx<BOTH>(RC, RC);
    }
    return src < 0 ? -1 : (src | (neg ? 64 : 0));
}
template <bool BOTH> __host__ __device__ constexpr bool laser_slot_zero(int s) { return laser_slot_code<BOTH>(s) < 0; }
constexpr int LPC = LIW_LASER_PARTIAL_COMPACT;
__host__ __device__ constexpr int laser_stride(int compact) { return compact ? LPC : LP; }
constexpr int LPC_COST_BOTH = laser_pairidx<true>(8, 8), LPC_COST_ONE = laser_pairidx<false>(5, 5);
static_assert(laser_slot_code<true>(120) == LPC_COST_BOTH && laser_slot_code<false>(120) == LPC_COST_ONE && LPC_COST_BOTH == 44 && LPC_COST_ONE == 20, "cost total");
template <bool BOTH> __host__ __device__ inline double laser_slot(const double* rec, int s, int compact) {
    if (!compact) return rec[s];
    const int code = laser_slot_code<BOTH>(s);
// ... 74 lines not shown
    int use_active;
};
struct ExportArgs {
    int B, n, mode, fast_mode, buf;
    const double* x; const double* prior_X; const double* prior_J; const int* has_prior;
    WsView w;
    double* H; double* g; double* cost;
};
struct MargArgs {
    int B, n;
    const double* x; double* prior_X; double* prior_J; double* prior_R; int* has_prior;
    WsView w;
    double* sqrt_H; double* Delta_H; double* Delta_g; int* status;
    double* out_X; double* out_J; double* out_R; int* out_has;
    const LmState* gate;
    int use_cur;
};
constexpr int LIW_RESULT_HDR = 8;
struct PackArgs {
    int n, mode;
    const LmState* lm; liw_summary* info; const double* x; double* match_pose; const unsigned char* has_match;
    const double* marg; const int* marg_status;
    double* out;
    int seq;
};
void launch_linearize(const LinArgs& A, const DevParams& P, hipStream_t s, const LinFork* fk, bool defer_join = false);
void launch_linearize_join(hipStream_t s, const LinFork* fk);
void launch_exchange_pack(int B, int n, bool both, int compact, const double* PL0, const double* PL1, int candidate, const LmState* lm, double* buf, hipStream_t s);
void launch_exchange_unpack(int B, int n, bool both, int compact, int world, size_t stride, const double* buf, double* PL0, double* PL1, double* CS0, double* CS1, int candidate, const LmState* lm, hipStream_t s, bool sysload = false);
constexpr int P2P_MAX = 16;
struct P2pPeers { double* area[P2P_MAX]; unsigned long long* flags[P2P_MAX]; };
void launch_p2p_exchange(size_t nd, const double* buf, const P2pPeers& peers, int rank, int world, unsigned long long epoch, int* err, hipStream_t s);
void launch_group_offsets(int B, int n, const int* laser_off, const int* laser_frame, int* group_off, hipStream_t s);
void launch_laser_z_scan(long Ltot, const double* laser_pts, int* flag, hipStream_t s);
__host__ __device__ inline int laser_slab_count(int B) { return (B + 63) / 64; }
void launch_laser_slab_prepare(int B, int n, const int* group_off, int* perm, int* mx, long long* off, const int* hz, hipStream_t s);
#ifndef LIW_SLAB_WPLANE
#define LIW_SLAB_WPLANE 0
#endif
constexpr int LASER_SLAB_ROWD = (8 + LIW_SLAB_WPLANE) * 64;
void launch_laser_slab_pack(int B, int n, long Ltot, const int* group_off, const int* perm, const double* pts, const long long* off, const int* mx, double* pk, hipStream_t s);
void launch_lin_laser_slab(const LinArgs& A, const DevParams& P, hipStream_t s);
void launch_imu_pack(int B, int n, const double* imu_X, const double* imu_J, const double* imu_sqrtP, const double* imu_Dt, double* pk, int* bad, hipStream_t s);
void launch_pack_result(const PackArgs& a, hipStream_t s);
void launch_lm_begin(int B, int n, LmState* lm, int max_iters, hipStream_t s);
void launch_lm_step(const StepArgs& a, hipStream_t s);
void launch_lm_step_quad(const StepArgs& a, hipStream_t s);
bool lm_step_quad_fits(const StepArgs& a);
size_t compact_list_bytes_host(int B);
bool lin_builds_active_list(int B, int eval_small);
void launch_lm_finish(const StepArgs& a, hipStream_t s);
void launch_export_dense(const ExportArgs& a, hipStream_t s);
void launch_laser_expand(int B, int n, bool both, int compact, const double* PL, double* out, hipStream_t s);
void launch_marg_schur(const MargArgs& a, hipStream_t s);

struct PreintNoise { double q_na[3], q_nw[3], q_nba[3], q_nbw[3], wheel_cov[3]; };
void launch_preint_imu(int M, const int* sample_off, const double* samples, const double* t_start, const double* t_end, const double* bias6,
                       const PreintNoise& N, double* X, double* J, double* Pscratch, double* sqrtP, double* Dt, hipStream_t s);
void launch_preint_wheel(int M, const int* sample_off, const double* samples, const double* t_start, const double* t_end,
                         const PreintNoise& N, double* T12, double* sq9, double* Dt, hipStream_t s);

}
```

include/liw_window.h:

```cpp
#ifndef LIW_WINDOW_H
#define LIW_WINDOW_H
#include <stddef.h>
#include <stdint.h>

#ifdef __cplusplus
extern "C" {
#endif

#define LIW_OK 0
#define LIW_EINVAL (-22)
#define LIW_ENOMEM (-12)
#define LIW_ENODEV (-19)
#define LIW_EHIP (-5)
#define LIW_ESTATE (-1)

enum { LIW_MODE_INIT = 0, LIW_MODE_TRACK = 1, LIW_MODE_MARG = 2 };

typedef struct liw_params {
    double T_imu_to_wheel[16];
    double T_imu_to_laser[16];
    double g;
    double line_to_line_sigma;
    double manifold_p_sigma, manifold_q_sigma;
    double imu_noise_acc_sigma[3], imu_bias_acc_sigma[3], imu_noise_gyro_sigma[3], imu_bias_gyro_sigma[3];
// ... 26 lines not shown
    int termination;
    double initial_cost, final_cost;
} liw_summary;

typedef struct liw_ctx liw_ctx;

liw_ctx* liw_create(const liw_params* prm);
void liw_destroy(liw_ctx* ctx);
const char* liw_last_error(const liw_ctx* ctx);
int liw_get_extrinsics(const liw_ctx* ctx, double* T_imu_to_wheel16, double* T_imu_to_laser16);

int liw_set_window(liw_ctx* ctx, const liw_window* w);
int liw_clear_window(liw_ctx* ctx);
int liw_solve(liw_ctx* ctx, int mode, int max_iters, liw_summary* summary);
int liw_get_history(liw_ctx* ctx, double* x, int max_records);
int liw_linearize(liw_ctx* ctx, int mode, double* H, double* g, double* cost);
int liw_eval_factors(liw_ctx* ctx, int mode, double* laser_res, double* laser_jac, double* imu_res, double* imu_jac,
                     double* wheel_res, double* wheel_jac, double* ground_res, double* ground_jac);
int liw_marginalize(liw_ctx* ctx, double* sqrt_H36, double* Delta_H225, double* Delta_g15);
int liw_get_prior(liw_ctx* ctx, double* X15, double* J225, double* R15);
int liw_set_prior(liw_ctx* ctx, int has_prior, const double* X15, const double* J225, const double* R15);

typedef struct liw_batch {
    int B;
    int n;
    int Ltot;
    double* x;
    const int* laser_off;
    const int* laser_frame;
    const double* laser_pts;
    double* match_pose;
    const unsigned char* has_match;
    const double* imu_X;
    const double* imu_J;
    const double* imu_sqrtP;
    const double* imu_Dt;
    const double* wheel_T;
    const double* wheel_sqrtP;
    double* prior_X;
    double* prior_J;
    double* prior_R;
    int* has_prior;
    int eval_small;
    int history_records;
} liw_batch;

typedef struct liw_ws_layout {
    size_t bytes;
    size_t laser_partial_off[2];
    size_t laser_partial_bytes;
    size_t info_off;
    size_t history_off;
    int laser_partial_stride;
} liw_ws_layout;
#define LIW_LASER_PARTIAL 128
#define LIW_LASER_PARTIAL_COMPACT 48
int liw_batch_ws_layout(int B, int n, int history_records, liw_ws_layout* out);

int liw_batch_set_max_iters(liw_ctx* ctx, int mode, int max_iters);
int liw_batch_linearize(liw_ctx* ctx, const liw_batch* b, int mode, void* ws, void* stream);
int liw_batch_time_kernels(liw_ctx* ctx, const liw_batch* b, int mode, void* ws, void* stream, int reps, double* out_ms);
int liw_batch_lm_begin(liw_ctx* ctx, const liw_batch* b, int mode, int max_iters, void* ws, void* stream);
int liw_batch_launch_paths(liw_ctx* ctx, const liw_batch* b, const void* ws, int* flags);
int liw_batch_packed_rows(liw_ctx* ctx, const liw_batch* b, const void* ws, long long* rows, long long* blocks);
int liw_batch_lm_linearize(liw_ctx* ctx, const liw_batch* b, int mode, int candidate, void* ws, void* stream);
int liw_batch_laser_records(liw_ctx* ctx, const liw_batch* b, int mode, int buffer, void* ws, double* out, void* stream);
int liw_batch_lm_step(liw_ctx* ctx, const liw_batch* b, int mode, void* ws, void* stream);
int liw_batch_lm_finish(liw_ctx* ctx, const liw_batch* b, int mode, void* ws, void* stream);
int liw_batch_lm_linearize_async(liw_ctx* ctx, const liw_batch* b, int mode, int candidate, void* ws, void* stream);
int liw_batch_lm_join(liw_ctx* ctx, void* stream);
typedef int (*liw_exchange_fn)(void* user, double* buf, double* all, size_t doubles, void* stream);
int liw_batch_solve_sharded(liw_ctx* ctx, const liw_batch* b, int mode, int max_iters, void* ws, void* stream,
                            double* xbuf, double* xall, int world, liw_exchange_fn exchange, void* user);
size_t liw_batch_p2p_area_doubles(int B, int n, int mode, int world);
int liw_batch_p2p_setup(liw_ctx* ctx, int rank, int world, double* const* areas, unsigned long long* const* flags);
int liw_batch_p2p_status(liw_ctx* ctx, int* timed_out_rank_plus_1);
int liw_batch_exchange_timing(liw_ctx* ctx, int enable, double* avg_ms, int* count);
int liw_batch_exchange_doubles(int B, int n, int mode);
int liw_batch_exchange_pack(liw_ctx* ctx, const liw_batch* b, int mode, int candidate, void* ws, double* buf, void* stream);
int liw_batch_exchange_unpack(liw_ctx* ctx, const liw_batch* b, int mode, int candidate, void* ws, const double* buf, int copies, void* stream);
int liw_batch_solve(liw_ctx* ctx, const liw_batch* b, int mode, int max_iters, void* ws, void* stream, int use_graph);
int liw_batch_marg_linearize(liw_ctx* ctx, const liw_batch* b, void* ws, void* stream);
int liw_batch_marg_schur(liw_ctx* ctx, const liw_batch* b, void* ws, double* sqrt_H, double* Delta_H, double* Delta_g, void* stream);
int liw_batch_export_dense(liw_ctx* ctx, const liw_batch* b, int mode, int buf, void* ws, double* H, double* g, double* cost, void* stream);
int liw_set_timing(liw_ctx* ctx, int enable);
int liw_get_timing(liw_ctx* ctx, double* linearize_ms_avg, int* linearize_launches, double* step_ms_avg, int* step_launches);

int liw_batch_imu_preint(liw_ctx* ctx, int M, const int* sample_off, const double* samples, const double* t_start, const double* t_end,
                         const double* bias6, double* X, double* J, double* P_scratch, double* sqrt_inverse_P, double* Dt, void* stream);
int liw_batch_wheel_preint(liw_ctx* ctx, int M, const int* sample_off, const double* samples, const double* t_start, const double* t_end,
                           double* delta_Tij, double* sqrt_inverse_P, double* Dt, void* stream);

typedef struct liw_imu_preint liw_imu_preint;
liw_imu_preint* liw_imu_preint_create(const liw_params* prm);
void liw_imu_preint_destroy(liw_imu_preint* p);
void liw_imu_preint_reset(liw_imu_preint* p, double time, const double* acc_bias3, const double* gyr_bias3);
int liw_imu_preint_add(liw_imu_preint* p, double time_stamp, const double* acc3, const double* gyro3);
void liw_imu_preint_update_only_t(liw_imu_preint* p, double time);
double liw_imu_preint_Dt(const liw_imu_preint* p);
void liw_imu_preint_result(const liw_imu_preint* p, double* X15, double* J225, double* sqrt_inverse_P225, double* Dt);

typedef struct liw_wheel_preint liw_wheel_preint;
liw_wheel_preint* liw_wheel_preint_create(const liw_params* prm);
void liw_wheel_preint_destroy(liw_wheel_preint* p);
void liw_wheel_preint_reset(liw_wheel_preint* p, double time);
int liw_wheel_preint_add(liw_wheel_preint* p, double time_stamp, const double* pose_R9, const double* pose_t3);
void liw_wheel_preint_update_only_t(liw_wheel_preint* p, double time);
void liw_wheel_preint_result(const liw_wheel_preint* p, double* T12, double* sqrt_inverse_P9, double* Dt);

#ifdef __cplusplus
}
#endif
#endif
```

Measured before the change: 141,100 solves/s.

## Store compact wheel and ground factor records and rebuild Gram entries on read

Wheel and ground linearization now writes compact per-factor Jacobian/residual rows (40 and 14 doubles) instead of expanded upper-triangular Hessian records. The LM assembly, cost and diagonal readers recompute each Hessian entry on the fly as a small dot product. This cuts global store and load traffic per iteration in exchange for extra FMAs in the consumers. A debug expansion kernel and API keep the old record format available for inspection.

Result: no change. 140,400 solves/s (-0.5%).

```diff
diff --git a/2dliw-slam_amd/__init__.py b/2dliw-slam_amd/__init__.py
--- a/2dliw-slam_amd/__init__.py
+++ b/2dliw-slam_amd/__init__.py
@@ -53,13 +53,13 @@
 
 class WsLayoutC(C.Structure):
     _fields_ = [("bytes", C.c_size_t), ("laser_partial_off", C.c_size_t * 2), ("laser_partial_bytes", C.c_size_t),
-                ("info_off", C.c_size_t), ("history_off", C.c_size_t), ("laser_partial_stride", C.c_int)]
+                ("info_off", C.c_size_t), ("history_off", C.c_size_t), ("laser_partial_stride", C.c_int), ("cost_off", C.c_size_t * 2)]
 
 
 EXPORTS = [
     "liw_create", "liw_destroy", "liw_last_error", "liw_get_extrinsics", "liw_set_window", "liw_clear_window", "liw_solve", "liw_get_history",
     "liw_linearize", "liw_eval_factors", "liw_marginalize", "liw_get_prior", "liw_set_prior", "liw_batch_ws_layout",
-    "liw_batch_set_max_iters", "liw_batch_launch_paths", "liw_batch_packed_rows", "liw_batch_linearize", "liw_batch_time_kernels", "liw_batch_lm_begin", "liw_batch_lm_linearize", "liw_batch_laser_records", "liw_batch_lm_step",
+    "liw_batch_set_max_iters", "liw_batch_launch_paths", "liw_batch_packed_rows", "liw_batch_linearize", "liw_batch_time_kernels", "liw_batch_lm_begin", "liw_batch_lm_linearize", "liw_batch_laser_records", "liw_batch_small_records", "liw_batch_lm_step",
     "liw_batch_lm_finish", "liw_batch_lm_linearize_async", "liw_batch_lm_join", "liw_batch_exchange_doubles", "liw_batch_exchange_pack",
     "liw_batch_exchange_unpack", "liw_batch_solve_sharded", "liw_batch_exchange_timing", "liw_batch_p2p_area_doubles", "liw_batch_p2p_setup", "liw_batch_p2p_status", "liw_batch_solve", "liw_batch_marg_linearize", "liw_batch_marg_schur", "liw_batch_export_dense",
     "liw_set_timing", "liw_get_timing", "liw_batch_imu_preint", "liw_batch_wheel_preint", "liw_imu_preint_create", "liw_imu_preint_destroy", "liw_imu_preint_reset",
diff --git a/2dliw-slam_amd/batch.py b/2dliw-slam_amd/batch.py
--- a/2dliw-slam_amd/batch.py
+++ b/2dliw-slam_amd/batch.py
@@ -240,6 +240,25 @@
             out.append(o)
         return out
 
+    def _small_records(self):
+        nb = max(self.n - 1, 0)
+        out = []
+        for k in range(2):
+            pw = self.torch.zeros(self.B * nb * 92, dtype=self.torch.float64, device=self.dev)
+            pg = self.torch.zeros(self.B * self.n * 28, dtype=self.torch.float64, device=self.dev)
+            self._chk(self.L.liw_batch_small_records(self.h, C.byref(self.b), C.c_int(k), self._wsp(),
+                                                     C.c_void_p(pw.data_ptr() if nb else None), C.c_void_p(pg.data_ptr()), self._stream()))
+            out.append((pw, pg))
+        return out
+
+    @property
+    def PW(self):
+        return [r[0] for r in self._small_records()]
+
+    @property
+    def PG(self):
+        return [r[1] for r in self._small_records()]
+
     INPUT_KEYS = ("x", "laser_off", "laser_frame", "laser_pts", "match_pose", "has_match", "imu_X", "imu_J", "imu_sqrtP", "imu_Dt", "wheel_T", "wheel_sqrtP")
 
     def rebind(self, t, Ltot):
diff --git a/2dliw-slam_amd/csrc/k_linearize.hip b/2dliw-slam_amd/csrc/k_linearize.hip
--- a/2dliw-slam_amd/csrc/k_linearize.hip
+++ b/2dliw-slam_amd/csrc/k_linearize.hip
@@ -486,18 +486,7 @@
 struct WheelRcTab { int e[PWS]; };
 constexpr WheelRcTab make_wheel_rc() {
     WheelRcTab t{};
-    for (int e = 0; e < PWS; ++e) {
-        int r = 12, c = 12;
-        if (e < PW_IJ(0, 0) || (e >= PW_JJ(0, 0) && e < PW_G(0))) {
-            const int jj = e >= PW_JJ(0, 0);
-            int q = e - (jj ? PW_JJ(0, 0) : 0);
-            r = 0;
-            while (q >= 6 - r) { q -= 6 - r; ++r; }
-            c = r + q + (jj ? 6 : 0); r += jj ? 6 : 0;
-        } else if (e < PW_JJ(0, 0)) { r = (e - PW_IJ(0, 0)) / 6; c = 6 + (e - PW_IJ(0, 0)) % 6; }
-        else if (e < PW_C) { r = e - PW_G(0); c = 12; }
-        t.e[e] = e <= PW_C ? (r << 8) | c : -1;
-    }
+    for (int e = 0; e < PWS; ++e) t.e[e] = wheel_rc(e);
     return t;
 }
 __constant__ WheelRcTab c_wheel_rc = make_wheel_rc();
@@ -687,11 +676,7 @@
 struct GroundRcTab { int e[PGS]; };
 constexpr GroundRcTab make_ground_rc() {
     GroundRcTab t{};
-    for (int e = 0; e < PGS; ++e) {
-        int r = 0, c = e;
-        while (c >= 7 - r) { c -= 7 - r; ++r; }
-        t.e[e] = (r << 8) | (c + r);
-    }
+    for (int e = 0; e < PGS; ++e) t.e[e] = ground_rc(e);
     return t;
 }
 __constant__ GroundRcTab c_ground_rc = make_ground_rc();
@@ -736,7 +721,16 @@
         constexpr int LPF = PGS / 2;
         const int j = lane / LPF, pr = lane - j * LPF;
         const bool all_on = __builtin_amdgcn_ballot_w64(lane < nfr && meta[lane & 31] < 0) == 0;
-        if (j < 4) {
+        if (A.pw_compact) {
+            constexpr int LPC_ = PGC / 2;
+            const int jf = lane / LPC_, pc = lane - jf * LPC_;
+            if (jf < 9)
+                for (int q = jf; q < nfr; q += 9) {
+                    const int sel = meta[q], fq = meta[32 + q];
+                    const double2 v = reinterpret_cast<const double2*>(lds + q * 16)[pc];
+                    if (sel >= 0) nt_store<8>(reinterpret_cast<double2*>(&(sel ? A.PG[1] : A.PG[0])[(size_t)fq * PGC + 2 * pc]), v);
+                }
+        } else if (j < 4) {
             const int rc0 = c_ground_rc.e[2 * pr], rc1 = c_ground_rc.e[2 * pr + 1];
             const int r0 = rc0 >> 8, c0 = rc0 & 255, r1 = rc1 >> 8, c1 = rc1 & 255;
             auto frame = [&](int q) {
@@ -924,6 +918,38 @@
     const int ml = lane < WG_PER_WAVE ? lane : 0;
     const int selv = meta[ml], fkv = meta[32 + ml], csv = meta[64 + ml], fiv = meta[96 + ml], cgv = meta[128 + ml], kv = meta[160 + ml];
     const bool all_on = __builtin_amdgcn_ballot_w64(lane < nblk && selv < 0) == 0;
+    if (A.pw_compact) {
+        {
+            constexpr int LPB = PWC / 2;
+            const int jb = lane / LPB, pr = lane - jb * LPB;
+            if (jb < 3)
+                for (int q = jb; q < nblk; q += 3) {
+                    const int sel = meta[q], fq = meta[32 + q];
+                    const double* Yq = lds + q * WG_REC + 2 * pr;
+                    double2 v;
+                    v.x = Yq[0];
+                    v.y = 2 * pr + 1 < 39 ? Yq[1] : 0.0;
+                    if (sel >= 0) nt_store<8>(reinterpret_cast<double2*>(&(sel ? A.PW[1] : A.PW[0])[(size_t)fq * PWC + 2 * pr]), v);
+                }
+        }
+        {
+            constexpr int LPF = PGC / 2;
+            const int jf = lane / LPF, pr = lane - jf * LPF;
+            const bool any_k0 = __builtin_amdgcn_ballot_w64(lane < nblk && kv == 0) != 0;
+            if (jf < 9)
+                for (int pass = 0; pass < (any_k0 ? 2 : 1); ++pass) {
+                    const int yo = pass ? 53 : 39;
+                    for (int q = jf; q < nblk; q += 9) {
+                        const int sel = meta[q], fq = meta[96 + q] + (pass ? 0 : 1), kq = meta[160 + q];
+                        const double* Yq = lds + q * WG_REC + yo + 2 * pr;
+                        double2 v;
+                        v.x = Yq[0]; v.y = Yq[1];
+                        if (sel >= 0 && (pass == 0 || kq == 0))
+                            nt_store<8>(reinterpret_cast<double2*>(&(sel ? A.PG[1] : A.PG[0])[(size_t)fq * PGC + 2 * pr]), v);
+                    }
+                }
+        }
+    } else
     if (lane < PWS / 2) {
         const int rc0 = c_wheel_rc.e[2 * lane], rc1 = c_wheel_rc.e[2 * lane + 1];
         const int r0 = rc0 >> 8, c0 = rc0 & 255;
@@ -956,7 +982,7 @@
         constexpr int LPF = PGS / 2;
         const int j = lane / LPF, pr = lane - j * LPF;
         const bool any_k0 = __builtin_amdgcn_ballot_w64(lane < nblk && kv == 0) != 0;
-        if (j < 4) {
+        if (j < 4 && !A.pw_compact) {
             const int rc0 = c_ground_rc.e[2 * pr], rc1 = c_ground_rc.e[2 * pr + 1];
             const int r0 = rc0 >> 8, c0 = rc0 & 255, r1 = rc1 >> 8, c1 = rc1 & 255;
             for (int pass = 0; pass < (any_k0 ? 2 : 1); ++pass) {
@@ -1270,6 +1296,20 @@
     if (both) hipLaunchKernelGGL(k_laser_expand<true>, dim3(blocks), dim3(256), 0, s, groups, compact, PL, out);
     else hipLaunchKernelGGL(k_laser_expand<false>, dim3(blocks), dim3(256), 0, s, groups, compact, PL, out);
 }
+__global__ void k_small_expand(int B, int n, int compact, const double* PW, const double* PG, double* PW_out, double* PG_out) {
+    const size_t t = (size_t)blockIdx.x * blockDim.x + threadIdx.x;
+    const size_t nw = (size_t)B * (n - 1) * PWS, ng = (size_t)B * n * PGS;
+    if (t < nw) {
+        if (PW_out) PW_out[t] = wheel_slot(PW + (t / PWS) * wheel_stride(compact), (int)(t % PWS), compact);
+    } else if (t < nw + ng) {
+        const size_t u = t - nw;
+        if (PG_out) PG_out[u] = ground_slot(PG + (u / PGS) * ground_stride(compact), (int)(u % PGS), compact, (double)n);
+    }
+}
+void launch_small_expand(int B, int n, int compact, const double* PW, const double* PG, double* PW_out, double* PG_out, hipStream_t s) {
+    const size_t tot = (size_t)B * (n - 1) * PWS + (size_t)B * n * PGS;
+    hipLaunchKernelGGL(k_small_expand, dim3((unsigned)((tot + 255) / 256)), dim3(256), 0, s, B, n, compact, PW, PG, PW_out, PG_out);
+}
 __global__ void k_count_active(int B, const LmState* lm, double* out) {
     __shared__ int cnt;
     if (threadIdx.x == 0) cnt = 0;
diff --git a/2dliw-slam_amd/csrc/k_lm.hip b/2dliw-slam_amd/csrc/k_lm.hip
--- a/2dliw-slam_amd/csrc/k_lm.hip
+++ b/2dliw-slam_amd/csrc/k_lm.hip
@@ -31,6 +31,7 @@
     int n, mode, fast, b, buf;
     int pif;
     int plc;
+    int pwc;
     const double* PL; const double* PI; const double* PW; const double* PG;
     const double* x;
     const double* pJ; const double* pX; bool prior_on;
@@ -44,6 +45,8 @@
 }
 
 __device__ __forceinline__ double pl_slot(const AsmCtx& c, const double* rec, int s) { return laser_slot(rec, s, c.plc, c.mode == LIW_MODE_INIT); }
+__device__ __forceinline__ double pw_slot(const AsmCtx& c, const double* rec, int e, int r, int cc) { return c.pwc ? wheel_pair(rec, r, cc) : rec[(unsigned)e]; }
+__device__ __forceinline__ double pg_slot(const AsmCtx& c, const double* rec, int e, int r, int cc) { return c.pwc ? ground_pair(rec, r, cc, (double)c.n) : rec[(unsigned)e]; }
 
 struct FrameExtra { double sc_i, sc_m, dg_i, x_i; };
 
@@ -85,16 +88,17 @@
     const bool pif = c.pif != 0;
     const bool hasm = i >= 1, hasp = i <= n - 2;
     const double* PIb = c.PI + (size_t)c.b * (pif ? (size_t)n * PIFS : (size_t)(n - 1) * PIS);
-    const double* PWb = c.PW + (size_t)c.b * (n - 1) * PWS;
-    const double* PGb = c.PG + (size_t)c.b * n * PGS;
+    const int WST = wheel_stride(c.pwc), GST = ground_stride(c.pwc);
+    const double* PWb = c.PW + (size_t)c.b * (n - 1) * WST;
+    const double* PGb = c.PG + (size_t)c.b * n * GST;
     const double* PIm = pif ? PIb + (size_t)i * PIFS : PIb + (size_t)(hasm ? i - 1 : 0) * PIS;
     const double* PIp = pif ? PIb + (size_t)(hasp ? i + 1 : i) * PIFS : PIb + (size_t)(hasp ? i : 0) * PIS;
     const int oJJ = pif ? PIF_D : PI_JJ, oIJ = pif ? PIF_IJ : PI_IJ;
-    const double* PWm = PWb + (size_t)(hasm ? i - 1 : 0) * PWS;
-    const double* PWp = PWb + (size_t)(hasp ? i : 0) * PWS;
+    const double* PWm = PWb + (size_t)(hasm ? i - 1 : 0) * WST;
+    const double* PWp = PWb + (size_t)(hasp ? i : 0) * WST;
     const double* PLi = PLb + (size_t)i * LPS;
     const double* PL1 = PLb + (size_t)(n > 1 ? 1 : 0) * LPS;
-    const double* PGi = PGb + (size_t)i * PGS;
+    const double* PGi = PGb + (size_t)i * GST;
     AsmRegs R;
 #pragma unroll
     for (int q = 0; q < 4; ++q) {
@@ -110,20 +114,20 @@
         const bool pl = lane < 36;
         const int r = pl ? lane / 6 : 0, cc = pl ? lane % 6 : 0;
         R.t1 = pl_slot(c, PLi, 36 + r * 6 + cc);
-        R.t2 = PWm[(unsigned)PW_JJ(r, cc)];
-        R.t3 = PWp[(unsigned)PW_II(r, cc)];
-        R.t4 = PGi[(unsigned)PG_H(r, cc)];
-        R.t8 = up ? PWp[(unsigned)PW_IJ(cc, r)] : PWm[(unsigned)PW_IJ(r, cc)];
-        R.e2 = up ? PWm[(unsigned)PW_IJ(r, cc)] : 0.0;
+        R.t2 = pw_slot(c, PWm, PW_JJ(r, cc), 6 + r, 6 + cc);
+        R.t3 = pw_slot(c, PWp, PW_II(r, cc), r, cc);
+        R.t4 = pg_slot(c, PGi, PG_H(r, cc), r, cc);
+        R.t8 = up ? pw_slot(c, PWp, PW_IJ(cc, r), cc, 6 + r) : pw_slot(c, PWm, PW_IJ(r, cc), r, 6 + cc);
+        R.e2 = up ? pw_slot(c, PWm, PW_IJ(r, cc), r, 6 + cc) : 0.0;
         R.t9 = pl_slot(c, PL1, 72 + r * 6 + cc);
         R.t10 = pl_slot(c, PLi, 72 + r * 6 + cc);
     }
     {
         const int r = lane < 15 ? lane : 0, r6 = r < 6 ? r : 0;
         R.g1 = pl_slot(c, PLi, 114 + r6);
-        R.g2 = PWm[(unsigned)PW_G(6 + r6)];
-        R.g3 = PWp[(unsigned)PW_G(r6)];
-        R.g4 = PGi[(unsigned)PG_G(r6)];
+        R.g2 = pw_slot(c, PWm, PW_G(6 + r6), 6 + r6, 12);
+        R.g3 = pw_slot(c, PWp, PW_G(r6), r6, 12);
+        R.g4 = pg_slot(c, PGi, PG_G(r6), r6, 6);
         R.g5 = PIm[(unsigned)((pif ? PIF_GJ : PI_G + 15) + r)];
         R.g6 = pif ? PIm[(unsigned)(PIF_GI + r)] : PIp[(unsigned)(PI_G + r)];
     }
@@ -328,14 +332,15 @@
     const double* PLb = c.PL + (size_t)c.b * n * LPS;
     const bool pif = c.pif != 0;
     const double* PIb = c.PI + (size_t)c.b * (pif ? (size_t)n * PIFS : (size_t)(n - 1) * PIS);
-    const double* PWb = c.PW + (size_t)c.b * (n - 1) * PWS;
-    const double* PGb = c.PG + (size_t)c.b * n * PGS;
+    const int WST = wheel_stride(c.pwc), GST = ground_stride(c.pwc);
+    const double* PWb = c.PW + (size_t)c.b * (n - 1) * WST;
+    const double* PGb = c.PG + (size_t)c.b * n * GST;
     const bool track = c.mode == LIW_MODE_TRACK;
     double s = 0.0, gs = 0.0;
     for (int i = lane; i < n; i += 64) {
         const bool gon = !(track && i < n - 1);
         if (gon) s += pl_slot(c, PLb + (size_t)i * LPS, 120);
-        if (gon) s += PGb[(size_t)i * PGS + PG_C];
+        if (gon) s += pg_slot(c, PGb + (size_t)i * GST, PG_C, 6, 6);
         if (gchk) {
             if (gon) {
 #pragma unroll
@@ -343,21 +348,21 @@
             }
             if (gon) {
 #pragma unroll
-                for (int k = 0; k < 6; ++k) gs += PGb[(size_t)i * PGS + PG_G(k)];
+                for (int k = 0; k < 6; ++k) gs += pg_slot(c, PGb + (size_t)i * GST, PG_G(k), k, 6);
             }
         }
     }
     for (int k = lane; k < n - 1; k += 64) {
         s += pif ? PIb[(size_t)(k + 1) * PIFS + PIF_C] : PIb[(size_t)k * PIS + PI_C];
         const bool won = !(track && k < n - 2);
-        if (won) s += PWb[(size_t)k * PWS + PW_C];
+        if (won) s += pw_slot(c, PWb + (size_t)k * WST, PW_C, 12, 12);
         if (gchk) {
 #pragma unroll
             for (int e = 0; e < 30; ++e)
                 gs += pif ? (e < 15 ? PIb[(size_t)k * PIFS + PIF_GI + e] : PIb[(size_t)(k + 1) * PIFS + PIF_GJ + e - 15]) : PIb[(size_t)k * PIS + PI_G + e];
             if (won) {
 #pragma unroll
-                for (int e = 0; e < 12; ++e) gs += PWb[(size_t)k * PWS + PW_G(e)];
+                for (int e = 0; e < 12; ++e) gs += pw_slot(c, PWb + (size_t)k * WST, PW_G(e), e, 12);
             }
         }
     }
@@ -455,15 +460,16 @@
     const int LPS = laser_stride(c.plc);
     const double* PLb = c.PL + (size_t)c.b * n * LPS;
     const double* PIb = c.PI + (size_t)c.b * (c.pif ? (size_t)n * PIFS : (size_t)(n - 1) * PIS);
-    const double* PWb = c.PW + (size_t)c.b * (n - 1) * PWS;
-    const double* PGb = c.PG + (size_t)c.b * n * PGS;
+    const int WST = wheel_stride(c.pwc), GST = ground_stride(c.pwc);
+    const double* PWb = c.PW + (size_t)c.b * (n - 1) * WST;
+    const double* PGb = c.PG + (size_t)c.b * n * GST;
     double d = 0.0;
     if (r < 6) {
         d += pl_slot(c, PLb + (size_t)i * LPS, 36 + r * 7);
         if (i == 0) for (int j = 0; j < n; ++j) d += pl_slot(c, PLb + (size_t)j * LPS, r * 7);
-        if (i >= 1) d += PWb[(size_t)(i - 1) * PWS + PW_JJ(r, r)];
-        if (i <= n - 2) d += PWb[(size_t)i * PWS + PW_II(r, r)];
-        d += PGb[(size_t)i * PGS + PG_H(r, r)];
+        if (i >= 1) d += pw_slot(c, PWb + (size_t)(i - 1) * WST, PW_JJ(r, r), 6 + r, 6 + r);
+        if (i <= n - 2) d += pw_slot(c, PWb + (size_t)i * WST, PW_II(r, r), r, r);
+        d += pg_slot(c, PGb + (size_t)i * GST, PG_H(r, r), r, r);
     }
     if (c.pif) { if (n > 1) d += PIb[(size_t)i * PIFS + PIF_D + pi_tri(r, r)]; }
     else {
@@ -490,8 +496,8 @@
         for (int k = 0; k < 2; ++k) {
             v[4 * k + 0] = touch_lines(a.w.PL[k] + (size_t)b * n2 * laser_stride(a.w.pl_compact), sizeof(double) * n2 * laser_stride(a.w.pl_compact));
             v[4 * k + 1] = touch_lines(a.w.PI[k] + (size_t)b * (n2 - 1) * PIS, sizeof(double) * (n2 - 1) * PIS);
-            v[4 * k + 2] = touch_lines(a.w.PW[k] + (size_t)b * (n2 - 1) * PWS, sizeof(double) * (n2 - 1) * PWS);
-            v[4 * k + 3] = touch_lines(a.w.PG[k] + (size_t)b * n2 * PGS, sizeof(double) * n2 * PGS);
+            v[4 * k + 2] = touch_lines(a.w.PW[k] + (size_t)b * (n2 - 1) * wheel_stride(a.w.pw_compact), sizeof(double) * (n2 - 1) * wheel_stride(a.w.pw_compact));
+            v[4 * k + 3] = touch_lines(a.w.PG[k] + (size_t)b * n2 * ground_stride(a.w.pw_compact), sizeof(double) * n2 * ground_stride(a.w.pw_compact));
         }
         v[8] = touch_lines(a.x + (size_t)b * n2 * 15, sizeof(double) * n2 * 15);
         v[9] = touch_lines(a.w.x_cand + (size_t)b * n2 * 15, sizeof(double) * n2 * 15);
@@ -523,6 +529,7 @@
     AsmCtx c;
     c.pif = a.w.pi_frame;
     c.plc = a.w.pl_compact;
+    c.pwc = a.w.pw_compact;
     c.n = n; c.mode = a.mode; c.fast = a.fast_mode; c.b = b;
     c.pJ = a.prior_J + (size_t)b * 225; c.pX = a.prior_X + (size_t)b * 15;
     c.prior_on = a.mode == LIW_MODE_TRACK && a.has_prior[b] && !a.fast_mode;
@@ -1026,6 +1033,7 @@
     AsmCtx c;
     c.pif = a.w.pi_frame;
     c.plc = a.w.pl_compact;
+    c.pwc = a.w.pw_compact;
     c.n = n; c.mode = a.mode; c.fast = a.fast_mode; c.b = b;
     c.pJ = a.prior_J + (size_t)b * 225; c.pX = a.prior_X + (size_t)b * 15;
     c.prior_on = a.mode == LIW_MODE_TRACK && a.has_prior[b] && !a.fast_mode;
@@ -1500,6 +1508,7 @@
     AsmCtx c;
     c.pif = a.w.pi_frame;
     c.plc = a.w.pl_compact;
+    c.pwc = a.w.pw_compact;
     c.n = n; c.mode = a.mode; c.fast = a.fast_mode; c.b = b; c.buf = a.buf;
     c.PL = a.w.PL[0]; c.PI = a.w.PI[0]; c.PW = a.w.PW[0]; c.PG = a.w.PG[0];
     c.x = a.x + (size_t)b * n * 15;
@@ -1533,6 +1542,7 @@
     AsmCtx c;
     c.pif = a.w.pi_frame;
     c.plc = a.w.pl_compact;
+    c.pwc = a.w.pw_compact;
     const int sel = a.use_cur ? __builtin_amdgcn_readfirstlane(a.w.lm[b].cur) : 0;
     c.n = n; c.mode = LIW_MODE_MARG; c.fast = 0; c.b = b; c.buf = sel;
     c.PL = sel ? a.w.PL[1] : a.w.PL[0]; c.PI = sel ? a.w.PI[1] : a.w.PI[0]; c.PW = sel ? a.w.PW[1] : a.w.PW[0]; c.PG = sel ? a.w.PG[1] : a.w.PG[0];
diff --git a/2dliw-slam_amd/csrc/k_lm_quad.hip b/2dliw-slam_amd/csrc/k_lm_quad.hip
--- a/2dliw-slam_amd/csrc/k_lm_quad.hip
+++ b/2dliw-slam_amd/csrc/k_lm_quad.hip
@@ -50,11 +50,11 @@
 constexpr int QNT1 = (LIW_NT_MASK & 16) ? 2 : 0, QNT2 = (LIW_NT_MASK & 64) ? 2 : 0;
 constexpr int QTR = 4 * 15 * 6;
 #endif
-constexpr int K_A = 0, K_B = 6, K_C = 12, K_HA = 18, K_D = 24, K_CW = 39, K_GSH = 45, K_RL = 46, NRD = 52;
+constexpr int K_A = 0, K_HA = 6, K_D = 12, K_RL = 27, K_WJ = 33, K_WI = 34, K_GC = 35, NRD = 36;
 constexpr int QTAB = NRD * 16;
 constexpr int QZB = 86;
-constexpr int QPAD = 96;
-constexpr int QTOT_1 = 4 * (PIFS + LPC + PWS + PGS) + QPAD + QTR + QZB + QTAB;
+constexpr int QPAD = 104;
+constexpr int QTOT_1 = 4 * (PIFS + LPC + PWC + PGC) + QPAD + QTR + QZB + QTAB;
 constexpr int quad_laser_slot(int kind, int r, int j) {
     return kind == 0 ? (j == 15 ? 114 + r : 36 + r * 6 + j) : kind == 1 ? (j == 15 ? 108 + r : r * 6 + j) : 72 + j * 6 + r;
 }
@@ -250,8 +250,8 @@
     const unsigned bp = (g_qprobe & 1) ? 0u : (unsigned)b;
     const unsigned oPL = bp * (unsigned)(n * LPC) + (cur ? (unsigned)(a.w.PL[1] - a.w.PL[0]) : 0u);
     const unsigned oPI = bp * (unsigned)(n * PIFS) + (cur ? (unsigned)(a.w.PI[1] - a.w.PI[0]) : 0u);
-    const unsigned oPW = bp * (unsigned)((n - 1) * PWS) + (cur ? (unsigned)(a.w.PW[1] - a.w.PW[0]) : 0u);
-    const unsigned oPG = bp * (unsigned)(n * PGS) + (cur ? (unsigned)(a.w.PG[1] - a.w.PG[0]) : 0u);
+    const unsigned oPW = bp * (unsigned)((n - 1) * PWC) + (cur ? (unsigned)(a.w.PW[1] - a.w.PW[0]) : 0u);
+    const unsigned oPG = bp * (unsigned)(n * PGC) + (cur ? (unsigned)(a.w.PG[1] - a.w.PG[0]) : 0u);
     const int qprobe = g_qprobe;
     const unsigned oWS = (qprobe & 2) ? 0u : (unsigned)b * (unsigned)(n * SOLVE_WS);
     double* const WS = a.w.solve_ws;
@@ -265,18 +265,29 @@
         if (prior_row) for (int k = 0; k < 15; ++k) { const double v = a.prior_J[(size_t)b * 225 + k * 15 + jc]; sp += v * v; }
         const int cbb = track ? laser_slot_code<false>(36 + (l6 ? jc : 0) * 7) : laser_slot_code<true>(36 + (l6 ? jc : 0) * 7);
         const int caa = track ? laser_slot_code<false>((l6 ? jc : 0) * 7) : laser_slot_code<true>((l6 ? jc : 0) * 7);
+        const double gmult = (double)n;
         for (int i0 = 0; i0 < n; i0 += 4) {
             double vbb[4], vjj[4], vii[4], vg[4], vi[4];
+            double yj[4][3], yi[4][3], yg[4][2];
 #pragma unroll
             for (int u = 0; u < 4; ++u) {
                 const int i = min(i0 + u, n - 1);
                 const int j6 = l6 ? jc : 0;
                 vbb[u] = PL0[oPL + (unsigned)(i * LPC + (cbb >= 0 ? cbb & 63 : 0))];
                 vbb[u] = cbb >= 0 ? vbb[u] : 0.0;
-                vjj[u] = n > 1 ? PW0[oPW + (unsigned)(max(i - 1, 0) * PWS + PW_JJ(j6, j6))] : 0.0;
-                vii[u] = n > 1 ? PW0[oPW + (unsigned)(min(i, n - 2) * PWS + PW_II(j6, j6))] : 0.0;
-                vg[u] = PG0[oPG + (unsigned)(i * PGS + PG_H(j6, j6))];
+#pragma unroll
+                for (int q = 0; q < 3; ++q) {
+                    yj[u][q] = n > 1 ? PW0[oPW + (unsigned)(max(i - 1, 0) * PWC + 13 * q + 6 + j6)] : 0.0;
+                    yi[u][q] = n > 1 ? PW0[oPW + (unsigned)(min(i, n - 2) * PWC + 13 * q + j6)] : 0.0;
+                }
+                yg[u][0] = PG0[oPG + (unsigned)(i * PGC + j6)]; yg[u][1] = PG0[oPG + (unsigned)(i * PGC + 7 + j6)];
                 vi[u] = PI0[oPI + (unsigned)(i * PIFS + PIF_D + pi_tri(jc, jc))];
+            }
+#pragma unroll
+            for (int u = 0; u < 4; ++u) {
+                vjj[u] = wheel_gram(yj[u][0], yj[u][1], yj[u][2], yj[u][0], yj[u][1], yj[u][2]);
+                vii[u] = wheel_gram(yi[u][0], yi[u][1], yi[u][2], yi[u][0], yi[u][1], yi[u][2]);
+                vg[u] = ground_gram(yg[u][0], yg[u][1], yg[u][0], yg[u][1], gmult);
             }
 #pragma unroll
             for (int u = 0; u < 4; ++u) {
@@ -298,7 +309,7 @@
     }
     const double sc0 = l6 ? LMD[oSC + (unsigned)jc] : 0.0;
 
-    constexpr int S_IMU = 0, S_PL = 4 * PIFS, S_PW = S_PL + 4 * LPC, S_PG = S_PW + 4 * PWS, S_TR = S_PG + 4 * PGS + QPAD;
+    constexpr int S_IMU = 0, S_PL = 4 * PIFS, S_PW = S_PL + 4 * LPC, S_PG = S_PW + 4 * PWC, S_TR = S_PG + 4 * PGC + QPAD;
     constexpr int S_ZERO = S_TR + QTR, S_TAB = S_ZERO + QZB;
     static_assert(S_TAB + QTAB <= QTOT && 8 * QTOT < 65536, "LDS layout");
     const unsigned rPI[4] = {(unsigned)__builtin_amdgcn_readlane(oPI, 0), (unsigned)__builtin_amdgcn_readlane(oPI, 16), (unsigned)__builtin_amdgcn_readlane(oPI, 32), (unsigned)__builtin_amdgcn_readlane(oPI, 48)};
@@ -329,16 +340,16 @@
             });
         }
         {
-            const unsigned fl = (unsigned)(f * LPC), fw = (unsigned)((k >= 0 ? k : 0) * PWS), fg = (unsigned)(f * PGS);
-            constexpr int NPC = (4 * (LPC + PWS + PGS) + 127) / 128;
-            static_assert(NPC * 128 - 4 * (LPC + PWS + PGS) <= QPAD && LPC % 2 == 0 && PWS % 2 == 0 && PGS % 2 == 0, "stream pieces: pad, 16-byte slots");
+            const unsigned fl = (unsigned)(f * LPC), fw = (unsigned)((k >= 0 ? k : 0) * PWC), fg = (unsigned)(f * PGC);
+            constexpr int NPC = (4 * (LPC + PWC + PGC) + 127) / 128;
+            static_assert(NPC == 4 && NPC * 128 - 4 * (LPC + PWC + PGC) <= QPAD && LPC % 2 == 0 && PWC % 2 == 0 && PGC % 2 == 0, "stream pieces: pad, 16-byte slots");
             sfor<0, NPC>([&](auto P) {
                 constexpr int q0 = KI(P) * 128;
                 unsigned off = 0;
                 sfor<0, 12>([&](auto G) {
                     constexpr int g = KI(G);
-                    constexpr int st = g < 4 ? g * LPC : g < 8 ? 4 * LPC + (g - 4) * PWS : 4 * (LPC + PWS) + (g - 8) * PGS;
-                    constexpr int en = g == 11 ? (1 << 20) : st + (g < 4 ? LPC : g < 8 ? PWS : PGS);
+                    constexpr int st = g < 4 ? g * LPC : g < 8 ? 4 * LPC + (g - 4) * PWC : 4 * (LPC + PWC) + (g - 8) * PGC;
+                    constexpr int en = g == 11 ? (1 << 20) : st + (g < 4 ? LPC : g < 8 ? PWC : PGC);
                     if constexpr (st < q0 + 128 && en > q0) {
                         const unsigned v = (g < 4 ? rPLw[g & 3] + fl : g < 8 ? rPW[g & 3] + fw : rPGw[g & 3] + fg) + (unsigned)(lane2 - (st - q0));
                         if constexpr (st <= q0) off = v; else off = lane2 >= st - q0 ? v : off;
@@ -355,7 +366,7 @@
     {
         const int jt = j < 15 ? j : 0, cjt = 14 * jt - (jt * (jt - 1)) / 2, j6t = j < 6 ? j : 0;
         const bool t6 = j < 6, t15 = j == 15, tm = j < 15;
-        const int oL = S_PL + w * LPC, oW_ = S_PW + w * PWS, oG = S_PG + w * PGS, oI = S_IMU + w * PIFS;
+        const int oL = S_PL + w * LPC, oW_ = S_PW + w * PWC, oG = S_PG + w * PGC, oI = S_IMU + w * PIFS;
         auto put = [&](int k, bool on, int idx) { TAB[k * 64 + lane] = (unsigned short)(8 * (on ? idx : S_ZERO)); };
         const int role = t15 ? 6 : j6t;
         auto put_laser = [&](int k, bool on, int code) { put(k, on && code >= 0, oL + (code & 63)); };
@@ -363,13 +374,13 @@
         sfor<0, 6>([&](auto R) {
             constexpr int r = KI(R);
             put_laser(K_A + r, t6 || t15, quad_code<0, r>(track, role));
-            put(K_B + r, t6 || t15, oW_ + (t15 ? PW_G(6 + r) : PW_JJ(r, j6t)));
-            put(K_C + r, t6 || t15, oG + (t15 ? PG_G(r) : PG_H(r, j6t)));
             put_laser(K_HA + r, t6 || t15, quad_code<1, r>(track, role));
-            put(K_CW + r, t6 || t15, oW_ + (t15 ? PW_G(r) : PW_II(r, j6t)));
             put_laser(K_RL + r, t6, quad_code<2, r>(track, role));
         });
-        put(K_GSH, t6, oW_ + PW_G(j6t));
+        static_assert(QZB >= 27, "zero block behind a column read");
+        put(K_WJ, t6 || t15, oW_ + (t15 ? 12 : 6 + j6t));
+        put(K_WI, t6 || t15, oW_ + (t15 ? 12 : j6t));
+        put(K_GC, t6 || t15, oG + (t15 ? 6 : j6t));
         sfor<0, 15>([&](auto R) {
             constexpr int r = KI(R);
             put(K_D + r, tm, oI + PIF_D + tri_rc<r>(jt, cjt));
@@ -385,11 +396,6 @@
         sgR0 = (t6 && cR0 >= 0 && (cR0 & 64)) ? 0x80000000u : 0u;
     }
     const int lane_tab = lane * 2;
-    auto RD = [&](auto K) -> double {
-        constexpr int k = KI(K);
-        const unsigned off = *reinterpret_cast<const unsigned short*>(reinterpret_cast<const char*>(TAB) + k * 128 + lane_tab);
-        return *reinterpret_cast<const double*>(reinterpret_cast<const char*>(S) + off);
-    };
 #ifdef LIW_QUAD_TILE_ALIAS
     double* ST = S + S_IMU + w * PIFS + PIF_IJ + 100;
 #else
@@ -425,20 +431,30 @@
             auto tab_at = [&](int k) { return (unsigned)*reinterpret_cast<const unsigned short*>(reinterpret_cast<const char*>(TAB) + k * 128 + lane_tab); };
             sfor<0, NT>([&](auto Q) { constexpr int q = KI(Q); of[q] = tab_at(K_A + q); });
             sfor<0, 6>([&](auto Q) { constexpr int q = KI(Q); ofR[q] = tab_at(K_RL + q); });
+            const unsigned ofWJ = tab_at(K_WJ), ofWI = tab_at(K_WI), ofGC = tab_at(K_GC);
             if (n > 1) sfor<0, 15>([&](auto Q) { constexpr int q = KI(Q); of[NT + q] = tab_at(K_D + q); });
             const char* const Sb = reinterpret_cast<const char*>(S);
             const int w8 = (lane >> 4) * 8;
             const char* const bOV = Sb + (l15 ? 8 * (S_IMU + PIF_GJ) : 8 * (S_IMU + PIF_IJ) + jc * 120) + w8 * PIFS;
             const char* const bGI = Sb + (l15 ? 8 * (S_IMU + PIF_GI) + w8 * PIFS : 8 * S_ZERO);
-            const char* const bOW = Sb + (l6 ? 8 * (S_PW + PW_IJ(0, 0)) + w8 * PWS + j6 * 48 : 8 * S_ZERO);
+            const char* const bWR = Sb + 8 * S_PW + w8 * PWC;
+            const char* const bGR = Sb + 8 * S_PG + w8 * PGC;
             double gi[15];
             if (n > 1) {
                 sfor<0, 15>([&](auto R) { constexpr int r = KI(R); o[r] = *reinterpret_cast<const double*>(bOV + 8 * r); gi[r] = *reinterpret_cast<const double*>(bGI + 8 * r); });
             } else {
                 sfor<0, 15>([&](auto R) { constexpr int r = KI(R); d[r] = 0.0; o[r] = 0.0; gi[r] = 0.0; });
             }
-            sfor<0, 6>([&](auto R) { constexpr int r = KI(R); oW[r] = *reinterpret_cast<const double*>(bOW + 8 * r); });
+            double uJ[6][3], uG[6][2];
+            sfor<0, 3>([&](auto Q) {
+                constexpr int q = KI(Q);
+                sfor<0, 6>([&](auto R) { constexpr int r = KI(R); uJ[r][q] = *reinterpret_cast<const double*>(bWR + 8 * (13 * q + 6 + r)); });
+            });
+            sfor<0, 2>([&](auto Q) { constexpr int q = KI(Q); sfor<0, 6>([&](auto R) { constexpr int r = KI(R); uG[r][q] = *reinterpret_cast<const double*>(bGR + 8 * (7 * q + r)); }); });
             asm volatile("" ::: "memory");
+            double cJ[3], cI[3], cG[2];
+            sfor<0, 3>([&](auto Q) { constexpr int q = KI(Q); cJ[q] = *reinterpret_cast<const double*>(Sb + ofWJ + 8 * 13 * q); cI[q] = *reinterpret_cast<const double*>(Sb + ofWI + 8 * 13 * q); });
+            sfor<0, 2>([&](auto Q) { constexpr int q = KI(Q); cG[q] = *reinterpret_cast<const double*>(Sb + ofGC + 8 * 7 * q); });
             double pb[NT];
             sfor<0, NT>([&](auto Q) { constexpr int q = KI(Q); pb[q] = *reinterpret_cast<const double*>(Sb + of[q]); });
             sfor<0, 6>([&](auto R) { constexpr int r = KI(R); rL[r] = *reinterpret_cast<const double*>(Sb + ofR[r]); });
@@ -447,7 +463,15 @@
             pb[K_A + 0] = flip_sign(pb[K_A + 0], sgA0); pb[K_A + 1] = flip_sign(pb[K_A + 1], sgA0);
             pb[K_A + 3] = flip_sign(pb[K_A + 3], sgA3); pb[K_A + 4] = flip_sign(pb[K_A + 4], sgA3); pb[K_A + 5] = flip_sign(pb[K_A + 5], sgA3);
             rL[0] = flip_sign(rL[0], sgR0); rL[1] = flip_sign(rL[1], sgR0);
-            sfor<0, 6>([&](auto R) { constexpr int r = KI(R); tS[r] = pb[K_A + r] + bits_and(pb[K_B + r], mh) + pb[K_C + r]; });
+            const unsigned long long mP = (l6 || l15) ? ~0ull : 0ull, m6 = l6 ? ~0ull : 0ull;
+            const double gmult = (double)n;
+            sfor<0, 6>([&](auto R) {
+                constexpr int r = KI(R);
+                const double wjj = wheel_gram(uJ[r][0], uJ[r][1], uJ[r][2], cJ[0], cJ[1], cJ[2]);
+                const double ghh = ground_gram(uG[r][0], uG[r][1], cG[0], cG[1], gmult);
+                tS[r] = pb[K_A + r] + bits_and(wjj, mh & mP) + bits_and(ghh, mP);
+                oW[r] = bits_and(wheel_gram(cI[0], cI[1], cI[2], uJ[r][0], uJ[r][1], uJ[r][2]), m6);
+            });
             if (!track) {
                 sfor<0, 6>([&](auto R) { constexpr int r = KI(R); hA[r] += pb[K_HA + r]; });
                 if (i == 0) sfor<0, 6>([&](auto R) { tS[KI(R)] += hA[KI(R)]; });
@@ -546,8 +570,22 @@
         if (hasm) {
             dpp_fence();
             double cw[6];
-            sfor<0, 6>([&](auto R) { constexpr int r = KI(R); cw[r] = RD(KC<K_CW + r>{}); });
-            gsh = RD(KC<K_GSH>{});
+            {
+                const char* const Sb = reinterpret_cast<const char*>(S);
+                const unsigned ofWI = (unsigned)*reinterpret_cast<const unsigned short*>(reinterpret_cast<const char*>(TAB) + K_WI * 128 + lane_tab);
+                const char* const bWR = Sb + 8 * S_PW + (lane >> 4) * (8 * PWC);
+                double cI[3], uI[6][3], uR[3];
+                sfor<0, 3>([&](auto Q) {
+                    constexpr int q = KI(Q);
+                    sfor<0, 6>([&](auto R) { constexpr int r = KI(R); uI[r][q] = *reinterpret_cast<const double*>(bWR + 8 * (13 * q + r)); });
+                    uR[q] = *reinterpret_cast<const double*>(bWR + 8 * (13 * q + 12));
+                });
+                asm volatile("" ::: "memory");
+                sfor<0, 3>([&](auto Q) { constexpr int q = KI(Q); cI[q] = *reinterpret_cast<const double*>(Sb + ofWI + 8 * 13 * q); });
+                const unsigned long long mP = (l6 || l15) ? ~0ull : 0ull, m6 = l6 ? ~0ull : 0ull;
+                sfor<0, 6>([&](auto R) { constexpr int r = KI(R); cw[r] = bits_and(wheel_gram(uI[r][0], uI[r][1], uI[r][2], cI[0], cI[1], cI[2]), mP); });
+                gsh = bits_and(wheel_gram(cI[0], cI[1], cI[2], uR[0], uR[1], uR[2]), m6);
+            }
             __builtin_amdgcn_sched_barrier(0);
             sfor<0, 15>([&](auto R) {
                 constexpr int r = KI(R);
@@ -789,8 +827,8 @@
     return a.n >= 1 && (a.mode == LIW_MODE_INIT || (a.mode == LIW_MODE_TRACK && a.n >= 2)) && span(a.w.PL[0], a.w.PL[1], (unsigned long long)a.n * LPC) && a.w.pi_frame && a.w.pl_compact &&
            a.w.PL[0] >= a.w.PW[0] && span(a.w.PW[0], a.w.PL[1], (unsigned long long)a.n * LPC) &&
            a.w.CS[0] && a.w.CS[1] && span(a.w.PI[0], a.w.PI[1], (unsigned long long)a.n * PIFS) &&
-           span(a.w.PW[0], a.w.PW[1], (unsigned long long)nm * PWS) && span(a.w.PG[0], a.w.PG[1], (unsigned long long)a.n * PGS) &&
-           a.w.PG[0] >= a.w.PW[0] && span(a.w.PW[0], a.w.PG[1], (unsigned long long)a.n * PGS) &&
+           a.w.pw_compact && span(a.w.PW[0], a.w.PW[1], (unsigned long long)nm * PWC) && span(a.w.PG[0], a.w.PG[1], (unsigned long long)a.n * PGC) &&
+           a.w.PG[0] >= a.w.PW[0] && span(a.w.PW[0], a.w.PG[1], (unsigned long long)a.n * PGC) &&
            (unsigned long long)a.B * (sizeof(LmState) / 8) <= lim && (unsigned long long)a.B * a.n * SOLVE_WS <= lim;
 }
 extern "C" void liw_debug_quad_clk(int on, int block, int frame, int iteration, long long* out) {
diff --git a/2dliw-slam_amd/csrc/liw_capi.hip b/2dliw-slam_amd/csrc/liw_capi.hip
--- a/2dliw-slam_amd/csrc/liw_capi.hip
+++ b/2dliw-slam_amd/csrc/liw_capi.hip
@@ -221,6 +221,7 @@
     const int nm = n > 1 ? n - 1 : 1;
     const int lps = laser_stride(pi_frame_format(B) ? 1 : 0);
     for (int k = 0; k < 2; ++k) { f.PI[k] = o; o = al256(o + sizeof(double) * (size_t)B * pi_doubles_per_window(n)); }
+    static_assert(PWS >= PWC && PGS >= PGC, "wheel / ground buffers are sized by the expanded records");
     for (int k = 0; k < 2; ++k) { f.PW[k] = o; o = al256(o + sizeof(double) * (size_t)B * nm * PWS); }
     for (int k = 0; k < 2; ++k) { f.PL[k] = o; o = al256(o + sizeof(double) * (size_t)B * n * lps); }
     for (int k = 0; k < 2; ++k) { f.PG[k] = o; o = al256(o + sizeof(double) * (size_t)B * n * PGS); }
@@ -256,6 +257,7 @@
     v.active = (int*)(base + f.active);
     v.pi_frame = pi_frame_format(B) ? 1 : 0;
     v.pl_compact = v.pi_frame;
+    v.pw_compact = v.pi_frame;
     for (int k = 0; k < 2; ++k) v.CS[k] = (double*)(base + f.CS[k]);
     v.imu_pk = (double*)(base + f.imu_pk);
     v.imu_pk_bad = (int*)(base + f.imu_pk_bad);
@@ -271,6 +273,8 @@
     out->laser_partial_stride = laser_stride(pi_frame_format(B) ? 1 : 0);
     out->laser_partial_bytes = sizeof(double) * (size_t)B * n * out->laser_partial_stride;
     out->info_off = f.info;
+    out->cost_off[0] = f.CS[0];
+    out->cost_off[1] = f.CS[1];
     out->history_off = f.history;
     return LIW_OK;
 }
@@ -321,6 +325,7 @@
     A.candidate = candidate;
     A.pi_frame = v.pi_frame;
     A.pl_compact = v.pl_compact;
+    A.pw_compact = v.pw_compact;
     for (int k = 0; k < 2; ++k) A.CS[k] = v.pi_frame ? v.CS[k] : nullptr;
     if (packed && b->n > 1 && b->eval_small) { A.imu_pk = v.imu_pk; A.imu_pk_bad = v.imu_pk_bad; }
     if (packed) A.laser_hz = v.imu_pk_bad + 1;
@@ -426,6 +431,15 @@
     WsView v = make_view(ws, b->B, b->n, b->history_records);
     const size_t stride = (size_t)liw_batch_exchange_doubles(b->B, b->n, mode);
     launch_exchange_unpack(b->B, b->n, mode == LIW_MODE_INIT, v.pl_compact, copies, stride, buf, v.PL[0], v.PL[1], v.pi_frame ? v.CS[0] : nullptr, v.pi_frame ? v.CS[1] : nullptr, candidate, mode == LIW_MODE_MARG ? nullptr : v.lm, (hipStream_t)stream);
+    HIPCHK(c, hipGetLastError());
+    return LIW_OK;
+}
+int liw_batch_small_records(liw_ctx* c, const liw_batch* b, int buffer, void* ws, double* PW_out, double* PG_out, void* stream) {
+    NEEDDEV(c);
+    if (int r = check_batch(c, b, 1)) return r;
+    if ((!PW_out && !PG_out) || buffer < 0 || buffer > 1) return fail(c, LIW_EINVAL, "liw_batch_small_records: no output / buffer not 0 or 1");
+    WsView v = make_view(ws, b->B, b->n, b->history_records);
+    launch_small_expand(b->B, b->n, v.pw_compact, v.PW[buffer], v.PG[buffer], PW_out, PG_out, (hipStream_t)stream);
     HIPCHK(c, hipGetLastError());
     return LIW_OK;
 }
diff --git a/2dliw-slam_amd/csrc/liw_kernels.hpp b/2dliw-slam_amd/csrc/liw_kernels.hpp
--- a/2dliw-slam_amd/csrc/liw_kernels.hpp
+++ b/2dliw-slam_amd/csrc/liw_kernels.hpp
@@ -50,6 +50,49 @@
 __host__ __device__ constexpr int PG_H(int r, int c) { return tri_sym<7>(r, c); }
 __host__ __device__ constexpr int PG_G(int r) { return tri_sym<7>(r, 6); }
 constexpr int PG_C = 27;
+__host__ __device__ constexpr int wheel_rc(int e) {
+    int r = 12, c = 12;
+    if (e < PW_IJ(0, 0) || (e >= PW_JJ(0, 0) && e < PW_G(0))) {
+        const int jj = e >= PW_JJ(0, 0) ? 1 : 0;
+        int q = e - (jj ? PW_JJ(0, 0) : 0);
+        r = 0;
+        while (q >= 6 - r) { q -= 6 - r; ++r; }
+        c = r + q + (jj ? 6 : 0); r += jj ? 6 : 0;
+    } else if (e < PW_JJ(0, 0)) { r = (e - PW_IJ(0, 0)) / 6; c = 6 + (e - PW_IJ(0, 0)) % 6; }
+    else if (e < PW_C) { r = e - PW_G(0); c = 12; }
+    return e <= PW_C ? (r << 8) | c : -1;
+}
+__host__ __device__ constexpr int ground_rc(int e) {
+    int r = 0, c = e;
+    while (c >= 7 - r) { c -= 7 - r; ++r; }
+    return (r << 8) | (c + r);
+}
+constexpr int PWC = 40, PGC = 14;
+__host__ __device__ constexpr int wheel_stride(int compact) { return compact ? PWC : PWS; }
+__host__ __device__ constexpr int ground_stride(int compact) { return compact ? PGC : PGS; }
+__host__ __device__ inline double wheel_gram(double a0, double a1, double a2, double b0, double b1, double b2) {
+    return __builtin_fma(a2, b2, __builtin_fma(a0, b0, a1 * b1));
+}
+__host__ __device__ inline double ground_gram(double a0, double a1, double b0, double b1, double mult) {
+#pragma clang fp contract(off)
+    return mult * __builtin_fma(a1, b1, a0 * b0);
+}
+__host__ __device__ inline double wheel_pair(const double* y, int r, int c) {
+    return wheel_gram(y[r], y[13 + r], y[26 + r], y[c], y[13 + c], y[26 + c]);
+}
+__host__ __device__ inline double ground_pair(const double* y, int r, int c, double mult) {
+    return ground_gram(y[r], y[7 + r], y[c], y[7 + c], mult);
+}
+__host__ __device__ inline double wheel_entry(const double* y, int e) {
+    const int rc = wheel_rc(e);
+    return rc >= 0 ? wheel_pair(y, rc >> 8, rc & 255) : 0.0;
+}
+__host__ __device__ inline double ground_entry(const double* y, int e, double mult) {
+    const int rc = ground_rc(e);
+    return ground_pair(y, rc >> 8, rc & 255, mult);
+}
+__host__ __device__ inline double wheel_slot(const double* rec, int e, int compact) { return compact ? wheel_entry(rec, e) : rec[e]; }
+__host__ __device__ inline double ground_slot(const double* rec, int e, int compact, double mult) { return compact ? ground_entry(rec, e, mult) : rec[e]; }
 constexpr int FTF = 32;
 
 struct LmState {
@@ -81,6 +124,7 @@
     int* active;
     int pi_frame;
     int pl_compact;
+    int pw_compact;
     double* CS[2];
     double* imu_pk;
     int* imu_pk_bad;
@@ -113,6 +157,7 @@
     int* active;
     int pi_frame;
     int pl_compact;
+    int pw_compact;
     double* CS[2];
     const double* imu_pk;
     const int* imu_pk_bad;
@@ -293,6 +338,7 @@
 void launch_lm_finish(const StepArgs& a, hipStream_t s);
 void launch_export_dense(const ExportArgs& a, hipStream_t s);
 void launch_laser_expand(int B, int n, bool both, int compact, const double* PL, double* out, hipStream_t s);
+void launch_small_expand(int B, int n, int compact, const double* PW, const double* PG, double* PW_out, double* PG_out, hipStream_t s);
 void launch_marg_schur(const MargArgs& a, hipStream_t s);
 
 struct PreintNoise { double q_na[3], q_nw[3], q_nba[3], q_nbw[3], wheel_cov[3]; };
diff --git a/include/liw_window.h b/include/liw_window.h
--- a/include/liw_window.h
+++ b/include/liw_window.h
@@ -102,6 +102,7 @@
     size_t info_off;
     size_t history_off;
     int laser_partial_stride;
+    size_t cost_off[2];
 } liw_ws_layout;
 #define LIW_LASER_PARTIAL 128
 #define LIW_LASER_PARTIAL_COMPACT 48
@@ -115,6 +116,7 @@
 int liw_batch_packed_rows(liw_ctx* ctx, const liw_batch* b, const void* ws, long long* rows, long long* blocks);
 int liw_batch_lm_linearize(liw_ctx* ctx, const liw_batch* b, int mode, int candidate, void* ws, void* stream);
 int liw_batch_laser_records(liw_ctx* ctx, const liw_batch* b, int mode, int buffer, void* ws, double* out, void* stream);
+int liw_batch_small_records(liw_ctx* ctx, const liw_batch* b, int buffer, void* ws, double* PW_out, double* PG_out, void* stream);
 int liw_batch_lm_step(liw_ctx* ctx, const liw_batch* b, int mode, void* ws, void* stream);
 int liw_batch_lm_finish(liw_ctx* ctx, const liw_batch* b, int mode, void* ws, void* stream);
 int liw_batch_lm_linearize_async(liw_ctx* ctx, const liw_batch* b, int mode, int candidate, void* ws, void* stream);
```
